# sq/Illuminant

Measured on AMD Instinct MI355X. Metric: Mparticle-steps/sec + lit Mpixels/sec (4K, 256 point lights) at 1/2/4/8 GPUs, higher is better.
Workload: dtype f32

## Files before the change

illuminant_amd/csrc/api.hip:

```cpp
#include <atomic>
#include <dlfcn.h>
#include <hip/hip_runtime.h>

#include <cstdarg>
#include <cmath>
#include <cstdio>
#include <cstdlib>
#include <algorithm>
#include <functional>
#include <array>
#include <cstring>
#include <mutex>
#include <new>
#include <unordered_map>
#include <vector>

#include "internal.hpp"

namespace {

using namespace ilm;

constexpr int kPlanePad = 1088;

// ... 120 lines not shown
            const hipError_t e = hipStreamWaitEvent(owner->main(), sh.readers[i].second, 0);
            if (e != hipSuccess) return e;
            sh.pending[i] = false;
        }
    return hipSuccess;
}
inline hipError_t shared_before_read(Shared& sh, Ctx* owner, Ctx* reader) {
    if (!sh.owner_ev) { const hipError_t e = hipEventCreateWithFlags(&sh.owner_ev, hipEventDisableTiming); if (e != hipSuccess) return e; }
    hipError_t e = hipEventRecord(sh.owner_ev, owner->main());
    if (e != hipSuccess) return e;
    return hipStreamWaitEvent(reader->main(), sh.owner_ev, 0);
}
inline hipError_t shared_after_read(Shared& sh, Ctx* reader) {
    size_t i = 0;
    while (i < sh.readers.size() && sh.readers[i].first != reader) i++;
    if (i == sh.readers.size()) {
        hipEvent_t ev = nullptr;
        const hipError_t e = hipEventCreateWithFlags(&ev, hipEventDisableTiming);
        if (e != hipSuccess) return e;
        sh.readers.emplace_back(reader, ev); sh.pending.push_back(false);
    }
    const hipError_t e = hipEventRecord(sh.readers[i].second, reader->main());
    if (e == hipSuccess) sh.pending[i] = true;
    return e;
}
inline bool siblings(const Ctx* a, const Ctx* b) { return a == b || (a->family != 0 && a->family == b->family && a->device == b->device); }

struct Sdf {
    uint32_t magic = kMagicSdf;
    Ctx* ctx = nullptr;
    Shared shared;
    uint2* texels = nullptr; int width = 0, height = 0, format = 0;
    int filter = ILM_SDF_FILTER_FP32;
    void* cells = nullptr; size_t cells_bytes = 0;
    uint64_t version = 1, cells_version = 0;
    void* cells0 = nullptr; size_t cells0_bytes = 0; uint64_t cells0_version = 0;
    int cells_slices = 0, cells_columns = 0, cells_sw = 0, cells_sh = 0;
    bool escaped = false;
    static constexpr int kDirtyWords = (kMaxTableSlices + 63) / 64;
    uint64_t dirty[kDirtyWords];
    Sdf() { for (uint64_t& w : dirty) w = ~0ull; }
    void mark_all_dirty() { for (uint64_t& w : dirty) w = ~0ull; version++; }
    void mark_slices_dirty(int first, int count) {
        const int64_t lo = std::max<int64_t>(0, (int64_t)first - 1), hi = std::min<int64_t>((int64_t)first + (int64_t)count, (int64_t)kDirtyWords * 64);
        for (int64_t v = lo; v < hi; v++) dirty[v >> 6] |= 1ull << (v & 63);
        version++;
    }
    uint64_t cell_rebuilds = 0, cell_slices_rebuilt = 0;
    int last_rebuilt_slices = 0, last_table_slices = 0;
};

struct GBuffer {
    uint32_t magic = kMagicGBuffer;
    Ctx* ctx = nullptr;
    Shared shared;
    void* texels = nullptr; int width = 0, height = 0, format = 0;
};

struct Lightmap {
    uint32_t magic = kMagicLightmap;
    Ctx* ctx = nullptr;
    void* texels = nullptr; int width = 0, height = 0, format = 0; bool external = false;
    void** d_mirrors = nullptr; int mirror_count = 0;
};

struct RenderKey {
    IlmClampedBezier4 color_from_life, color_from_velocity;
    IlmClampedBezier1 size_from_life, size_from_velocity;
    float rotation_from_life_and_index[2];
    IlmFloat4 life_ramp;
    float velocity_rotation;
};
static_assert(sizeof(RenderKey) == sizeof(float) * (2 * 20 + 2 * 8 + 2 + 4 + 1), "RenderKey has no padding");

struct System {
    uint32_t magic = kMagicSystem;
    Engine* engine = nullptr;
    std::vector<float*> chunks;
    std::vector<int32_t> used;
    std::vector<uint64_t> render_gen;
    std::vector<uint8_t> ptr_out;
    RenderKey render_key; uint64_t render_key_gen = 0;
    bool render_captured = false;
    DeviceScratch d_table; bool table_dirty = true;
    unsigned long long* d_counts = nullptr; int counts_cap = 0; int count_parity = 0;
    unsigned long long* counts_region(int r) const { return d_counts + (size_t)r * (size_t)counts_cap * kCountLines * kCountStride; }
    static size_t counts_bytes(int cap) { return sizeof(unsigned long long) * (size_t)cap * kCountStride * (4 * kCountLines + 1); }
    int split_at = -1;
    IlmHandle sdf_handle = 0;
    float4* ramp = nullptr; int ramp_w = 0, ramp_h = 0;
    DeviceScratch d_slots, d_slot_count;
    DeviceScratch spawn_positions[ILM_MAX_SPAWNS]; int spawn_position_count[ILM_MAX_SPAWNS] = {};
    float4* bitmap = nullptr; int bitmap_w = 0, bitmap_h = 0;
    float4* spawn_pattern[ILM_MAX_SPAWNS] = {}; int pattern_w[ILM_MAX_SPAWNS] = {}, pattern_h[ILM_MAX_SPAWNS] = {}, pattern_levels[ILM_MAX_SPAWNS] = {};
    unsigned long long* h_counts = nullptr; unsigned long long* h_counts_dev = nullptr; int h_counts_cap = 0;
    uint32_t count_seq = 0; int counts_first = 0, counts_span = 0;
    int counts_n = 0; bool counts_pending = false;
    bool counts_valid = false;
    uint32_t* h_sense = nullptr; size_t h_sense_cap = 0;
    hipEvent_t sense_ev = nullptr;
    int sense_n = 0; bool sense_pending = false;
};

SdfView make_sdf_view(const Sdf* f, const IlmDistanceFieldUniforms* df) {
    SdfView v;
    v.texels = f ? f->texels : nullptr;
    v.width = f ? f->width : 0;
    v.height = f ? f->height : 0;
    v.format = f ? f->format : ILM_SDF_UNORM16;
    v.wf = (float)v.width;
    v.hf = (float)v.height;
    v.inv_wf = v.width > 0 ? 1.0f / v.wf : 0.0f;
    v.wrap_half = 0.0f;
    v.cells0 = nullptr;
    v.table_slices = 0; v.columns = 1;
    v.box_x0 = v.box_y0 = v.box_z0 = 1.0f; v.box_x1 = v.box_y1 = v.box_z1 = 0.0f;
    if (df && v.width > 0) {
        const double cols = df->TextureSliceCount.x, rows = df->TextureSliceCount.y, slices = df->TextureSliceCount.w;
        const double isx = df->ConeAndMisc.w, isy = df->StepAndMisc2.w, ex = df->Extent.x, ey = df->Extent.y, ez = df->Extent.z;
        auto nearest = [](double x) { const double r = std::floor(x + 0.5); return (std::fabs(x - r) <= 1e-6 * std::fmax(1.0, r)) ? r : x; };
        const double sw = nearest(ex / isx), sh = nearest(ey / isy);
        auto whole = [](double x) { return std::isfinite(x) && x >= 1.0 && x == std::floor(x); };
        const bool consistent =
            whole(cols) && whole(rows) && whole(slices) && whole(sw) && whole(sh) && slices <= kMaxTableSlices && cols <= 1024 &&
            cols * sw == (double)v.width && rows * sh == (double)v.height && std::ceil(slices / 3.0) <= cols * rows &&
            std::fabs((double)df->TextureSliceAndTexelSize.x * cols - 1.0) < 1e-6 && std::fabs((double)df->TextureSliceAndTexelSize.y * rows - 1.0) < 1e-6 &&
            std::fabs((double)df->TextureSliceAndTexelSize.z * ex * cols - 1.0) < 1e-6 && std::fabs((double)df->TextureSliceAndTexelSize.w * ey * rows - 1.0) < 1e-6 &&
            ez > 0 && std::isfinite(ez) && std::isfinite((double)df->ConeAndMisc.y) && df->Packed1.y > 0.0f && std::isfinite((double)df->Packed1.y) &&
            df->Packed1.z > 0.0f && sw >= 4 && sh >= 4;
        bool rows_agree = consistent;
        for (int vi = 0; rows_agree && vi < (int)slices; vi++)
            rows_agree = floorf((float)vi * df->Packed1.x) == (float)((vi / 3) / (int)cols);
        if (consistent && rows_agree) {
            v.table_slices = (int)slices;
            v.columns = (int)cols;
            const double tx = 0.5625 * isx, ty = 0.5625 * isy;
            v.box_x0 = (float)tx; v.box_x1 = (float)(ex - tx);
            v.box_y0 = (float)ty; v.box_y1 = (float)(ey - ty);
            const double zmax = std::min({ (double)df->Packed1.z, ez, (slices - 1e-3) / (double)df->Packed1.y });
            v.box_z0 = df->ConeAndMisc.y; v.box_z1 = (float)((double)df->ConeAndMisc.y + zmax * (1.0 - 1e-6));
        }
    }
    if (df && v.width > 0) {
        const double third_max = std::floor(std::fabs((double)df->Packed1.z * (double)df->Packed1.y)) / 3.0 + 1.0;
        const double u_max = third_max * std::fabs((double)df->TextureSliceAndTexelSize.x) +
                             std::fabs((double)df->Extent.x * (double)df->TextureSliceAndTexelSize.z) + 1.0;
        const double x_max = u_max * (double)v.width;
        if (x_max == x_max && x_max < 1048576.0)
            v.wrap_half = 0.5f * v.inv_wf;
    }
    return v;
}

static const char* field_extent_unusable(const IlmDistanceFieldUniforms* df, char* text, size_t n) {
    if (!df) return nullptr;
    const float e[3] = { df->Extent.x, df->Extent.y, df->Extent.z };
    for (int k = 0; k < 3; k++) {
        if (std::isfinite(e[k]) && e[k] >= 0.0f) continue;
        snprintf(text, n, "the distance-field Extent.%c is %g: the field's extent must be finite and >= 0", "xyz"[k], (double)e[k]);
        return text;
    }
    return nullptr;
}

const char* field_uniforms_mismatch(const Sdf* f, const IlmDistanceFieldUniforms* df, char* text, size_t n) {
    if (!f || !df) return nullptr;
// ... 159 lines not shown
}
inline size_t align64(size_t x) { return (x + 63) & ~(size_t)63; }

int32_t reserve_field_params(Ctx* c, size_t total) { return reserve(c, c->d_field_params, total, total < 65536 ? 65536 : total * 2); }
int32_t check_volume_ranges(const IlmHeightVolume* volumes, int32_t volume_count, int32_t polygon_vertex_count) {
    for (int i = 0; i < volume_count; i++)
        if (volumes[i].FirstVertex < 0 || volumes[i].VertexCount < 0 || volumes[i].FirstVertex + volumes[i].VertexCount > polygon_vertex_count)
            return fail(ILM_ERR_OUT_OF_RANGE, "height volume %d vertex range outside the polygon array", i);
    return ILM_OK;
}
int32_t ensure_staging(Ctx* c, size_t bytes) { return reserve(c, c->staging, bytes, std::max<size_t>(bytes, (size_t)1 << 20)); }

int32_t upload_small_begin(Ctx* c, size_t bytes, void** host, int* slot_out) {
    const int slot = c->ring_pos;
    c->ring_pos = (c->ring_pos + 1) % Ctx::kRing;
    if (c->pinned_ev[slot] == nullptr)
        HIP_TRY(hipEventCreateWithFlags(&c->pinned_ev[slot], hipEventDisableTiming));
    else
        HIP_TRY(hipEventSynchronize(c->pinned_ev[slot]));
    if (c->pinned_bytes[slot] < bytes) {
        if (c->pinned[slot]) HIP_TRY(hipHostFree(c->pinned[slot]));
        c->pinned[slot] = nullptr; c->pinned_bytes[slot] = 0;
        size_t cap = bytes < 65536 ? 65536 : bytes;
        HIP_TRY(hipHostMalloc(&c->pinned[slot], cap, hipHostMallocDefault));
        c->pinned_bytes[slot] = cap;
    }
    *host = c->pinned[slot];
    *slot_out = slot;
    return ILM_OK;
}
__global__ __launch_bounds__(256) void copy_from_pinned_kernel(const uint4* __restrict__ src, uint4* __restrict__ dst, size_t words, size_t bytes) {
    for (size_t i = (size_t)blockIdx.x * 256 + threadIdx.x; i < words; i += (size_t)gridDim.x * 256) dst[i] = src[i];
    if (blockIdx.x == 0 && threadIdx.x < (bytes & 15)) {
        const size_t at = (bytes & ~(size_t)15) + threadIdx.x;
        reinterpret_cast<unsigned char*>(dst)[at] = reinterpret_cast<const unsigned char*>(src)[at];
    }
}
int32_t upload_small_commit(Ctx* c, void* dst, int slot, size_t bytes) {
    if (bytes > 4096 && bytes <= ((size_t)2 << 20) && (reinterpret_cast<uintptr_t>(dst) & 15) == 0) {
        void* dv = nullptr;
        HIP_TRY(hipHostGetDevicePointer(&dv, c->pinned[slot], 0));
        const size_t words = bytes / 16;
        const unsigned blocks = (unsigned)std::min<size_t>((words + 255) / 256, 1024);
        hipLaunchKernelGGL(copy_from_pinned_kernel, dim3(blocks ? blocks : 1), dim3(256), 0, c->main(), static_cast<const uint4*>(dv), static_cast<uint4*>(dst), words, bytes);
        HIP_TRY(hipGetLastError());
    } else {
        HIP_TRY(hipMemcpyAsync(dst, c->pinned[slot], bytes, hipMemcpyHostToDevice, c->main()));
    }
    HIP_TRY(hipEventRecord(c->pinned_ev[slot], c->main()));
    return ILM_OK;
}

int32_t upload_small(Ctx* c, void* dst, const void* src, size_t bytes) {
    void* host = nullptr;
    int slot = -1;
    const int32_t rc = upload_small_begin(c, bytes, &host, &slot);
    if (rc != ILM_OK) return rc;
    memcpy(host, src, bytes);
    return upload_small_commit(c, dst, slot, bytes);
}

int32_t stage_small(Ctx* c, const void* src, size_t bytes, const void** device_visible, int* slot_out) {
    void* host = nullptr;
    const int32_t rc = upload_small_begin(c, bytes, &host, slot_out);
    if (rc != ILM_OK) return rc;
    memcpy(host, src, bytes);
    void* dev = nullptr;
    HIP_TRY(hipHostGetDevicePointer(&dev, host, 0));
    *device_visible = dev;
    return ILM_OK;
}
int32_t staged_small_done(Ctx* c, int slot) {
    HIP_TRY(hipEventRecord(c->pinned_ev[slot], c->main()));
    return ILM_OK;
}

int32_t refresh_table(System* s) {
    Ctx* c = s->engine->ctx;
    const int n = (int)s->chunks.size();
    if (sizeof(float*) * (size_t)n > s->d_table.bytes) {
        const int32_t rc = reserve(c, s->d_table, sizeof(float*) * (size_t)n, sizeof(float*) * (size_t)(n < 64 ? 64 : n * 2));
        if (rc != ILM_OK) return rc;
        s->table_dirty = true;
    }
    if (n > s->counts_cap) {
        if (s->d_counts) { HIP_TRY(hipStreamSynchronize(c->main())); HIP_TRY(hipFree(s->d_counts)); s->d_counts = nullptr; }
        int cap = n < 64 ? 64 : n * 2;
        HIP_TRY(hipMalloc(reinterpret_cast<void**>(&s->d_counts), System::counts_bytes(cap)));
        HIP_TRY(hipMemsetAsync(s->d_counts, 0, System::counts_bytes(cap), c->main()));
        unsigned long long* old = s->h_counts;
        unsigned long long* fresh = nullptr;
        HIP_TRY(hipHostMalloc(reinterpret_cast<void**>(&fresh), sizeof(unsigned long long) * (size_t)cap, hipHostMallocMapped));
        for (int i = 0; i < cap; i++) fresh[i] = (i < s->h_counts_cap && old) ? old[i] : 0ull;
        if (old) HIP_TRY(hipHostFree(old));
        s->h_counts = fresh;
        HIP_TRY(hipHostGetDevicePointer(reinterpret_cast<void**>(&s->h_counts_dev), fresh, 0));
        s->h_counts_cap = cap;
        s->counts_cap = cap;
    }
    if (s->table_dirty && n > 0) {
        int32_t rc = upload_small(c, s->d_table.p, s->chunks.data(), sizeof(float*) * (size_t)n);
        if (rc != ILM_OK) return rc;
    }
    s->table_dirty = false;
    return ILM_OK;
}

static bool randomness_offset_unusable(const float off[2], const char* owner, int k, const char* what, char* text, size_t n) {
    for (int a = 0; a < 2; a++) {
        if (std::fabs(off[a]) < 4194304.0f) continue;
        snprintf(text, n, "%s %d: %s.%c is %g, outside (-2^22, 2^22)", owner, k, what, "xy"[a], (double)off[a]);
        return true;
    }
    return false;
}

static bool position_index_unusable(const IlmSpawnParams& p, int k, char* text, size_t n) {
    const float w = p.ChunkSizeAndIndices[3], count = p.PositionConstantCount, rate = p.PolygonRate;
    if (!std::isfinite(rate)) {
        snprintf(text, n, "spawn record %d: PolygonRate %g is not finite", k, (double)rate);
        return true;
    }
    if (count != std::floor(count)) {
        snprintf(text, n, "spawn record %d: PositionConstantCount %g is not an integer", k, (double)count);
        return true;
    }
    const bool polygon = rate > 0.05f;
    if (!(w >= 0.0f && w < count) || (!polygon && w != std::floor(w))) {
        snprintf(text, n, "spawn record %d: ChunkSizeAndIndices.w %g is not %s in [0, PositionConstantCount = %g)", k, (double)w,
                 polygon ? "a number" : "an integer", (double)count);
        return true;
    }
    return false;
}

int32_t validate_step(const System* s, const IlmStepDesc* d, int* first, int* count) {
    const int n = (int)s->chunks.size();
    if (d->OpCount < 0 || d->OpCount > ILM_MAX_OPS)
        return fail(ILM_ERR_TOO_MANY, "OpCount %d outside [0, %d]", d->OpCount, ILM_MAX_OPS);
    if (d->SpawnCount < 0 || d->SpawnCount > ILM_MAX_SPAWNS)
        return fail(ILM_ERR_TOO_MANY, "SpawnCount %d outside [0, %d]", d->SpawnCount, ILM_MAX_SPAWNS);
    if (d->UpdateMode < ILM_UPDATE_NONE || d->UpdateMode > ILM_UPDATE_ERASE)
        return fail(ILM_ERR_INVALID_ARGUMENT, "unknown UpdateMode %d", d->UpdateMode);
    for (int o = 0; o < d->OpCount; o++) {
        const IlmTransformOp& op = d->Ops[o];
        if (op.Type == ILM_OP_GRAVITY) {
            if (op.u.Gravity.AttractorCount > ILM_MAX_ATTRACTORS || op.u.Gravity.AttractorCount < 0)
                return fail(ILM_ERR_TOO_MANY, "Maximum number of attractors per instance is %d", ILM_MAX_ATTRACTORS);
        } else if (op.Type == ILM_OP_NOISE) {
            char why[256];
            if (randomness_offset_unusable(op.u.Noise.RandomnessOffset, "op", o, "RandomnessOffset", why, sizeof(why)) ||
                randomness_offset_unusable(op.u.Noise.NextRandomnessOffset, "op", o, "NextRandomnessOffset", why, sizeof(why)))
                return fail(ILM_ERR_OUT_OF_RANGE, "%s", why);
        } else if (op.Type != ILM_OP_FMA && op.Type != ILM_OP_MATRIX_MULTIPLY && op.Type != ILM_OP_SPATIAL_NOISE) {
            return fail(ILM_ERR_INVALID_ARGUMENT, "unknown transform type %d", op.Type);
        }
    }
    for (int k = 0; k < d->SpawnCount; k++) {
        const IlmSpawnRecord& r = d->Spawns[k];
        if (r.ChunkIndex < 0 || r.ChunkIndex >= n)
            return fail(ILM_ERR_OUT_OF_RANGE, "spawn target chunk %d outside [0, %d)", r.ChunkIndex, n);
        const float cs = r.Params.ChunkSizeAndIndices[0], first_i = r.Params.ChunkSizeAndIndices[1], last_i = r.Params.ChunkSizeAndIndices[2];
        if ((int)cs != s->engine->chunk_size)
            return fail(ILM_ERR_INVALID_ARGUMENT, "ChunkSizeAndIndices.x %g != engine chunk size %d", (double)cs, s->engine->chunk_size);
        if (first_i < 0 || last_i >= (float)s->engine->slots)
            return fail(ILM_ERR_OUT_OF_RANGE, "spawn range [%g, %g] outside the chunk", (double)first_i, (double)last_i);
// ... 324 lines not shown
                const float divisor = (op.Type == ILM_OP_NOISE) ? op.u.Noise.TimeDivisor : op.u.FMA.TimeDivisor;
                const int t = ar.AreaType < 0 ? -ar.AreaType : ar.AreaType;
                dv.op[o].area_none = (t < 1 || t > 5) ? 1 : 0;
                dv.op[o].t = ar.Strength * dt_ms / divisor;
                if (op.Type == ILM_OP_NOISE) {
                    const IlmNoiseParams& np = op.u.Noise;
                    const bool inert = (np.PositionScale.w == 0.0f) && std::isfinite(np.PositionOffset.w) && std::isfinite(np.PositionMinimum.w) &&
                                       std::isfinite(ar.Strength) && std::isfinite(dt_ms) && std::isfinite(divisor) && (divisor != 0.0f) &&
                                       std::isfinite(ar.AreaFalloff);
                    if (!inert) dv.noise_may_revive = 1;
                }
            } else if (op.Type == ILM_OP_SPATIAL_NOISE) {
                const IlmNoiseParams& np = op.u.SpatialNoise.Noise;
                const bool inert = (np.PositionScale.w == 0.0f) && std::isfinite(np.PositionOffset.w) && std::isfinite(np.Area.Strength) &&
                                   std::isfinite(dt_ms) && std::isfinite(np.TimeDivisor) && (np.TimeDivisor != 0.0f) && std::isfinite(np.Area.AreaFalloff);
                if (!inert) dv.noise_may_revive = 1;
            }
        }
    }
    a.partial_count = 0;
    {
        const bool noise_op = (a.op_mask & ((1u << ILM_OP_NOISE) | (1u << ILM_OP_SPATIAL_NOISE))) != 0u;
        const bool noise_touches_dead = noise_op && ((d->UpdateMode == ILM_UPDATE_NONE) || (a.derived.noise_may_revive != 0));
        for (int ci = first; noise_touches_dead && ci < first + count; ci++) s->used[(size_t)ci] = e->slots;
        for (int ci = first; !noise_touches_dead && ci < first + count && a.partial_count < kMaxPartialChunks; ci++) {
            const int used_units = (s->used[(size_t)ci] + 63) / 64;
            if (used_units * 64 < e->slots) {
                a.partial_chunk[a.partial_count] = ci;
                a.partial_units[a.partial_count] = used_units;
                a.partial_count++;
            }
        }
    }
    return ILM_OK;
}
static void finish_step(System* s, const IlmStepDesc* d, int first, int count) {
    if (d->UpdateMode == ILM_UPDATE_ERASE)
        for (int ci = first; ci < first + count; ci++) s->used[(size_t)ci] = 0;
    if (d->Flags & ILM_STEP_COUNT_LIVE) {
        s->counts_n = (int)s->chunks.size();
        s->counts_first = first; s->counts_span = count;
        s->counts_pending = true;
        s->counts_valid = true;
        s->count_parity ^= 1;
    }
}

int32_t run_step(System* s, const IlmStepDesc* d) {
    int first = 0, count = 0;
    StepLaunch a;
    const int32_t rc = prepare_step(s, d, a, &first, &count);
    if (rc != ILM_OK || count == 0) return rc;
    Engine* e = s->engine;
    Ctx* c = e->ctx;
    const bool counting = (d->Flags & ILM_STEP_COUNT_LIVE) != 0;
    const int region = s->count_parity;
    int mid = -1;
    if (step_streams() >= 2 && !c->exported && count >= 2 && (int64_t)count * (e->span / 64) >= kSplitMinUnits) {
        bool reads_other_chunks = false;
        for (int k = 0; k < d->SpawnCount; k++) reads_other_chunks = reads_other_chunks || (d->Spawns[k].Kind == ILM_SPAWN_FEEDBACK);
        if (!reads_other_chunks) {
            int64_t total = 0, left = 0;
            for (int ci = first; ci < first + count; ci++) total += (s->used[(size_t)ci] + 63) / 64 + 1;
            mid = first + 1;
            for (int ci = first; ci < first + count - 1; ci++) {
                left += (s->used[(size_t)ci] + 63) / 64 + 1;
                mid = ci + 1;
                if (2 * left >= total) break;
            }
        }
    }
    const uint64_t key = (d->UpdateMode == ILM_UPDATE_POSITIONS) ? render_key_generation(s, d) : 0;
    if (stream_capturing(c->stream_) || stream_capturing(c->aux)) s->render_captured = true;
    auto render_elide = [&](int lo, int hi) -> uint32_t {
        bool current = key != 0 && !s->render_captured;
        for (int ci = lo; current && ci < hi; ci++) current = (s->render_gen[(size_t)ci] == key) && !s->ptr_out[(size_t)ci];
        return current ? kElideDerived : 0u;
    };
    auto render_refreshed = [&](int lo, int hi, bool refreshed) {
        for (int ci = lo; ci < hi; ci++) s->render_gen[(size_t)ci] = (refreshed && key != 0 && !s->render_captured && !s->ptr_out[(size_t)ci]) ? key : 0;
    };
    const uint32_t elide_a = render_elide(first, (mid < 0) ? first + count : mid), elide_b = (mid < 0) ? 0u : render_elide(mid, first + count);
    render_refreshed(first, first + count, false);
    bool fresh_a = false, fresh_b = false;
    if (mid < 0) {
        HIP_TRY(launch_step(a, c->main(), elide_a, &fresh_a));
        render_refreshed(first, first + count, fresh_a);
    } else {
        if (s->split_at != mid) { (void)c->main(); s->split_at = mid; }
        if (c->main_pending) {
            HIP_TRY(hipEventRecord(c->ev_main, c->stream_));
            HIP_TRY(hipStreamWaitEvent(c->aux, c->ev_main, 0));
            c->main_pending = false;
        }
        StepLaunch b = a;
        a.chunk_count = mid - first;
        b.first_chunk = mid; b.chunk_count = first + count - mid;
        if (counting) {
            a.zero_n = b.zero_n = (int32_t)s->counts_cap * kCountLines;
            b.live_counts = s->counts_region(region * 2 + 1);
            b.zero_counts = s->counts_region((region ^ 1) * 2 + 1);
        }
        bool spawn_in_b = false;
        for (int k = 0; k < d->SpawnCount; k++) spawn_in_b = spawn_in_b || (d->Spawns[k].ChunkIndex >= mid);
        if (spawn_in_b) {
            HIP_TRY(launch_step(b, c->aux, elide_b, &fresh_b));
            c->aux_pending = true;
            HIP_TRY(launch_step(a, c->stream_, elide_a, &fresh_a));
        } else {
            HIP_TRY(launch_step(a, c->stream_, elide_a, &fresh_a));
            HIP_TRY(launch_step(b, c->aux, elide_b, &fresh_b));
            c->aux_pending = true;
        }
        render_refreshed(first, mid, fresh_a);
        render_refreshed(mid, first + count, fresh_b);
    }
    finish_step(s, d, first, count);
    return ILM_OK;
}

static int32_t fail_item(int32_t code, int item) {
    char text[sizeof(g_last_error)];
    snprintf(text, sizeof(text), "item %d: %s", item, g_last_error);
    memcpy(g_last_error, text, sizeof(text));
    return code;
}
int32_t run_step_batch(Engine* e, const IlmHandle* handles, const IlmStepDesc* descs, int32_t count) {
    Ctx* c = e->ctx;
    constexpr int kUnitsPerBlock = kStepThreads / 64;
    std::vector<System*> sys((size_t)count);
    size_t block_bound = 0;
    for (int i = 0; i < count; i++) {
        System* s = from_handle<System>(handles[i], kMagicSystem);
        if (!s) return fail(ILM_ERR_INVALID_HANDLE, "item %d: not a system handle", i);
        if (s->engine != e) return fail(ILM_ERR_INVALID_ARGUMENT, "item %d: the system belongs to another engine", i);
        int first = 0, n = 0;
        const int32_t rc = validate_step(s, &descs[i], &first, &n);
        if (rc != ILM_OK) return fail_item(rc, i);
        sys[(size_t)i] = s;
        block_bound += ((size_t)n * (size_t)(e->span / 64) + kUnitsPerBlock - 1) / kUnitsPerBlock;
    }
    HIP_TRY(hipSetDevice(c->device));
    const bool capturing = stream_capturing(c->stream_) || stream_capturing(c->aux);

    const size_t table_bytes = sizeof(StepBatchItem) * (size_t)count, bytes = table_bytes + sizeof(int32_t) * block_bound;
    StepBatchItem* items = nullptr;
    int32_t* item_of_block = nullptr;
    std::vector<StepLaunch> captured;
    int slot = -1;
    if (capturing) {
        captured.resize((size_t)count);
    } else {
        slot = e->batch_pos;
        e->batch_pos = (e->batch_pos + 1) % Engine::kBatchRing;
        if (e->batch_ev[slot] == nullptr) HIP_TRY(hipEventCreateWithFlags(&e->batch_ev[slot], hipEventDisableTiming));
        else HIP_TRY(hipEventSynchronize(e->batch_ev[slot]));
        if (e->batch_pinned_bytes[slot] < bytes) {
            if (e->batch_pinned[slot]) HIP_TRY(hipHostFree(e->batch_pinned[slot]));
            e->batch_pinned[slot] = nullptr; e->batch_pinned_bytes[slot] = 0;
            const size_t cap = std::max(bytes + bytes / 2, (size_t)1 << 16);
            HIP_TRY(hipHostMalloc(&e->batch_pinned[slot], cap, hipHostMallocDefault));
            e->batch_pinned_bytes[slot] = cap;
        }
        if (e->d_batch_bytes < bytes) {
            const size_t cap = std::max(std::max(bytes, e->d_batch_bytes * 2), (size_t)1 << 16);
            if (e->d_batch) e->d_batch_outgrown.push_back(e->d_batch);
            e->d_batch = nullptr; e->d_batch_bytes = 0;
            HIP_TRY(hipMalloc(&e->d_batch, cap));
            e->d_batch_bytes = cap;
        }
        items = static_cast<StepBatchItem*>(e->batch_pinned[slot]);
        item_of_block = reinterpret_cast<int32_t*>(static_cast<unsigned char*>(e->batch_pinned[slot]) + table_bytes);
    }
    auto record = [&](int i) -> StepLaunch& { return capturing ? captured[(size_t)i] : items[i].a; };

    struct Planned { int round, variant, blocks; };
    std::vector<Planned> plan((size_t)count);
    std::unordered_map<const System*, int> last_round;
    int rounds = 0, fallback = 0;
    for (int i = 0; i < count; i++) {
        System* s = sys[(size_t)i];
        const IlmStepDesc* d = &descs[i];
        int first = 0, n = 0;
        const int32_t rc = prepare_step(s, d, record(i), &first, &n);
        if (rc != ILM_OK) return fail_item(rc, i);
        plan[(size_t)i] = Planned{ 0, -1, 0 };
        if (n == 0) continue;
        if (d->UpdateMode == ILM_UPDATE_POSITIONS) (void)render_key_generation(s, d);
        if (capturing) s->render_captured = true;
        for (int ci = first; ci < first + n; ci++) s->render_gen[(size_t)ci] = 0;
        finish_step(s, d, first, n);

        Planned& p = plan[(size_t)i];
        p.variant = step_batch_layout(record(i), &p.blocks);
        if (capturing) p.variant = -1;
        if (p.variant < 0) fallback++;
        int after = last_round[s];
        for (int k = 0; k < d->SpawnCount; k++)
            if (d->Spawns[k].Kind == ILM_SPAWN_FEEDBACK) after = std::max(after, last_round[from_handle<System>(d->Spawns[k].Feedback.SourceSystem, kMagicSystem)]);
        p.round = after + 1;
        last_round[s] = p.round;
        for (int k = 0; k < d->SpawnCount; k++)
            if (d->Spawns[k].Kind == ILM_SPAWN_FEEDBACK) last_round[from_handle<System>(d->Spawns[k].Feedback.SourceSystem, kMagicSystem)] = p.round;
        rounds = std::max(rounds, p.round);
    }

    struct Launch { int round, variant, first_block, blocks, item; };
    std::vector<Launch> launches;
    size_t blocks_used = 0;
    for (int r = 1; r <= rounds; r++) {
        const size_t round_begin = launches.size();
        for (int i = 0; i < count; i++) {
            const Planned& p = plan[(size_t)i];
            if (p.round != r) continue;
            if (p.variant < 0) continue;
            size_t at = round_begin;
            while (at < launches.size() && launches[at].variant != p.variant) at++;
            if (at == launches.size()) launches.push_back(Launch{ r, p.variant, 0, 0, -1 });
            launches[at].blocks += p.blocks;
        }
        for (size_t l = round_begin; l < launches.size(); l++) {
            launches[l].first_block = (int)blocks_used;
            int block = 0;
            for (int i = 0; i < count; i++) {
                const Planned& p = plan[(size_t)i];
                if (p.round != r || p.variant != launches[l].variant) continue;
                items[i].first_block = block;
                items[i].block_count = p.blocks;
                for (int b = 0; b < p.blocks; b++) item_of_block[blocks_used + (size_t)block + (size_t)b] = i;
                block += p.blocks;
            }
            blocks_used += (size_t)launches[l].blocks;
        }
        for (int i = 0; i < count; i++)
            if (plan[(size_t)i].round == r && plan[(size_t)i].variant < 0) launches.push_back(Launch{ r, -1, 0, 0, i });
    }
    if (blocks_used > block_bound) return fail(ILM_ERR_STATE, "step batch: %zu blocks planned, %zu reserved", blocks_used, block_bound);

    const hipStream_t stream = c->main();
    int kernel_launches = 0;
    if (blocks_used > 0) {
        HIP_TRY(hipMemcpyAsync(e->d_batch, e->batch_pinned[slot], table_bytes + sizeof(int32_t) * blocks_used, hipMemcpyHostToDevice, stream));
        HIP_TRY(hipEventRecord(e->batch_ev[slot], stream));
    }
    const StepBatchItem* d_items = static_cast<const StepBatchItem*>(e->d_batch);
    const int32_t* d_item_of_block = reinterpret_cast<const int32_t*>(static_cast<const unsigned char*>(e->d_batch) + table_bytes);
    for (const Launch& l : launches) {
        if (l.variant >= 0) {
            HIP_TRY(launch_step_batch(l.variant, d_items, d_item_of_block + l.first_block, l.blocks, stream));
            kernel_launches++;
        } else {
            HIP_TRY(launch_step(record(l.item), stream, 0u, nullptr));
        }
    }
    e->last_batch_launches = kernel_launches; e->last_batch_rounds = rounds; e->last_batch_fallback = fallback;
    return ILM_OK;
}

int32_t copy_counts(System* s, const unsigned long long* d_region64, uint32_t* out, int32_t capacity, int32_t saturate16) {
    const uint32_t* d_region = reinterpret_cast<const uint32_t*>(d_region64);
    Ctx* c = s->engine->ctx;
    const int n = (int)s->chunks.size();
    if (capacity < n)
        return fail(ILM_ERR_OUT_OF_RANGE, "capacity %d < chunk count %d", capacity, n);
    if (n == 0) return ILM_OK;
    const size_t bytes = sizeof(uint32_t) * (size_t)n * kCountStride;
    std::vector<uint32_t> fallback;
    const uint32_t* tmp = nullptr;
    if ((reinterpret_cast<uintptr_t>(d_region) & 15) == 0 && bytes <= ((size_t)2 << 20)) {
        unsigned char* block = nullptr;
        int slot = -1;
        const int32_t rc = upload_small_begin(c, bytes, reinterpret_cast<void**>(&block), &slot);
        if (rc != ILM_OK) return rc;
        void* dv = nullptr;
        HIP_TRY(hipHostGetDevicePointer(&dv, block, 0));
        const size_t words = bytes / 16;
        hipLaunchKernelGGL(copy_from_pinned_kernel, dim3((unsigned)std::max<size_t>(1, std::min<size_t>((words + 255) / 256, 1024))), dim3(256), 0, c->main(),
                           reinterpret_cast<const uint4*>(d_region), static_cast<uint4*>(dv), words, bytes);
        HIP_TRY(hipGetLastError());
        const int32_t rc2 = staged_small_done(c, slot);
        if (rc2 != ILM_OK) return rc2;
        HIP_TRY(hipStreamSynchronize(c->main()));
        tmp = reinterpret_cast<const uint32_t*>(block);
    } else {
        fallback.resize((size_t)n * kCountStride);
        HIP_TRY(hipMemcpyAsync(fallback.data(), d_region, bytes, hipMemcpyDeviceToHost, c->main()));
        HIP_TRY(hipStreamSynchronize(c->main()));
        tmp = fallback.data();
    }
    for (int i = 0; i < n; i++) {
        const uint32_t v = tmp[(size_t)i * kCountStride];
        out[i] = (saturate16 && v > ref::kLiveCountSaturation) ? ref::kLiveCountSaturation : v;
    }
    return ILM_OK;
}

}

namespace ilm {
int32_t api_fail(int32_t code, const char* fmt, ...) {
    va_list ap;
    va_start(ap, fmt);
    vsnprintf(g_last_error, sizeof(g_last_error), fmt, ap);
    va_end(ap);
    return code;
}
IlmHandle handle_register(const void* object, uint32_t magic) {
    HandleRegistry& r = handle_registry();
    std::lock_guard<std::mutex> lock(r.mutex);
    r.live[reinterpret_cast<uintptr_t>(object)] = magic;
    return static_cast<IlmHandle>(reinterpret_cast<uintptr_t>(object));
}
bool handle_is_live(IlmHandle h, uint32_t magic) {
    HandleRegistry& r = handle_registry();
    std::lock_guard<std::mutex> lock(r.mutex);
    const auto it = r.live.find(static_cast<uintptr_t>(h));
    return it != r.live.end() && it->second == magic;
}
void handle_retire(const void* object) { retire_handle(object); }
int ctx_child_count(IlmHandle h) {
    const Ctx* c = from_handle<Ctx>(h, kMagicCtx);
    return c ? c->children : -1;
}
int set_step_streams(int n) { return set_step_streams_impl(n); }
int32_t system_chunk_view(IlmHandle system, int chunk, bool written, float** out_base, int64_t* out_stride, int32_t* out_chunk_size, IlmHandle* out_ctx) {
    System* s = from_handle<System>(system, kMagicSystem);
    if (!s) return fail(ILM_ERR_INVALID_HANDLE, "not a system handle");
    if (chunk < 0 || chunk >= (int)s->chunks.size()) return fail(ILM_ERR_OUT_OF_RANGE, "chunk %d outside [0, %d)", chunk, (int)s->chunks.size());
    if (out_base) *out_base = s->chunks[(size_t)chunk];
    if (out_stride) *out_stride = s->engine->stride;
    if (out_chunk_size) *out_chunk_size = s->engine->chunk_size;
    if (out_ctx) *out_ctx = to_handle(s->engine->ctx);
    if (written) {
        s->used[(size_t)chunk] = s->engine->slots;
        s->render_gen[(size_t)chunk] = 0;
    }
    return ILM_OK;
}
hipStream_t ctx_stream_joined(IlmHandle h) {
    Ctx* c = from_handle<Ctx>(h, kMagicCtx);
    return c ? c->main() : nullptr;
}
const TraceApi& trace_api() {
    static const TraceApi api = [] {
        TraceApi t;
        const char* e = getenv("ILM_TRACE");
        if (!e || atoi(e) == 0) return t;
        for (const char* name : { "librocprofiler-sdk-roctx.so.1", "librocprofiler-sdk-roctx.so", "libroctx64.so.4", "libroctx64.so" }) {
            void* lib = dlopen(name, RTLD_NOW | RTLD_GLOBAL);
            if (!lib) continue;
            t.push = reinterpret_cast<int (*)(const char*)>(dlsym(lib, "roctxRangePushA"));
            t.pop = reinterpret_cast<int (*)()>(dlsym(lib, "roctxRangePop"));
            if (t.push && t.pop) { t.on = true; break; }
        }
        if (!t.on) fprintf(stderr, "libilluminant_hip: ILM_TRACE is set but no roctx library could be bound: no ranges\n");
        return t;
    }();
    return api;
}
static std::mutex g_armed_mutex;
static std::vector<Lightmap*> g_armed;
static std::atomic<int> g_armed_count{0};
static void forget_armed(const Lightmap* m) {
    std::lock_guard<std::mutex> lock(g_armed_mutex);
    g_armed.erase(std::remove(g_armed.begin(), g_armed.end(), m), g_armed.end());
    g_armed_count.store((int)g_armed.size(), std::memory_order_release);
}

int32_t lightmap_set_mirrors(IlmHandle h, void* const* buffers, int count) {
    Lightmap* m = from_handle<Lightmap>(h, kMagicLightmap);
    if (!m) return fail(ILM_ERR_INVALID_HANDLE, "not a lightmap handle");
    if (count < 0 || count > 64 || (count > 0 && !buffers)) return fail(ILM_ERR_INVALID_ARGUMENT, "bad mirror list");
    HIP_TRY(hipSetDevice(m->ctx->device));
    HIP_TRY(hipStreamSynchronize(m->ctx->main()));
    std::vector<Lightmap*>& armed = m->ctx->mirrored;
    armed.erase(std::remove(armed.begin(), armed.end(), m), armed.end());
    forget_armed(m);
    if (count == 0) {
        if (m->d_mirrors) HIP_TRY(hipFree(m->d_mirrors));
        m->d_mirrors = nullptr; m->mirror_count = 0;
        return ILM_OK;
    }
    if (!m->d_mirrors) HIP_TRY(hipMalloc(reinterpret_cast<void**>(&m->d_mirrors), sizeof(void*) * 64));
    HIP_TRY(hipMemcpy(m->d_mirrors, buffers, sizeof(void*) * (size_t)count, hipMemcpyHostToDevice));
    m->mirror_count = count;
    armed.push_back(m);
    {
        std::lock_guard<std::mutex> lock(g_armed_mutex);
        g_armed.push_back(m);
        g_armed_count.store((int)g_armed.size(), std::memory_order_release);
    }
    return ILM_OK;
}

static const Lightmap* mirror_table_of(const Lightmap* m, bool* foreign) {
    *foreign = false;
    if (m->d_mirrors && m->mirror_count > 0) return m;
    if (!m->external || g_armed_count.load(std::memory_order_acquire) == 0) return nullptr;
    for (const Lightmap* e : m->ctx->mirrored)
        if (e->texels == m->texels && e->width == m->width && m->height <= e->height && e->format == m->format && e->d_mirrors && e->mirror_count > 0) return e;
    std::lock_guard<std::mutex> lock(g_armed_mutex);
    for (const Lightmap* e : g_armed)
        if (e->texels == m->texels && e->ctx != m->ctx) *foreign = true;
    return nullptr;
}
static int32_t set_launch_mirrors(const Lightmap* m, LightLaunch* a) {
    bool foreign = false;
    const Lightmap* t = mirror_table_of(m, &foreign);
    if (foreign)
        return fail(ILM_ERR_STATE, "the lightmap aliases the buffer of a group lightmap member that ANOTHER context holds in store mode: a pass from here "
                                   "would not be mirrored into the other members' frames (render through the member's context, or disarm the mode)");
    a->mirrors = t ? t->d_mirrors : nullptr; a->mirror_count = t ? t->mirror_count : 0;
    return ILM_OK;
}
}

extern "C" {

// ... 152 lines not shown
    *out = h;
    return ILM_OK;
}

static int32_t acquire_chunk(Engine* e, float** out) {
    if (e->spare.empty()) {
        const size_t bytes = e->chunk_bytes();
        const int k = (int)std::min<size_t>(8, std::max<size_t>(1, ((size_t)64 << 20) / bytes));
        float* base = nullptr;
        hipError_t err = hipMalloc(reinterpret_cast<void**>(&base), bytes * (size_t)k);
        int got = k;
        if (err != hipSuccess && k > 1) { (void)hipGetLastError(); got = 1; err = hipMalloc(reinterpret_cast<void**>(&base), bytes); }
        if (err != hipSuccess) return fail((int32_t)err, "a particle chunk of %zu bytes: %s", bytes, hipGetErrorString(err));
        HIP_TRY(hipMemsetAsync(base, 0, bytes * (size_t)got, e->ctx->main()));
        e->slabs.push_back(Engine::Slab{ base, got });
        for (int i = got - 1; i >= 0; i--) e->spare.push_back(base + (size_t)i * (bytes / sizeof(float)));
    }
    *out = e->spare.back();
    e->spare.pop_back();
    return ILM_OK;
}
static void release_chunk(Engine* e, float* chunk) {
    (void)hipMemsetAsync(chunk, 0, e->chunk_bytes(), e->ctx->main());
    e->spare.push_back(chunk);
    const size_t chunk_floats = e->chunk_bytes() / sizeof(float);
    while ((int)e->spare.size() > Engine::kSpareChunks) {
        size_t victim = e->slabs.size();
        for (size_t i = 0; i < e->slabs.size() && victim == e->slabs.size(); i++) {
            const float* lo = e->slabs[i].base; const float* hi = lo + (size_t)e->slabs[i].chunks * chunk_floats;
            int spare_here = 0;
            for (const float* p : e->spare) spare_here += (p >= lo && p < hi) ? 1 : 0;
            if (spare_here == e->slabs[i].chunks) victim = i;
        }
        if (victim == e->slabs.size()) break;
        const float* lo = e->slabs[victim].base; const float* hi = lo + (size_t)e->slabs[victim].chunks * chunk_floats;
        e->spare.erase(std::remove_if(e->spare.begin(), e->spare.end(), [&](const float* p) { return p >= lo && p < hi; }), e->spare.end());
        (void)hipStreamSynchronize(e->ctx->main());
        (void)hipFree(e->slabs[victim].base);
        e->slabs.erase(e->slabs.begin() + (long)victim);
    }
}

int32_t ilm_engine_destroy(IlmHandle h) {
    Engine* e = from_handle<Engine>(h, kMagicEngine);
    if (!e) return fail(ILM_ERR_INVALID_HANDLE, "not an engine handle");
    if (e->children > 0) return fail(ILM_ERR_STATE, "%d system(s) of this engine are still alive", e->children);
    e->ctx->children--;
    (void)hipSetDevice(e->ctx->device);
    (void)hipStreamSynchronize(e->ctx->main());
    if (e->rnd) (void)hipFree(e->rnd);
    if (e->rnd_lp) (void)hipFree(e->rnd_lp);
    for (const Engine::Slab& slab : e->slabs) (void)hipFree(slab.base);
    for (int k = 0; k < Engine::kBatchRing; k++) {
        if (e->batch_pinned[k]) (void)hipHostFree(e->batch_pinned[k]);
        if (e->batch_ev[k]) (void)hipEventDestroy(e->batch_ev[k]);
    }
    if (e->d_batch) (void)hipFree(e->d_batch);
    for (void* p : e->d_batch_outgrown) (void)hipFree(p);
    retire_handle(e);
    delete e;
    return ILM_OK;
}

int32_t ilm_system_create(IlmHandle hengine, IlmHandle* out) {
    Engine* e = from_handle<Engine>(hengine, kMagicEngine);
    if (!e) return fail(ILM_ERR_INVALID_HANDLE, "not an engine handle");
    if (!out) return fail(ILM_ERR_INVALID_ARGUMENT, "NULL argument");
    System* s = new (std::nothrow) System();
    if (!s) return fail(ILM_ERR_INVALID_ARGUMENT, "out of host memory");
    s->engine = e;
    e->children++;
    *out = to_handle(s);
    return ILM_OK;
}

int32_t ilm_system_destroy(IlmHandle h) {
    System* s = from_handle<System>(h, kMagicSystem);
    if (!s) return fail(ILM_ERR_INVALID_HANDLE, "not a system handle");
    Ctx* c = s->engine->ctx;
    s->engine->children--;
    (void)hipSetDevice(c->device);
    (void)hipStreamSynchronize(c->main());
    for (float* p : s->chunks) release_chunk(s->engine, p);
    for (DeviceScratch* b : { &s->d_table, &s->d_slots, &s->d_slot_count }) release(*b);
    for (DeviceScratch& b : s->spawn_positions) release(b);
    if (s->d_counts) (void)hipFree(s->d_counts);
    if (s->ramp) (void)hipFree(s->ramp);
    for (int k = 0; k < ILM_MAX_SPAWNS; k++)
        if (s->spawn_pattern[k]) (void)hipFree(s->spawn_pattern[k]);
    if (s->bitmap) (void)hipFree(s->bitmap);
    if (s->h_counts) (void)hipHostFree(s->h_counts);
    if (s->h_sense) (void)hipHostFree(s->h_sense);
    if (s->sense_ev) (void)hipEventDestroy(s->sense_ev);
    retire_handle(s);
    delete s;
    return ILM_OK;
}

int32_t ilm_system_add_chunk(IlmHandle h, int32_t* out_index) {
    System* s = from_handle<System>(h, kMagicSystem);
    if (!s) return fail(ILM_ERR_INVALID_HANDLE, "not a system handle");
    Engine* e = s->engine;
    HIP_TRY(hipSetDevice(e->ctx->device));
    float* base = nullptr;
    { const int32_t rc = acquire_chunk(e, &base); if (rc != ILM_OK) return rc; }
    s->chunks.push_back(base);
    s->used.push_back(0);
    s->render_gen.push_back(0);
    s->ptr_out.push_back(0);
    s->table_dirty = true;
    if (out_index) *out_index = (int32_t)s->chunks.size() - 1;
    return ILM_OK;
}

int32_t ilm_system_remove_chunk(IlmHandle h, int32_t index) {
    System* s = from_handle<System>(h, kMagicSystem);
    if (!s) return fail(ILM_ERR_INVALID_HANDLE, "not a system handle");
    if (index < 0 || index >= (int)s->chunks.size())
        return fail(ILM_ERR_OUT_OF_RANGE, "chunk %d outside [0, %d)", index, (int)s->chunks.size());
    Ctx* c = s->engine->ctx;
    HIP_TRY(hipSetDevice(c->device));
    HIP_TRY(hipStreamSynchronize(c->main()));
    release_chunk(s->engine, s->chunks[(size_t)index]);
    s->chunks.erase(s->chunks.begin() + index);
    s->used.erase(s->used.begin() + index);
    s->render_gen.erase(s->render_gen.begin() + index);
    s->ptr_out.erase(s->ptr_out.begin() + index);
    s->table_dirty = true;
    return ILM_OK;
}

int32_t ilm_system_chunk_count(IlmHandle h, int32_t* out_count) {
    System* s = from_handle<System>(h, kMagicSystem);
    if (!s || !out_count) return fail(ILM_ERR_INVALID_HANDLE, "not a system handle");
    *out_count = (int32_t)s->chunks.size();
    return ILM_OK;
}

static int32_t check_plane_range(System* s, int32_t chunk, int32_t plane, int32_t first_slot, int32_t count) {
    if (chunk < 0 || chunk >= (int)s->chunks.size())
        return fail(ILM_ERR_OUT_OF_RANGE, "chunk %d outside [0, %d)", chunk, (int)s->chunks.size());
    if (plane < ILM_PLANE_POSITION || plane > ILM_PLANE_RENDER_DATA)
        return fail(ILM_ERR_INVALID_ARGUMENT, "unknown plane %d", plane);
    if (first_slot < 0 || count < 0 || first_slot + count > s->engine->slots)
        return fail(ILM_ERR_OUT_OF_RANGE, "slot range [%d, %d) outside [0, %d)", first_slot, first_slot + count, s->engine->slots);
    return ILM_OK;
}

int32_t ilm_chunk_upload(IlmHandle h, int32_t chunk, int32_t plane, const IlmFloat4* src, int32_t first_slot, int32_t count) {
    ILM_TRACE_RANGE("ilm_chunk_upload");
    System* s = from_handle<System>(h, kMagicSystem);
    if (!s) return fail(ILM_ERR_INVALID_HANDLE, "not a system handle");
    if (!src) return fail(ILM_ERR_INVALID_ARGUMENT, "src is NULL");
    int32_t rc = check_plane_range(s, chunk, plane, first_slot, count);
    if (rc != ILM_OK || count == 0) return rc;
    Engine* e = s->engine; Ctx* c = e->ctx;
    HIP_TRY(hipSetDevice(c->device));
    const size_t bytes = sizeof(float4) * (size_t)count;
    rc = ensure_staging(c, bytes);
    if (rc != ILM_OK) return rc;
    HIP_TRY(hipMemcpyAsync(c->staging.p, src, bytes, hipMemcpyHostToDevice, c->main()));
    s->used[(size_t)chunk] = std::max(s->used[(size_t)chunk], first_slot + count);
    s->render_gen[(size_t)chunk] = 0;
    HIP_TRY(launch_aos_to_soa(c->staging.as<const float4>(), s->chunks[(size_t)chunk] + (int64_t)plane * 4 * e->stride,
                              e->stride, first_slot, count, c->main()));
    HIP_TRY(hipStreamSynchronize(c->main()));
    return ILM_OK;
}

int32_t ilm_chunk_download(IlmHandle h, int32_t chunk, int32_t plane, IlmFloat4* dst, int32_t first_slot, int32_t count) {
    ILM_TRACE_RANGE("ilm_chunk_download");
    System* s = from_handle<System>(h, kMagicSystem);
    if (!s) return fail(ILM_ERR_INVALID_HANDLE, "not a system handle");
    if (!dst) return fail(ILM_ERR_INVALID_ARGUMENT, "dst is NULL");
    int32_t rc = check_plane_range(s, chunk, plane, first_slot, count);
    if (rc != ILM_OK || count == 0) return rc;
    Engine* e = s->engine; Ctx* c = e->ctx;
    HIP_TRY(hipSetDevice(c->device));
    const size_t bytes = sizeof(float4) * (size_t)count;
    rc = ensure_staging(c, bytes);
    if (rc != ILM_OK) return rc;
    HIP_TRY(launch_soa_to_aos(s->chunks[(size_t)chunk] + (int64_t)plane * 4 * e->stride, e->stride,
                              c->staging.as<float4>(), first_slot, count, c->main()));
    HIP_TRY(hipMemcpyAsync(dst, c->staging.p, bytes, hipMemcpyDeviceToHost, c->main()));
    HIP_TRY(hipStreamSynchronize(c->main()));
    return ILM_OK;
}

int32_t ilm_chunk_device_ptr(IlmHandle h, int32_t chunk, int32_t component, void** out_ptr, int64_t* out_stride) {
    System* s = from_handle<System>(h, kMagicSystem);
    if (!s) return fail(ILM_ERR_INVALID_HANDLE, "not a system handle");
    if (chunk < 0 || chunk >= (int)s->chunks.size() || component < 0 || component >= kComponents)
        return fail(ILM_ERR_OUT_OF_RANGE, "chunk/component out of range");
    if (out_ptr) *out_ptr = s->chunks[(size_t)chunk] + (int64_t)component * s->engine->stride;
    s->used[(size_t)chunk] = s->engine->slots;
    s->render_gen[(size_t)chunk] = 0;
    s->ptr_out[(size_t)chunk] = 1;
    if (out_stride) *out_stride = s->engine->stride;
    return ILM_OK;
}

int32_t ilm_system_set_distance_field(IlmHandle h, IlmHandle hsdf) {
    System* s = from_handle<System>(h, kMagicSystem);
    if (!s) return fail(ILM_ERR_INVALID_HANDLE, "not a system handle");
    if (hsdf == 0) { s->sdf_handle = 0; return ILM_OK; }
    Sdf* f = from_handle<Sdf>(hsdf, kMagicSdf);
    if (!f) return fail(ILM_ERR_INVALID_HANDLE, "not a distance field handle");
    if (f->ctx != s->engine->ctx) return fail(ILM_ERR_INVALID_ARGUMENT, "distance field belongs to another context");
    { char why[256]; if (field_filter_unsupported(f, "a particle system", why, sizeof(why))) return fail(ILM_ERR_INVALID_ARGUMENT, "%s", why); }
    s->sdf_handle = hsdf;
    return ILM_OK;
}

int32_t ilm_system_set_life_ramp(IlmHandle h, const IlmFloat4* texels, int32_t width, int32_t height) {
    System* s = from_handle<System>(h, kMagicSystem);
    if (!s) return fail(ILM_ERR_INVALID_HANDLE, "not a system handle");
    Ctx* c = s->engine->ctx;
    HIP_TRY(hipSetDevice(c->device));
    HIP_TRY(hipStreamSynchronize(c->main()));
    if (s->ramp) { HIP_TRY(hipFree(s->ramp)); s->ramp = nullptr; s->ramp_w = s->ramp_h = 0; }
    if (!texels || width <= 0 || height <= 0) return ILM_OK;
    const size_t bytes = sizeof(float4) * (size_t)width * (size_t)height;
    HIP_TRY(hipMalloc(reinterpret_cast<void**>(&s->ramp), bytes));
    HIP_TRY(hipMemcpy(s->ramp, texels, bytes, hipMemcpyHostToDevice));
    s->ramp_w = width; s->ramp_h = height;
    return ILM_OK;
}

int32_t ilm_system_set_spawn_positions(IlmHandle h, int32_t slot, const IlmFloat4* positions, int32_t count) {
    System* s = from_handle<System>(h, kMagicSystem);
    if (!s) return fail(ILM_ERR_INVALID_HANDLE, "not a system handle");
    if (slot < 0 || slot >= ILM_MAX_SPAWNS) return fail(ILM_ERR_OUT_OF_RANGE, "spawn slot %d outside [0, %d)", slot, ILM_MAX_SPAWNS);
    if (count < 0 || (count > 0 && !positions)) return fail(ILM_ERR_INVALID_ARGUMENT, "bad position list");
    if (count > (1 << 20)) return fail(ILM_ERR_TOO_MANY, "at most %d positions", 1 << 20);
    Ctx* c = s->engine->ctx;
    HIP_TRY(hipSetDevice(c->device));
    int32_t rc = reserve(c, s->spawn_positions[slot], sizeof(float4) * (size_t)count, sizeof(float4) * (size_t)((count + 127) / 128 * 128));
    if (rc != ILM_OK) return rc;
    if (count > 0) {
        rc = upload_small(c, s->spawn_positions[slot].p, positions, sizeof(float4) * (size_t)count);
        if (rc != ILM_OK) return rc;
    }
    s->spawn_position_count[slot] = count;
    return ILM_OK;
}

int32_t ilm_system_set_spawn_pattern(IlmHandle h, int32_t slot, const IlmFloat4* texels, int32_t width, int32_t height, int32_t levels) {
    System* s = from_handle<System>(h, kMagicSystem);
    if (!s) return fail(ILM_ERR_INVALID_HANDLE, "not a system handle");
    if (slot < 0 || slot >= ILM_MAX_SPAWNS) return fail(ILM_ERR_OUT_OF_RANGE, "spawn slot %d outside [0, %d)", slot, ILM_MAX_SPAWNS);
    if (levels < 0 || levels > 16) return fail(ILM_ERR_OUT_OF_RANGE, "%d mip levels outside [0, 16]", levels);
    if (levels > 0 && (!texels || width < 1 || height < 1 || width > 16384 || height > 16384))
        return fail(ILM_ERR_INVALID_ARGUMENT, "bad pattern texture (%d x %d)", width, height);
    Ctx* c = s->engine->ctx;
    HIP_TRY(hipSetDevice(c->device));
    HIP_TRY(hipStreamSynchronize(c->main()));
    if (s->spawn_pattern[slot]) HIP_TRY(hipFree(s->spawn_pattern[slot]));
    s->spawn_pattern[slot] = nullptr;
    s->pattern_w[slot] = s->pattern_h[slot] = s->pattern_levels[slot] = 0;
    if (levels == 0) return ILM_OK;
    size_t total = 0;
    for (int l = 0, lw = width, lh = height; l < levels; l++) {
        total += (size_t)lw * (size_t)lh;
        lw = std::max(1, lw >> 1); lh = std::max(1, lh >> 1);
    }
    HIP_TRY(hipMalloc(reinterpret_cast<void**>(&s->spawn_pattern[slot]), sizeof(float4) * total));
    HIP_TRY(hipMemcpy(s->spawn_pattern[slot], texels, sizeof(float4) * total, hipMemcpyHostToDevice));
    s->pattern_w[slot] = width; s->pattern_h[slot] = height; s->pattern_levels[slot] = levels;
    return ILM_OK;
}

int32_t ilm_system_step(IlmHandle h, const IlmStepDesc* desc) {
    ILM_TRACE_RANGE("ilm_system_step");
    System* s = from_handle<System>(h, kMagicSystem);
    if (!s) return fail(ILM_ERR_INVALID_HANDLE, "not a system handle");
    if (!desc) return fail(ILM_ERR_INVALID_ARGUMENT, "desc is NULL");
    return run_step(s, desc);
}

// ... 405 lines not shown
    HIP_TRY(hipMemcpyAsync(out_distances, d_out, out_bytes, hipMemcpyDeviceToHost, c->main()));
    HIP_TRY(hipStreamSynchronize(c->main()));
    return ILM_OK;
}

int32_t ilm_debug_sdf_sample_inside(IlmHandle h, const IlmDistanceFieldUniforms* df, const float* positions, int32_t count, float* out_distances,
                                    int32_t* out_used_table) {
    Sdf* f = from_handle<Sdf>(h, kMagicSdf);
    if (!f) return fail(ILM_ERR_INVALID_HANDLE, "not a distance field handle");
    if (!df || count < 0 || (count > 0 && (!positions || !out_distances || !out_used_table))) return fail(ILM_ERR_INVALID_ARGUMENT, "bad arguments");
    { char why[256]; if (field_extent_unusable(df, why, sizeof(why))) return fail(ILM_ERR_INVALID_ARGUMENT, "%s", why); }
    if (count == 0) return ILM_OK;
    Ctx* c = f->ctx;
    HIP_TRY(hipSetDevice(c->device));
    const size_t in_bytes = sizeof(float) * 3 * (size_t)count, out_bytes = sizeof(float) * (size_t)count;
    int32_t rc = ensure_staging(c, in_bytes + 2 * out_bytes);
    if (rc != ILM_OK) return rc;
    float* d_in = c->staging.as<float>();
    float* d_out = d_in + 3 * (size_t)count;
    int32_t* d_used = reinterpret_cast<int32_t*>(d_out + (size_t)count);
    HIP_TRY(hipMemcpyAsync(d_in, positions, in_bytes, hipMemcpyHostToDevice, c->main()));
    TraceSdfView view;
    HIP_TRY(make_trace_view(f, df, c->main(), &view));
    HIP_TRY(launch_sdf_sample_inside(view, *df, d_in, count, d_out, d_used, c->main(), f->filter));
    HIP_TRY(hipMemcpyAsync(out_distances, d_out, out_bytes, hipMemcpyDeviceToHost, c->main()));
    HIP_TRY(hipMemcpyAsync(out_used_table, d_used, out_bytes, hipMemcpyDeviceToHost, c->main()));
    HIP_TRY(hipStreamSynchronize(c->main()));
    return ILM_OK;
}

int32_t ilm_debug_divide_by_constants(IlmHandle hctx, float* out_divisors, uint64_t* out_mismatches, int32_t capacity, int32_t* out_count) {
    Ctx* c = from_handle<Ctx>(hctx, kMagicCtx);
    if (!c) return fail(ILM_ERR_INVALID_HANDLE, "not a context handle");
    if (!out_divisors || !out_mismatches || !out_count || capacity < 2) return fail(ILM_ERR_INVALID_ARGUMENT, "bad arguments");
    HIP_TRY(hipSetDevice(c->device));
    float pairs[2][2];
    light_constant_divisors(pairs);
    for (int i = 0; i < 2; i++) {
        HIP_TRY(hipMemsetAsync(c->d_stats, 0, 2 * sizeof(unsigned long long), c->main()));
        HIP_TRY(launch_divide_by_constant(pairs[i][0], pairs[i][1], c->d_stats, c->main()));
        unsigned long long bad[2] = { 0, 0 };
        HIP_TRY(hipMemcpyAsync(bad, c->d_stats, sizeof(bad), hipMemcpyDeviceToHost, c->main()));
        HIP_TRY(hipStreamSynchronize(c->main()));
        out_divisors[i] = pairs[i][0];
        out_mismatches[2 * i] = bad[0];
        out_mismatches[2 * i + 1] = bad[1];
    }
    *out_count = 2;
    return ILM_OK;
}

int32_t ilm_debug_step_interpreter(int32_t interpreter) { return (int32_t)set_step_interpreter(interpreter); }
int32_t ilm_debug_last_step_kernel(void) { return (int32_t)last_step_kernel(); }
int32_t ilm_debug_step_streams(int32_t streams) { return (int32_t)set_step_streams(streams); }
int32_t ilm_debug_last_light_launch(IlmHandle hctx, int32_t* out_workgroups, int32_t* out_split, int32_t* out_tile_macro) {
    Ctx* c = from_handle<Ctx>(hctx, kMagicCtx);
    if (!c) return fail(ILM_ERR_INVALID_HANDLE, "not a context handle");
    if (out_workgroups) *out_workgroups = c->last_light_blocks;
    if (out_split) *out_split = c->last_light_split;
    if (out_tile_macro) *out_tile_macro = c->last_light_macro;
    return ILM_OK;
}

int32_t ilm_debug_step_sdf_samples(IlmHandle hctx, int32_t enable, uint64_t* out_samples) {
    Ctx* c = from_handle<Ctx>(hctx, kMagicCtx);
    if (!c) return fail(ILM_ERR_INVALID_HANDLE, "not a context handle");
    HIP_TRY(hipSetDevice(c->device));
    HIP_TRY(hipStreamSynchronize(c->main()));
    unsigned long long value = 0;
    HIP_TRY(step_sdf_sample_counter(enable, &value));
    if (out_samples) *out_samples = (uint64_t)value;
    return ILM_OK;
}

int32_t ilm_debug_step_regular_waves(IlmHandle hctx, int32_t enable, uint64_t* out_regular, uint64_t* out_selected) {
    Ctx* c = from_handle<Ctx>(hctx, kMagicCtx);
    if (!c) return fail(ILM_ERR_INVALID_HANDLE, "not a context handle");
    HIP_TRY(hipSetDevice(c->device));
    HIP_TRY(hipStreamSynchronize(c->main()));
    unsigned long long value[2] = { 0, 0 };
    HIP_TRY(step_regular_wave_counter(enable, value));
    if (out_regular) *out_regular = (uint64_t)value[0];
    if (out_selected) *out_selected = (uint64_t)value[1];
    return ILM_OK;
}

int32_t ilm_debug_divide(IlmHandle hctx, const float* numerators, const float* denominators, int32_t count, float* out_fast, float* out_ieee) {
    Ctx* c = from_handle<Ctx>(hctx, kMagicCtx);
    if (!c) return fail(ILM_ERR_INVALID_HANDLE, "not a context handle");
    if (count < 0 || (count > 0 && (!numerators || !denominators || !out_fast || !out_ieee))) return fail(ILM_ERR_INVALID_ARGUMENT, "bad arguments");
    if (count == 0) return ILM_OK;
    HIP_TRY(hipSetDevice(c->device));
    const size_t bytes = sizeof(float) * (size_t)count;
    int32_t rc = ensure_staging(c, 4 * bytes);
    if (rc != ILM_OK) return rc;
    float* d_n = c->staging.as<float>();
    float* d_d = d_n + count; float* d_f = d_d + count; float* d_i = d_f + count;
    HIP_TRY(hipMemcpyAsync(d_n, numerators, bytes, hipMemcpyHostToDevice, c->main()));
    HIP_TRY(hipMemcpyAsync(d_d, denominators, bytes, hipMemcpyHostToDevice, c->main()));
    HIP_TRY(launch_divide_probe(d_n, d_d, count, d_f, d_i, c->main()));
    HIP_TRY(hipMemcpyAsync(out_fast, d_f, bytes, hipMemcpyDeviceToHost, c->main()));
    HIP_TRY(hipMemcpyAsync(out_ieee, d_i, bytes, hipMemcpyDeviceToHost, c->main()));
    HIP_TRY(hipStreamSynchronize(c->main()));
    return ILM_OK;
}

int32_t ilm_sdf_destroy(IlmHandle h) {
    Sdf* f = from_handle<Sdf>(h, kMagicSdf);
    if (!f) return fail(ILM_ERR_INVALID_HANDLE, "not a distance field handle");
    f->ctx->children--;
    (void)hipSetDevice(f->ctx->device);
    (void)hipStreamSynchronize(f->ctx->main());
    for (auto& r : f->shared.readers) (void)hipEventSynchronize(r.second);
    f->shared.release();
    if (f->texels) (void)hipFree(f->texels);
    if (f->cells) (void)hipFree(f->cells);
    if (f->cells0) (void)hipFree(f->cells0);
    retire_handle(f);
    delete f;
    return ILM_OK;
}

int32_t ilm_sdf_download(IlmHandle h, uint16_t* texels) {
    ILM_TRACE_RANGE("ilm_sdf_download");
    Sdf* f = from_handle<Sdf>(h, kMagicSdf);
    if (!f) return fail(ILM_ERR_INVALID_HANDLE, "not a distance field handle");
    if (!texels) return fail(ILM_ERR_INVALID_ARGUMENT, "texels is NULL");
    HIP_TRY(hipSetDevice(f->ctx->device));
    HIP_TRY(hipMemcpyAsync(texels, f->texels, sizeof(uint2) * (size_t)f->width * (size_t)f->height, hipMemcpyDeviceToHost, f->ctx->main()));
    HIP_TRY(hipStreamSynchronize(f->ctx->main()));
    return ILM_OK;
}

int32_t ilm_sdf_device_ptr(IlmHandle h, void** out_ptr) {
    Sdf* f = from_handle<Sdf>(h, kMagicSdf);
    if (!f || !out_ptr) return fail(ILM_ERR_INVALID_HANDLE, "not a distance field handle");
    *out_ptr = f->texels;
    f->escaped = true;
    return ILM_OK;
}

int32_t ilm_sdf_mark_dirty(IlmHandle h, int32_t first_virtual_slice, int32_t slice_count) {
    Sdf* f = from_handle<Sdf>(h, kMagicSdf);
    if (!f) return fail(ILM_ERR_INVALID_HANDLE, "not a distance field handle");
    if (slice_count < 0 || first_virtual_slice < 0) return fail(ILM_ERR_OUT_OF_RANGE, "slices [%d, %d + %d)", first_virtual_slice, first_virtual_slice, slice_count);
    if (slice_count == 0) f->mark_all_dirty(); else f->mark_slices_dirty(first_virtual_slice, slice_count);
    f->escaped = false;
    return ILM_OK;
}

int32_t ilm_sdf_trace_info(IlmHandle h, IlmSdfTraceInfo* out) {
    Sdf* f = from_handle<Sdf>(h, kMagicSdf);
    if (!f || !out) return fail(ILM_ERR_INVALID_HANDLE, "not a distance field handle");
    out->CellBytes = (uint64_t)f->cells_bytes;
    out->CellRebuilds = f->cell_rebuilds; out->CellSlicesRebuilt = f->cell_slices_rebuilt;
    out->LastRebuiltSlices = f->last_rebuilt_slices; out->TableSlices = f->last_table_slices;
    out->RebuiltEveryFrame = f->escaped ? 1 : 0; out->Reserved = 0;
    return ILM_OK;
}

int32_t ilm_sdf_set_filter(IlmHandle h, int32_t fraction_bits) {
    Sdf* f = from_handle<Sdf>(h, kMagicSdf);
    if (!f) return fail(ILM_ERR_INVALID_HANDLE, "not a distance field handle");
    if (fraction_bits != ILM_SDF_FILTER_FP32 && fraction_bits != ILM_SDF_FILTER_FIXED8)
        return fail(ILM_ERR_INVALID_ARGUMENT, "filter of %d fraction bits: ILM_SDF_FILTER_FP32 (0) or ILM_SDF_FILTER_FIXED8 (8)", fraction_bits);
    f->filter = fraction_bits;
// ... 1690 lines not shown
```

illuminant_amd/csrc/internal.hpp:

```cpp
#pragma once

#include <hip/hip_runtime.h>
#include <stdint.h>

#include "../../include/illuminant_hip.h"
#include "hlsl_math.hpp"

namespace ilm {

constexpr int kComponents = 20;
constexpr int kSlotsPerThread = 4;
constexpr int kStepThreads = 128;
constexpr int kSlotsPerBlock = 1024;

struct StepDerived {
    float dt_s;
    float inv_rw, inv_rh;
    int32_t cs_shift;
    int32_t noise_may_revive;
    uint32_t bezier_codes;
    uint32_t update_bits;
    struct NoiseFast {
        int32_t op;
        int32_t classes;
        int32_t yb[4];
        uint32_t wcode[16];
        IlmFloat4 position[3][3];
        IlmFloat4 velocity[3][3];
    } noise;
    struct Op {
        int32_t area_none;
        float   t;
        float   max_accel;
        int32_t _pad;
    } op[ILM_MAX_OPS];
};

constexpr int kNoiseBigClasses = 5;
static_assert(sizeof(IlmSpawnRecord) * ILM_MAX_SPAWNS >= 2 * kNoiseBigClasses * kNoiseBigClasses * sizeof(IlmFloat4), "noise tables fit the spawn records");

constexpr int kMaxPartialChunks = 4;
struct StepLaunch {
    IlmStepDesc desc;
    StepDerived derived;
    float* const* chunk_bases;
    int64_t stride;
    int32_t span;
    int32_t chunk_size;
    int32_t slots;
    int32_t first_chunk, chunk_count;
    uint32_t op_mask;
    int32_t streaming;
    const float4* rnd; int32_t rw, rh;
    const uint2* rnd_lp;
    const float4* ramp; int32_t ramp_w, ramp_h;
    const float4* spawn_positions[ILM_MAX_SPAWNS]; int32_t spawn_position_count[ILM_MAX_SPAWNS];
    const float* source_base[ILM_MAX_SPAWNS];
    const float4* spawn_pattern[ILM_MAX_SPAWNS]; int32_t pattern_w[ILM_MAX_SPAWNS], pattern_h[ILM_MAX_SPAWNS], pattern_levels[ILM_MAX_SPAWNS];
    SdfView sdf;
    int32_t partial_count; int32_t partial_chunk[kMaxPartialChunks]; int32_t partial_units[kMaxPartialChunks];
    unsigned long long* live_counts;
    unsigned long long* zero_counts;
    unsigned long long* host_counts;
    uint32_t count_seq;
    int32_t zero_n;
    int32_t count_buckets;
    int32_t units_per_chunk;
    int32_t upc_shift;
    int32_t unit_begin, unit_end;
    int32_t unit_rotate, total_padded;
};

static_assert(sizeof(StepLaunch) <= 4096, "StepLaunch travels in the kernarg segment (4 KB)");

struct alignas(4096) StepBatchItem {
    StepLaunch a;
    int32_t first_block;
    int32_t block_count;
};
static_assert(sizeof(StepBatchItem) == 4096 && offsetof(StepBatchItem, a) == 0, "a batch record is its StepLaunch plus the block range, 4 KB");

constexpr int kCountStride = 16;
constexpr int kCountLines = 17;
constexpr uint32_t kElideDerived = 1u;
constexpr uint32_t kElideColor = 2u;
constexpr uint32_t kElideRotation = 4u;
hipError_t launch_step(StepLaunch& a, hipStream_t stream, uint32_t render_elide = 0u, bool* refreshed = nullptr);
int step_batch_layout(StepLaunch& a, int* blocks);
hipError_t launch_step_batch(int variant, const StepBatchItem* table, const int32_t* item_of_block, int blocks, hipStream_t stream);
hipError_t step_sdf_sample_counter(int enable, unsigned long long* out);
hipError_t step_regular_wave_counter(int enable, unsigned long long out[2]);
bool step_wants_slice0_cells(const IlmStepDesc& d, int format);
hipError_t launch_build_slice0_cells(const uint2* texels, int width, int height, void* cells, hipStream_t stream);
int set_step_interpreter(int on);
int last_step_kernel();
int set_step_streams(int n);
hipStream_t ctx_stream_joined(IlmHandle ctx);
struct TraceApi { int (*push)(const char*) = nullptr; int (*pop)() = nullptr; bool on = false; };
const TraceApi& trace_api();
struct TraceRange {
    bool on;
    explicit TraceRange(const char* name) : on(trace_api().on) { if (on) (void)trace_api().push(name); }
    ~TraceRange() { if (on) (void)trace_api().pop(); }
    TraceRange(const TraceRange&) = delete;
    TraceRange& operator=(const TraceRange&) = delete;
};
#define ILM_TRACE_RANGE(name) ::ilm::TraceRange ilm_trace_range_(name)
int32_t lightmap_set_mirrors(IlmHandle lightmap, void* const* buffers, int count);

hipError_t launch_aos_to_soa(const float4* src, float* plane0, int64_t stride, int32_t first_slot, int32_t count, hipStream_t stream);
hipError_t launch_soa_to_aos(const float* plane0, int64_t stride, float4* dst, int32_t first_slot, int32_t count, hipStream_t stream);

hipError_t launch_count_live(float* const* chunk_bases, int64_t stride, int32_t span, int32_t slots, int32_t chunk_count, uint32_t* counts, hipStream_t stream);
constexpr int kSenseStride = 32;
struct SenseLaunch {
    float* const* chunk_bases; int64_t stride; int32_t span, slots;
    int32_t first_chunk, chunk_count, sensor_count;
    int32_t tiles_per_block;
    uint32_t* counts;
    IlmAreaParams sensors[ILM_MAX_SENSORS];
};
hipError_t launch_sense(SenseLaunch& a, hipStream_t stream);
hipError_t launch_live_slots(const float* life, int32_t slots, uint32_t* out_slots, uint32_t capacity, uint32_t* out_count, uint32_t* block_counts, hipStream_t stream);

struct GBufferView {
    const void* texels;
    int32_t width, height, format;
};

struct RampView { const float4* texels; int32_t width, height; };

struct LightLaunch {
    int32_t light_count;
    IlmEnvironment env;
    IlmDistanceFieldUniforms df;
    GBufferView gbuffer;
    TraceSdfView sdf;
    float ambient[4];
    void* lightmap; int32_t width, height, format;
    int32_t row_begin, row_end;
    unsigned long long* stats;
    const int32_t* light_count_ptr;
    int32_t accumulate;
    int32_t blend_fp16;
    RampView ramp;
    int32_t tile_macro;
    const uint16_t* group_order;
    int32_t split;
    int32_t taper[3], taper_slots;
    float4* partials;
    uint32_t* tickets;
    void* const* mirrors;
    int32_t mirror_count;
    int16_t blend_color, blend_alpha;
};
static_assert(sizeof(LightLaunch) == 456, "the blend functions fill the descriptor's tail padding: the kernels' argument offsets stay where they were");
constexpr int kLightParts = 8;
constexpr int kLightTile = 16;
constexpr int kLightTileThreads = (kLightTile / 8) * (kLightTile / 8) * 64;

constexpr size_t kLightRecBytes = 128;
struct TraceGate {
    float x0, x1, y0, y1, z0, z1;
    float field_ok;
};
TraceGate make_trace_gate(const IlmDistanceFieldUniforms& df, const SdfView& sdf);
hipError_t launch_prepare_lights(const IlmLightVertex* lights, int count, const IlmEnvironment& env, const IlmDistanceFieldUniforms& df,
                                 const SdfView& sdf, void* recs, hipStream_t stream);
hipError_t launch_sphere_lights_prepared(const LightLaunch& a, const void* recs, hipStream_t stream, int sdf_filter = ILM_SDF_FILTER_FP32);
hipError_t launch_prepare_directional_lights(const IlmLightVertex* lights, int count, const IlmEnvironment& env, const IlmDistanceFieldUniforms& df,
                                             void* recs, hipStream_t stream);
hipError_t launch_directional_lights_prepared(const LightLaunch& a, const void* recs, hipStream_t stream);
constexpr size_t kProjectorRecBytes = 192;
constexpr int32_t kMaxProjectorLights = 1 << 24;
// ... 255 lines not shown
```

illuminant_amd/csrc/particles.hip:

```cpp
#include <cmath>
#include <cstddef>
#include <cstdlib>
#include <cstring>

#include <atomic>
#include <type_traits>
#include "internal.hpp"
#include "distance_functions.hpp"
#include "bezier.hpp"

namespace ilm {

ILM_DEV float dt_seconds(const IlmParticleSystemUniforms& s) { return s.GlobalSettings.x / kVelocityConstantScale; }

ILM_DEV bool category_ok(float type, const float mm[2]) { return (type >= mm[0]) && (type <= mm[1]); }

ILM_DEV float4 random_custom(const float4* __restrict__ rnd, int rw, int rh, float texel_x, float texel_y, float x, float y,
                             float off_x, float off_y, float rate_x, float rate_y) {
#pragma clang fp contract(off)
    const float u = ((x * rate_x) + off_x) * texel_x;
    const float v = ((y * rate_y) + off_y) * texel_y;
    const int tx = wrap_index_fast(floorf(u * (float)rw), rw);
    const int ty = wrap_index_fast(floorf(v * (float)rh), rh);
    return rnd[ty * rw + tx];
// ... 535 lines not shown

ILM_DEV float render_index(float vx, float vy) { return vx + (vy * ref::kRenderDataIndexRowPitch); }
ILM_DEV float rotation_unscaled(float vx, float vy) { return ((vx != vx) || (vy != vy)) ? __builtin_nanf("") : 0.0f; }
ILM_DEV float render_rotation(float rotation, float life, float index, const IlmParticleSystemUniforms& sys, const IlmUpdateParams& p) {
    return (rotation * sys.AnimationRateAndRotationAndZToY.z) + ((life * p.RotationFromLifeAndIndex[0]) + (index * p.RotationFromLifeAndIndex[1]));
}

ILM_DEV void render_data(float vx, float vy, float4 position, float4 velocity, float4 attributes,
                         const IlmParticleSystemUniforms& sys, const IlmUpdateParams& p, uint32_t codes, uint32_t bits,
                         const float4* __restrict__ ramp, int ramp_w, int ramp_h,
                         float4& render_color, float4& rdata) {
    if (position.w <= 0.0f) {
        render_color = rdata = mk4(0.0f, 0.0f, 0.0f, 0.0f);
        return;
    }
    const float index = render_index(vx, vy);
    const float velocity_length = fmaxf(len3_fast(xyz(velocity)), 0.0001f);

    float4 color = mul4(bezier4_coded(p.ColorFromLife, position.w, codes & 0xFFu), bezier4_coded(p.ColorFromVelocity, velocity_length, (codes >> 8) & 0xFFu));
    if (bits & 1u) {
        float u = (position.w - p.LifeRampSettings.y) / p.LifeRampSettings.z;
        if (bits & 4u)
            u = 1.0f - sat(u);
        const float v = index / p.LifeRampSettings.w;
        float4 texel = mk4(1.0f, 1.0f, 1.0f, 1.0f);
        if (ramp != nullptr && ramp_w > 0 && ramp_h > 0) {
            const int tx = clamp_tap(floorf(u * (float)ramp_w), ramp_w);
            const int ty = wrap_index(floorf(v * (float)ramp_h), ramp_h);
            texel = ramp[ty * ramp_w + tx];
        }
        color = lerp4(color, mul4(texel, color), sat(fabsf(p.LifeRampSettings.x)));
    }

    float4 rc = mul4(attributes, color);
    rc.w = sat(rc.w);
    rc.x *= rc.w; rc.y *= rc.w; rc.z *= rc.w;
    render_color = rc;

    float rotation = 0.0f;
    if (bits & 2u) {
        rotation = rotation_unscaled(velocity.x, velocity.y);
    } else if (!((fabsf(velocity.x) < 0.01f) && (fabsf(velocity.y) < 0.01f))) {
        rotation = atan2f(velocity.y, velocity.x);
        if (rotation < 0.0f)
            rotation += 2.0f * kPi;
    }
    rdata.x = bezier1_coded(p.SizeFromLife, position.w, (codes >> 16) & 0xFFu) * bezier1_coded(p.SizeFromVelocity, velocity_length, codes >> 24);
    rdata.y = render_rotation(rotation, position.w, index, sys, p);
    rdata.z = velocity_length;
    rdata.w = velocity.w;
}

ILM_DEV void update_positions(float4& pos, float4& vel, const IlmParticleSystemUniforms& sys, float dts) {
#pragma clang fp contract(off)
    const f3 velocity = friction_and_maximum(xyz(vel), sys, dts);
    const float new_life = pos.w - (sys.GlobalSettings.w * dts);
    if (new_life <= 0.0f) {
        pos = vel = mk4(0.0f, 0.0f, 0.0f, 0.0f);
    } else {
        pos = mk4(pos.x + velocity.x * dts, pos.y + velocity.y * dts, pos.z + velocity.z * dts, new_life);
        vel = mk4(velocity.x, velocity.y, velocity.z, vel.w);
    }
}
ILM_DEV void update_positions_select(float4& pos, float4& vel, const IlmParticleSystemUniforms& sys, float dts, bool live) {
#pragma clang fp contract(off)
    const f3 velocity = friction_and_maximum(xyz(vel), sys, dts);
    const float new_life = pos.w - (sys.GlobalSettings.w * dts);
    const bool keep = live && !(new_life <= 0.0f);
    pos = mk4(keep ? pos.x + velocity.x * dts : 0.0f, keep ? pos.y + velocity.y * dts : 0.0f, keep ? pos.z + velocity.z * dts : 0.0f, keep ? new_life : 0.0f);
    vel = mk4(keep ? velocity.x : 0.0f, keep ? velocity.y : 0.0f, keep ? velocity.z : 0.0f, keep ? vel.w : 0.0f);
}
ILM_DEV void update_positions_unselected(float4& pos, float4& vel, const IlmParticleSystemUniforms& sys, float dts) {
#pragma clang fp contract(off)
    const f3 velocity = friction_and_maximum(xyz(vel), sys, dts);
    const float new_life = pos.w - (sys.GlobalSettings.w * dts);
    pos = mk4(pos.x + velocity.x * dts, pos.y + velocity.y * dts, pos.z + velocity.z * dts, new_life);
    vel = mk4(velocity.x, velocity.y, velocity.z, vel.w);
}

__device__ unsigned long long g_step_sdf_samples;
__device__ int g_step_count_sdf_samples;
__device__ unsigned long long g_step_regular_waves[2];
__device__ int g_step_count_regular_waves;

template <int FMT>
ILM_DEV void df_long(float4& pos, float4& vel, float x, float y, float initial_distance, float step_distance0, bool first_done,
                     const IlmParticleSystemUniforms& sys, float dts, const IlmDistanceFieldUniforms& df, const SdfView& sdf, int& samples) {
#pragma clang fp contract(off)
    const float4 zero = mk4(0.0f, 0.0f, 0.0f, 0.0f);
    float new_life = pos.w - (sys.GlobalSettings.w * dts);
    const float collision_distance = sys.CollisionSettings.z;
    const float max_velocity = sys.GlobalSettings.z;
    const f3 old_xyz = xyz(pos);
    const f3 unit_vector = norm3(xyz(vel));
    const f3 velocity = friction_and_maximum(xyz(vel), sys, dts);
    const f3 scaled_velocity = velocity * dts;

    bool collided = false, escaping = false;
    f3 collision_position = mk3(0.0f, 0.0f, 0.0f), new_position = old_xyz;
    float4 new_velocity = zero;

    const bool was_colliding = initial_distance < collision_distance;
    float travel_distance = fmaxf(0.0f, fminf(initial_distance, len3(scaled_velocity)));
    int step_count = ref::kMaxStepCount;
    if (was_colliding)
        step_count = 1;
    else if (travel_distance <= 0.001f)
        step_count = 0;

    for (int i = 0; i < step_count; i++) {
        const f3 test_position = old_xyz + (unit_vector * travel_distance);
        float step_distance = step_distance0;
        if (!(first_done && i == 0)) {
            step_distance = sample_distance_field<(FMT & 1), true, (FMT & 2) != 0, (FMT & 4) != 0>(test_position, df, sdf);
            samples++;
        }
        if (step_distance < collision_distance) {
            collided = true;
            collision_position = test_position;
        }
        escaping = step_distance > initial_distance;
        if (collided && !escaping) {
            collision_position = test_position;
            const float offset = clampf(step_distance + collision_distance, 0.05f, 16.0f);
            travel_distance = fmaxf(0.0f, travel_distance - offset);
        } else
            step_count = 0;
        if (travel_distance <= 0.001f)
            step_count = 0;
    }

    if (collided) {
        const bool bounce = vel.w <= 0.0f;
        const bool redirect = was_colliding && !escaping;
        f3 normal = mk3(0.0f, 0.0f, 0.0f);
        if (bounce || redirect) {
            normal = estimate_normal4<FMT>(collision_position, df, sdf);
            samples += 4;
        }
        const float escape_speed = fminf(max_velocity, sys.CollisionSettings.x);
        if (redirect) {
            normal = normal * mk3(1.0f, 1.0f, 0.0f);
            if (len3(normal) < ref::kNoNormalThreshold) {
                const float a = (x / 67.0f) + (y / 13.0f);
                normal = mk3(sinf(a), cosf(a), 0.0f);
            }
            const f3 nv = (norm3(normal) * escape_speed) * ref::kInitialEscapeSpeed;
            new_velocity = mk4(nv.x, nv.y, nv.z, ref::kBounceDelay);
            new_position = old_xyz + (nv * dts);
        } else if (bounce) {
            const float d2 = 2.0f * dot3(normal, unit_vector);
            f3 bounce_vector = ((normal - unit_vector) * d2) * -1.0f;
            if (len3(bounce_vector) < ref::kNoNormalThreshold)
                bounce_vector = unit_vector * -1.0f;
            else
                bounce_vector = norm3(bounce_vector);
            new_position = collision_position;
            const f3 nv = bounce_vector * fminf(max_velocity, len3(velocity) * sys.CollisionSettings.y);
            new_velocity = mk4(nv.x, nv.y, nv.z, ref::kBounceDelay);
            new_life -= sys.CollisionSettings.w;
        } else {
            const float new_speed = fmaxf(len3(xyz(vel)) * ref::kEscapeSpeedAcceleration, escape_speed);
            const f3 nv = unit_vector * new_speed;
            new_velocity = mk4(nv.x, nv.y, nv.z, 0.0f);
            new_position = old_xyz + (unit_vector * travel_distance);
        }
// ... 295 lines not shown
                            a.units_per_chunk / kUnitsPerBlock, a.count_buckets, a.live_counts, a.zero_counts, a.zero_n, a.host_counts, a.count_seq);
    }
}

typedef const StepBatchItem __attribute__((address_space(4))) CStepBatchItem;
typedef const int32_t __attribute__((address_space(4))) CInt32;
ILM_DEV void touch_record_lines_step(CStepLaunch* ap) {
    uint32_t sink;
    asm volatile(ILM_T16(0x0) ILM_T16(0x400) ILM_T16(0x800) ILM_T4(0xc00) ILM_T4(0xd00) ILM_T4(0xe00) ILM_T1(0xf00) ILM_T1(0xf40) ILM_T1(0xf80)
                 "s_waitcnt lgkmcnt(0)" : "=&s"(sink) : "s"(ap));
}
template <int FMT, bool DF, bool SPAWN, int MINW, bool EXT = false>
__global__ __launch_bounds__(kStepThreads, MINW) void step_batch_kernel(const StepBatchItem* table, const int32_t* item_of_block) {
    __shared__ uint32_t wave_live[kStepThreads / 64];
    const int item = ((CInt32*)item_of_block)[blockIdx.x];
    CStepBatchItem* ip = (CStepBatchItem*)table + item;
    CStepLaunch* ap = (CStepLaunch*)ip;
    const StepLaunch& a = *(const StepLaunch*)ap;
    const int block = (int)blockIdx.x - ip->first_block;
    if (block < kTouchBlocks) touch_record_lines_step(ap);
    const unsigned lane = threadIdx.x & 63u;
    const int wave = __builtin_amdgcn_readfirstlane((int)threadIdx.x >> 6);
    int v = block * (kStepThreads / 64) + a.unit_rotate;
    const int total = a.unit_end - a.unit_begin;
    if (v >= a.total_padded) v -= a.total_padded;
    const int u = a.unit_begin + v + wave;
    uint32_t n_live = 0;
    if (v + wave < total) {
        const int chunk_rel = (a.upc_shift >= 0) ? (u >> a.upc_shift) : (u / a.units_per_chunk);
        const int seg = u - chunk_rel * a.units_per_chunk;
        const int chunk = a.first_chunk + chunk_rel;
        bool untouched = false;
        for (int k = 0; k < a.partial_count; k++)
            untouched = untouched || ((a.partial_chunk[k] == chunk) && (seg >= a.partial_units[k]));
        if (!untouched) {
            const UnitPlanes up = unit_planes(((CBase*)a.chunk_bases)[chunk], a.stride, seg * 64);
            const SlotIn cur = load_slot<true, false>(up, lane * 4u);
            NoiseDeltas noise;
            noise.valid = false;
            if (a.derived.noise.op >= 0) {
                const int first = seg * 64;
                const int row = (a.derived.cs_shift >= 0) ? (first >> a.derived.cs_shift) : (first / a.chunk_size);
                noise = noise_prepare(a.derived.noise, reinterpret_cast<const IlmFloat4*>(&a.desc.Spawns[0]), first - row * a.chunk_size, row);
            }
            const bool live_after = process_unit<FMT, DF, SPAWN, EXT, false>(ap, up, chunk, seg * 64 + (int)lane, lane, seg, cur, noise);
            n_live = (uint32_t)__popcll(__ballot(live_after));
        }
    }
    if (a.desc.Flags & ILM_STEP_COUNT_LIVE) {
        const int first_unit = a.unit_begin + v;
        const int chunk_rel = (a.upc_shift >= 0) ? (first_unit >> a.upc_shift) : (first_unit / a.units_per_chunk);
        constexpr int kUnitsPerBlock = kStepThreads / 64;
        publish_block_count_at(block == 0, wave_live, n_live, lane, wave, v < total, a.first_chunk + chunk_rel,
                               (first_unit - chunk_rel * a.units_per_chunk) / kUnitsPerBlock, a.units_per_chunk / kUnitsPerBlock, a.count_buckets,
                               a.live_counts, a.zero_counts, a.zero_n, a.host_counts, a.count_seq);
    }
}

struct LeanAttractor { float x, y, z, radius, strength, _p0, _p1, _p2; };
constexpr int kLeanMaxAttractors = 8;
struct LeanGravity {
    int32_t count; uint32_t types;
    float max_accel, _pad0;
    float cat_lo, cat_hi, _pad1, _pad2;
    LeanAttractor a[kLeanMaxAttractors];
};
union LeanOp {
    LeanGravity gravity;
    IlmNoiseParams noise;
    IlmFMAParams fma;
};
struct LeanStep {
    float* const* chunk_bases;
    unsigned long long* live_counts; unsigned long long* zero_counts; unsigned long long* host_counts;
    int64_t stride;
    int32_t upc_shift, unit_rotate, total_padded, total_units;
    int32_t first_chunk, cs_shift, zero_n; uint32_t flags;
    uint32_t count_seq; int32_t count_buckets;
    float regular_cat_lo, regular_cat_hi;
    int32_t partial_chunk[kMaxPartialChunks], partial_units[kMaxPartialChunks];
    int32_t partial_count, op_count, spawn_count; uint32_t elide;
    int32_t op_type[ILM_MAX_OPS];
    int32_t spawn_chunk[ILM_MAX_SPAWNS], spawn_unit_lo[ILM_MAX_SPAWNS], spawn_unit_hi[ILM_MAX_SPAWNS];
    int32_t _pad1[2];
    float dt_s; uint32_t bezier_codes, update_bits; int32_t noise_op;
    IlmParticleSystemUniforms sys;
    IlmUpdateParams update;
    StepDerived::Op dop[ILM_MAX_OPS];
    LeanOp op[ILM_MAX_OPS];
    StepDerived::NoiseFast noise;
    const float4* rnd; int32_t rw, rh; float inv_rw, inv_rh; int32_t _pad2[2];
    union {
        IlmSpawnRecord spawns[ILM_MAX_SPAWNS];
        IlmFloat4 noise_big[2 * kNoiseBigClasses * kNoiseBigClasses];
    };
};
static_assert(sizeof(LeanStep) <= 4096, "LeanStep travels in the kernarg segment (4 KB)");

template <bool FILTER = true>
ILM_DEV void apply_gravity_lean(float4& pos, float4& vel, const LeanGravity& g, float dt_ms, float mv) {
    if (FILTER && ((pos.w <= 0.0f) || !((vel.w >= g.cat_lo) && (vel.w <= g.cat_hi))))
        return;
    f3 acceleration = mk3(0.0f, 0.0f, 0.0f);
    const uint32_t types = g.types;
    int i = 0;
#ifndef ILM_GRAVITY_EXACT
    for (; i + 4 <= g.count && ((((types >> (2 * i)) | (types >> (2 * i + 1))) & 0x55u) == 0x55u); i += 4) {
        f3 term[4];
#pragma unroll
        for (int k = 0; k < 4; k++) {
            const LeanAttractor A = g.a[i + k];
            const bool squared = ((types >> (2 * (i + k))) & 2u) != 0u;
            term[k] = gravity_term(mk3(A.x, A.y, A.z) - xyz(pos), squared ? 2u : 1u, A.radius, A.strength, dt_ms);
        }
        acceleration = (((acceleration + term[0]) + term[1]) + term[2]) + term[3];
    }
#endif
    for (; i < g.count; i++) {
        const LeanAttractor A = g.a[i];
        acceleration = acceleration + gravity_term(mk3(A.x, A.y, A.z) - xyz(pos), (types >> (2 * i)) & 3u, A.radius, A.strength, dt_ms);
    }
    gravity_finish(vel, acceleration, g.max_accel, mv);
}

typedef const LeanStep __attribute__((address_space(4))) CLeanStep;
static_assert(sizeof(LeanStep) >= 0xc84 && sizeof(LeanStep) <= 0xcc0, "touch_kernarg_lines_lean reads one dword of each 64-byte line of LeanStep");

ILM_DEV void lean_unit_slot(const LeanStep& a, int seg, unsigned lane, int& first, int& row, int& x0, float& fx, float& fy) {
    first = seg * 64;
    row = first >> a.cs_shift;
    x0 = first - (row << a.cs_shift);
    fx = (float)(x0 + (int)lane); fy = (float)row;
}

ILM_DEV bool same_bits(float a, float b) { return __builtin_bit_cast(uint32_t, a) == __builtin_bit_cast(uint32_t, b); }
template <bool STREAM>
ILM_DEV void st_plane_changed(const UnitPlanes& u, int c, unsigned lane4, float v, float loaded) {
    if (!STREAM || __ballot(!same_bits(v, loaded)) != 0ull) st_plane<STREAM>(u, c, lane4, v);
}
ILM_DEV bool same_curve_t(const IlmFloat4& rc, float v0, float v1, uint32_t code) {
    if ((code & 3u) == 0u) return true;
    const float t1 = t_for_coded_bezier(rc, v1, code);
    return same_bits(t_for_coded_bezier(rc, v0, code), t1) && (t1 == t1);
}
template <bool SPAWN, bool STREAM>
ILM_DEV void store_changed_render_planes(const LeanStep& a, const UnitPlanes& up, unsigned lane4, float fx, float fy, const SlotIn& cur,
                                         float4 pos, float4 vel, float4 attr, bool spawned) {
    const float4 zero = mk4(0.0f, 0.0f, 0.0f, 0.0f);
    const IlmUpdateParams& p = a.update;
    const uint32_t codes = a.bezier_codes;
    const bool live0 = !(cur.life <= 0.0f), live1 = !(pos.w <= 0.0f);
    const bool dead = !live0 && !live1, both = live0 && live1;
    float4 rc, rd;
    render_data(fx, fy, pos, vel, zero, a.sys, p, codes, a.update_bits, nullptr, 0, 0, rc, rd);
    float speed0 = 0.0f, speed1 = 0.0f;
    if ((codes & 0x03000300u) != 0u) {
        speed0 = fmaxf(len3_fast(mk3(cur.vx, cur.vy, cur.vz)), 0.0001f);
        speed1 = fmaxf(len3_fast(xyz(vel)), 0.0001f);
    }
    const bool same_v = same_bits(cur.vx, vel.x) && same_bits(cur.vy, vel.y) && same_bits(cur.vz, vel.z);
    const bool rc_same = dead || (both && !spawned && ((a.elide & kElideColor) != 0u) && same_curve_t(p.ColorFromLife.RangeAndCount, cur.life, pos.w, codes & 0xFFu) &&
                                  same_curve_t(p.ColorFromVelocity.RangeAndCount, speed0, speed1, (codes >> 8) & 0xFFu));
    const bool rdx_same = dead || (both && same_curve_t(p.SizeFromLife.RangeAndCount, cur.life, pos.w, (codes >> 16) & 0xFFu) &&
                                   same_curve_t(p.SizeFromVelocity.RangeAndCount, speed0, speed1, codes >> 24) && (rd.x == rd.x));
    bool rdy_same = dead;
    if (a.update_bits & 2u) {
        const float y0 = render_rotation(rotation_unscaled(cur.vx, cur.vy), cur.life, render_index(fx, fy), a.sys, p);
        rdy_same = rdy_same || (both && same_bits(y0, rd.y) && (rd.y == rd.y));
    }
    const bool rdz_same = dead || (both && same_v);
    const bool rdw_same = dead || (both && same_bits(cur.ct, vel.w) && (vel.w == vel.w));
    if (__ballot(!rc_same) != 0ull) {
        const float4 stored = load_attributes<STREAM>(up, lane4);
        if (!SPAWN || !spawned) attr = stored;
        float4 rd_unused;
        render_data(fx, fy, pos, vel, attr, a.sys, p, codes, a.update_bits, nullptr, 0, 0, rc, rd_unused);
        store_render_color<STREAM>(up, lane4, rc);
    }
    if (__ballot(!rdx_same) != 0ull) st_plane<STREAM>(up, 16, lane4, rd.x);
    if (__ballot(!rdy_same) != 0ull) st_plane<STREAM>(up, 17, lane4, rd.y);
    if (__ballot(!rdz_same) != 0ull) st_plane<STREAM>(up, 18, lane4, rd.z);
    if (__ballot(!rdw_same) != 0ull) st_plane<STREAM>(up, 19, lane4, rd.w);
}

constexpr int kCurvesGeneral = 0, kCurvesClamp = 1;
constexpr uint32_t kClampCodes = 0x13131313u;

struct CurveT { float t1; bool same; };
ILM_DEV CurveT clamp_curve_t(const IlmFloat4& rc, float v0, float v1, uint32_t code) {
    CurveT c = { 0.0f, true };
    if ((code & 3u) != 0u) {
        c.t1 = t_for_clamp_bezier(rc, v1, code);
        c.same = same_bits(t_for_clamp_bezier(rc, v0, code), c.t1) && (c.t1 == c.t1);
    }
    return c;
}
ILM_DEV void store_changed_render_planes_clamp(const LeanStep& a, const UnitPlanes& up, unsigned lane4, float fx, float fy, const SlotIn& cur,
                                               float4 pos, float4 vel) {
    const IlmUpdateParams& p = a.update;
    const uint32_t codes = a.bezier_codes & kClampCodes;
    const uint32_t c_cl = codes & 0xFFu, c_cv = (codes >> 8) & 0xFFu, c_sl = (codes >> 16) & 0xFFu, c_sv = codes >> 24;
    const bool live0 = !(cur.life <= 0.0f), live1 = !(pos.w <= 0.0f);
    const bool dead = !live0 && !live1, both = live0 && live1;
    const float index = render_index(fx, fy);
    const float speed1 = fmaxf(len3_fast(xyz(vel)), 0.0001f);
    float speed0 = 0.0f;
    if ((codes & 0x03000300u) != 0u)
        speed0 = fmaxf(len3_fast(mk3(cur.vx, cur.vy, cur.vz)), 0.0001f);
    const CurveT cl = clamp_curve_t(p.ColorFromLife.RangeAndCount, cur.life, pos.w, c_cl);
    const CurveT cv = clamp_curve_t(p.ColorFromVelocity.RangeAndCount, speed0, speed1, c_cv);
    const CurveT sl = clamp_curve_t(p.SizeFromLife.RangeAndCount, cur.life, pos.w, c_sl);
    const CurveT sv = clamp_curve_t(p.SizeFromVelocity.RangeAndCount, speed0, speed1, c_sv);
    const float size_l = ((c_sl & 3u) == 0u) ? p.SizeFromLife.ABCD.x : bezier1_at(p.SizeFromLife, sl.t1, c_sl & 3u);
    const float size_v = ((c_sv & 3u) == 0u) ? p.SizeFromVelocity.ABCD.x : bezier1_at(p.SizeFromVelocity, sv.t1, c_sv & 3u);
    float4 rd;
    rd.x = live1 ? size_l * size_v : 0.0f;
    rd.y = live1 ? render_rotation(rotation_unscaled(vel.x, vel.y), pos.w, index, a.sys, p) : 0.0f;
    rd.z = live1 ? speed1 : 0.0f;
    rd.w = live1 ? vel.w : 0.0f;
    const float y0 = render_rotation(rotation_unscaled(cur.vx, cur.vy), cur.life, index, a.sys, p);
    const bool same_v = same_bits(cur.vx, vel.x) && same_bits(cur.vy, vel.y) && same_bits(cur.vz, vel.z);
    const bool rc_same = dead || (both && ((a.elide & kElideColor) != 0u) && cl.same && cv.same);
    const bool rdx_same = dead || (both && sl.same && sv.same && (rd.x == rd.x));
    const bool rdy_same = dead || (both && same_bits(y0, rd.y) && (rd.y == rd.y));
    const bool rdz_same = dead || (both && same_v);
    const bool rdw_same = dead || (both && same_bits(cur.ct, vel.w) && (vel.w == vel.w));
    if (__ballot(!rc_same) != 0ull) {
        const float4 attr = load_attributes<true>(up, lane4);
        const float4 color_l = ((c_cl & 3u) == 0u) ? ld4(p.ColorFromLife.A) : bezier4_at(p.ColorFromLife, cl.t1, c_cl & 3u);
        const float4 color_v = ((c_cv & 3u) == 0u) ? ld4(p.ColorFromVelocity.A) : bezier4_at(p.ColorFromVelocity, cv.t1, c_cv & 3u);
        float4 rc = mul4(attr, mul4(color_l, color_v));
        rc.w = sat(rc.w);
        rc.x *= rc.w; rc.y *= rc.w; rc.z *= rc.w;
        st_plane<true>(up, 12, lane4, live1 ? rc.x : 0.0f); st_plane<true>(up, 13, lane4, live1 ? rc.y : 0.0f);
        st_plane<true>(up, 14, lane4, live1 ? rc.z : 0.0f); st_plane<true>(up, 15, lane4, live1 ? rc.w : 0.0f);
    }
    if (__ballot(!rdx_same) != 0ull) st_plane<true>(up, 16, lane4, rd.x);
    if (__ballot(!rdy_same) != 0ull) st_plane<true>(up, 17, lane4, rd.y);
    if (__ballot(!rdz_same) != 0ull) st_plane<true>(up, 18, lane4, rd.z);
    if (__ballot(!rdw_same) != 0ull) st_plane<true>(up, 19, lane4, rd.w);
}

ILM_DEV uint64_t lane_mask(bool p) { return __builtin_amdgcn_ballot_w64(p); }
constexpr uint64_t kAllLanes = ~0ull;
constexpr int kBodySelecting = 0, kBodyRegular = 1;

ILM_DEV uint64_t regular_lanes_loaded(const LeanStep& a, const SlotIn& cur) {
    return lane_mask(cur.life > 0.0f) & lane_mask(cur.life < __builtin_inff()) & lane_mask(cur.ct >= a.regular_cat_lo) & lane_mask(cur.ct <= a.regular_cat_hi) &
           lane_mask(!__builtin_isunordered(cur.vx, cur.vy));
}
ILM_DEV uint64_t regular_lanes_updated(float new_life, float vx, float vy) {
    return lane_mask(new_life > 0.0f) & lane_mask(new_life < __builtin_inff()) & lane_mask(!__builtin_isunordered(vx, vy));
}
ILM_DEV uint64_t clamp_curve_changed(const IlmFloat4& rc, float v0, float v1, uint32_t code, float& t1) {
    t1 = 0.0f;
    if ((code & 3u) == 0u) return 0ull;
    t1 = t_for_clamp_bezier(rc, v1, code);
    return lane_mask(!same_bits(t_for_clamp_bezier(rc, v0, code), t1)) | lane_mask(t1 != t1);
}

ILM_DEV void store_changed_render_planes_regular(const LeanStep& a, const UnitPlanes& up, unsigned lane4, float fx, float fy, const SlotIn& cur,
                                                 float4 pos, float4 vel, uint64_t v_changed) {
    const IlmUpdateParams& p = a.update;
    const uint32_t codes = a.bezier_codes & kClampCodes;
    const uint32_t c_cl = codes & 0xFFu, c_cv = (codes >> 8) & 0xFFu, c_sl = (codes >> 16) & 0xFFu, c_sv = codes >> 24;
    const float speed1 = fmaxf(len3_fast(xyz(vel)), 0.0001f);
    float speed0 = 0.0f;
    if ((codes & 0x03000300u) != 0u)
        speed0 = fmaxf(len3_fast(mk3(cur.vx, cur.vy, cur.vz)), 0.0001f);
    float t_cl, t_cv, t_sl, t_sv;
    const uint64_t rc_changed = clamp_curve_changed(p.ColorFromLife.RangeAndCount, cur.life, pos.w, c_cl, t_cl) |
                                clamp_curve_changed(p.ColorFromVelocity.RangeAndCount, speed0, speed1, c_cv, t_cv);
    const uint64_t size_changed = clamp_curve_changed(p.SizeFromLife.RangeAndCount, cur.life, pos.w, c_sl, t_sl) |
                                  clamp_curve_changed(p.SizeFromVelocity.RangeAndCount, speed0, speed1, c_sv, t_sv);
    if (((a.elide & kElideColor) == 0u) || rc_changed != 0ull) {
        const float4 attr = load_attributes<true>(up, lane4);
        const float4 color_l = ((c_cl & 3u) == 0u) ? ld4(p.ColorFromLife.A) : bezier4_at(p.ColorFromLife, t_cl, c_cl & 3u);
        const float4 color_v = ((c_cv & 3u) == 0u) ? ld4(p.ColorFromVelocity.A) : bezier4_at(p.ColorFromVelocity, t_cv, c_cv & 3u);
        float4 rc = mul4(attr, mul4(color_l, color_v));
        rc.w = sat(rc.w);
        rc.x *= rc.w; rc.y *= rc.w; rc.z *= rc.w;
        st_plane<true>(up, 12, lane4, rc.x); st_plane<true>(up, 13, lane4, rc.y); st_plane<true>(up, 14, lane4, rc.z); st_plane<true>(up, 15, lane4, rc.w);
    }
    const float size_l = ((c_sl & 3u) == 0u) ? p.SizeFromLife.ABCD.x : bezier1_at(p.SizeFromLife, t_sl, c_sl & 3u);
    const float size_v = ((c_sv & 3u) == 0u) ? p.SizeFromVelocity.ABCD.x : bezier1_at(p.SizeFromVelocity, t_sv, c_sv & 3u);
    const float rdx = size_l * size_v;
    if ((size_changed | lane_mask(rdx != rdx)) != 0ull) st_plane<true>(up, 16, lane4, rdx);
    if ((a.elide & kElideRotation) == 0u) {
        const float index = render_index(fx, fy);
        const float rdy = render_rotation(0.0f, pos.w, index, a.sys, p);
        const float y0 = render_rotation(0.0f, cur.life, index, a.sys, p);
        if ((lane_mask(!same_bits(y0, rdy)) | lane_mask(rdy != rdy)) != 0ull) st_plane<true>(up, 17, lane4, rdy);
    }
    if (v_changed != 0ull) st_plane<true>(up, 18, lane4, speed1);
}


template <bool SPAWN, bool STREAM, int CURVES>
ILM_DEV void step_lean_block() {
    static_assert(CURVES == kCurvesGeneral || (STREAM && !SPAWN), "the curve classes are instantiations of the streaming variant without spawners");
    __shared__ uint32_t wave_live[kStepThreads / 64];
    const LeanStep& a = *(const LeanStep*)(CLeanStep*)__builtin_amdgcn_kernarg_segment_ptr();
    if (blockIdx.x < kTouchBlocks) touch_kernarg_lines_lean();
    const unsigned lane = threadIdx.x & 63u;
    const int wave = __builtin_amdgcn_readfirstlane((int)threadIdx.x >> 6);
    int v = (int)blockIdx.x * (kStepThreads / 64) + a.unit_rotate;
    if (v >= a.total_padded) v -= a.total_padded;
    const int u = v + wave;
    uint32_t n_live = 0;
    if (u < a.total_units) {
        const int chunk_rel = u >> a.upc_shift;
        const int seg = u - (chunk_rel << a.upc_shift);
        const int chunk = a.first_chunk + chunk_rel;
        bool untouched = false;
        if (a.partial_count != 0) {
#pragma unroll
            for (int k = 0; k < kMaxPartialChunks; k++)
                untouched = untouched || ((a.partial_chunk[k] == chunk) && (seg >= a.partial_units[k]));
        }
        if (!untouched) {
            const unsigned lane4 = lane * 4u;
            const UnitPlanes up = unit_planes(((CBase*)a.chunk_bases)[chunk], a.stride, seg * 64);
            const bool elide = STREAM && ((CURVES == kCurvesClamp) || (a.elide & kElideDerived) != 0u);
            SlotIn cur = load_slot<false, STREAM>(up, lane4);
            if (!elide) {
                const float4 stored = load_attributes<STREAM>(up, lane4);
                cur.ar = stored.x; cur.ag = stored.y; cur.ab = stored.z; cur.aa = stored.w;
            }
            int first, row, x0; float fx, fy;
            lean_unit_slot(a, seg, lane, first, row, x0, fx, fy);
            NoiseDeltas noise;
            noise.valid = false;
            if (a.noise_op >= 0)
                noise = noise_prepare(a.noise, a.noise_big, x0, row);

            float4 pos = mk4(cur.px, cur.py, cur.pz, cur.life);
            float4 vel = mk4(cur.vx, cur.vy, cur.vz, cur.ct);
            float4 attr = mk4(cur.ar, cur.ag, cur.ab, cur.aa);
            bool spawn_here = false, spawned = false;
            if constexpr (SPAWN) {
                for (int s = 0; s < a.spawn_count; s++) {
                    if (a.spawn_chunk[s] == chunk && seg >= a.spawn_unit_lo[s] && seg <= a.spawn_unit_hi[s]) {
                        const IlmSpawnRecord& r = a.spawns[s];
                        const float fi = (float)(first + (int)lane);
                        if (fi >= r.Params.ChunkSizeAndIndices[1] && fi <= r.Params.ChunkSizeAndIndices[2]) {
                            spawn_here = true;
                            if (spawn_slot(pos, vel, attr, fx, fy, a.rnd, a.rw, a.rh, a.inv_rw, a.inv_rh, r.Params))
                                spawned = true;
                        }
                    }
                }
            }
            const bool process = !(cur.life <= 0.0f) || spawn_here;
            const float4 zero = mk4(0.0f, 0.0f, 0.0f, 0.0f);
            float4 rc = zero, rd = zero;
            if constexpr (CURVES == kCurvesClamp) {
                int body = kBodySelecting;
                if (regular_lanes_loaded(a, cur) == kAllLanes) {
                    body = kBodyRegular;
#pragma unroll
                    for (int o = 0; o < ILM_MAX_OPS; o++) {
                        if (body == kBodyRegular && o < a.op_count) {
                            const int type = a.op_type[o];
                            if (type == ILM_OP_GRAVITY) {
                                apply_gravity_lean<false>(pos, vel, a.op[o].gravity, a.sys.GlobalSettings.x, a.sys.GlobalSettings.z);
                            } else if (type == ILM_OP_NOISE) {
                                apply_noise<false, false>(pos, vel, fx, fy, a.rnd, a.rw, a.rh, a.sys, a.op[o].noise, a.inv_rw, a.inv_rh, a.dop[o],
                                                          (o == a.noise_op) ? noise : NoiseDeltas{ false, zero, zero });
                            } else {
                                apply_fma<false, false>(pos, vel, a.sys, a.op[o].fma, a.dop[o]);
                                if ((lane_mask(pos.w <= 0.0f) | lane_mask(!same_bits(vel.w, cur.ct))) != 0ull) body = kBodySelecting;
                            }
                        }
                    }
                }
                if (body == kBodyRegular) {
                    update_positions_unselected(pos, vel, a.sys, a.dt_s);
                    const bool stays = regular_lanes_updated(pos.w, vel.x, vel.y) == kAllLanes;
                    if (__builtin_amdgcn_readfirstlane(*(CInt32*)&g_step_count_regular_waves) != 0 && lane == 0u)
                        atomicAdd(&g_step_regular_waves[stays ? 0 : 1], 1ull);
                    if (stays) {
                        const uint64_t vx_changed = lane_mask(!same_bits(vel.x, cur.vx)), vy_changed = lane_mask(!same_bits(vel.y, cur.vy)), vz_changed = lane_mask(!same_bits(vel.z, cur.vz));
                        if (lane_mask(!same_bits(pos.x, cur.px)) != 0ull) st_plane<true>(up, 0, lane4, pos.x);
                        if (lane_mask(!same_bits(pos.y, cur.py)) != 0ull) st_plane<true>(up, 1, lane4, pos.y);
                        if (lane_mask(!same_bits(pos.z, cur.pz)) != 0ull) st_plane<true>(up, 2, lane4, pos.z);
                        if (lane_mask(!same_bits(pos.w, cur.life)) != 0ull) st_plane<true>(up, 3, lane4, pos.w);
                        if (vx_changed != 0ull) st_plane<true>(up, 4, lane4, vel.x);
                        if (vy_changed != 0ull) st_plane<true>(up, 5, lane4, vel.y);
                        if (vz_changed != 0ull) st_plane<true>(up, 6, lane4, vel.z);
                        store_changed_render_planes_regular(a, up, lane4, fx, fy, cur, pos, vel, vx_changed | vy_changed | vz_changed);
                        n_live = 64u;
                        goto unit_stored;
                    }
                    const bool keep = !(pos.w <= 0.0f);
                    pos = mk4(keep ? pos.x : 0.0f, keep ? pos.y : 0.0f, keep ? pos.z : 0.0f, keep ? pos.w : 0.0f);
                    vel = mk4(keep ? vel.x : 0.0f, keep ? vel.y : 0.0f, keep ? vel.z : 0.0f, keep ? vel.w : 0.0f);
                }
                if (body == kBodySelecting) {
                    pos = mk4(cur.px, cur.py, cur.pz, cur.life);
                    vel = mk4(cur.vx, cur.vy, cur.vz, cur.ct);
                    if (__ballot(process) != 0ull) {
#pragma unroll
                        for (int o = 0; o < ILM_MAX_OPS; o++) {
                            if (o < a.op_count) {
                                const int type = a.op_type[o];
                                if (type == ILM_OP_GRAVITY)
                                    apply_gravity_lean(pos, vel, a.op[o].gravity, a.sys.GlobalSettings.x, a.sys.GlobalSettings.z);
                                else if (type == ILM_OP_NOISE)
                                    apply_noise<true, false>(pos, vel, fx, fy, a.rnd, a.rw, a.rh, a.sys, a.op[o].noise, a.inv_rw, a.inv_rh, a.dop[o],
                                                             (o == a.noise_op) ? noise : NoiseDeltas{ false, zero, zero });
                                else
                                    apply_fma<true, false>(pos, vel, a.sys, a.op[o].fma, a.dop[o]);
                            }
                        }
                        update_positions_select(pos, vel, a.sys, a.dt_s, process && !(pos.w <= 0.0f));
                    } else {
                        pos = vel = zero;
                    }
                }
            } else if (__ballot(process) != 0ull) {
                if (process) {
                    for (int o = 0; o < a.op_count; o++) {
                        const int type = a.op_type[o];
                        if (type == ILM_OP_GRAVITY)
                            apply_gravity_lean(pos, vel, a.op[o].gravity, a.sys.GlobalSettings.x, a.sys.GlobalSettings.z);
                        else if (type == ILM_OP_NOISE)
                            apply_noise(pos, vel, fx, fy, a.rnd, a.rw, a.rh, a.sys, a.op[o].noise, a.inv_rw, a.inv_rh, a.dop[o],
                                        (o == a.noise_op) ? noise : NoiseDeltas{ false, zero, zero });
                        else
                            apply_fma(pos, vel, a.sys, a.op[o].fma, a.dop[o]);
                    }
                    if (pos.w <= 0.0f) {
                        pos = vel = zero;
                    } else {
                        update_positions(pos, vel, a.sys, a.dt_s);
                        if (!elide)
                            render_data(fx, fy, pos, vel, attr, a.sys, a.update, a.bezier_codes, a.update_bits, nullptr, 0, 0, rc, rd);
                    }
                } else {
                    pos = vel = zero;
                }
            } else {
                pos = vel = zero;
            }
            st_plane_changed<STREAM>(up, 0, lane4, pos.x, cur.px); st_plane_changed<STREAM>(up, 1, lane4, pos.y, cur.py);
            st_plane_changed<STREAM>(up, 2, lane4, pos.z, cur.pz); st_plane_changed<STREAM>(up, 3, lane4, pos.w, cur.life);
            st_plane_changed<STREAM>(up, 4, lane4, vel.x, cur.vx); st_plane_changed<STREAM>(up, 5, lane4, vel.y, cur.vy);
            st_plane_changed<STREAM>(up, 6, lane4, vel.z, cur.vz); st_plane_changed<STREAM>(up, 7, lane4, vel.w, cur.ct);
            if constexpr (SPAWN) {
                if (spawned)
                    store_attributes<STREAM>(up, lane4, attr);
            }
            if (!elide) {
                store_render<STREAM>(up, lane4, rc, rd);
            } else if constexpr (CURVES == kCurvesClamp) {
                store_changed_render_planes_clamp(a, up, lane4, fx, fy, cur, pos, vel);
            } else {
                store_changed_render_planes<SPAWN, STREAM>(a, up, lane4, fx, fy, cur, pos, vel, attr, spawned);
            }
            n_live = (uint32_t)__popcll(__ballot(pos.w > 0.0f));
        unit_stored: __attribute__((unused));
        }
    }
    if (a.flags & ILM_STEP_COUNT_LIVE)
        publish_block_count(wave_live, n_live, lane, wave, v < a.total_units, a.first_chunk + (v >> a.upc_shift),
                            (v & ((1 << a.upc_shift) - 1)) / (kStepThreads / 64), (1 << a.upc_shift) / (kStepThreads / 64), a.count_buckets,
                            a.live_counts, a.zero_counts, a.zero_n, a.host_counts, a.count_seq);
}

template <bool SPAWN, bool STREAM>
__global__ __launch_bounds__(kStepThreads) void step_lean_kernel(const LeanStep a_) { step_lean_block<SPAWN, STREAM, kCurvesGeneral>(); }
__global__ __launch_bounds__(kStepThreads) void step_lean_clamp_kernel(const LeanStep a_) { step_lean_block<false, true, kCurvesClamp>(); }

struct LeanStepDf {
    LeanStep base;
    IlmDistanceFieldUniforms df;
    SdfView sdf;
};
static_assert(sizeof(LeanStepDf) <= 4096, "LeanStepDf travels in the kernarg segment (4 KB)");
static_assert(sizeof(LeanStepDf) > 0xd40 && sizeof(LeanStepDf) <= 0xe00, "touch_kernarg_lines_lean_df reads one dword of each 64-byte line of LeanStepDf");
ILM_DEV void touch_kernarg_lines_lean_df() {
// ... 237 lines not shown
            if (g.AttractorCount > kLeanMaxAttractors) return false;
            LeanGravity& l = f.op[o].gravity;
            l.count = g.AttractorCount < 0 ? 0 : g.AttractorCount;
            l.max_accel = a.derived.op[o].max_accel;
            l.cat_lo = g.CategoryFilter[0]; l.cat_hi = g.CategoryFilter[1];
            l.types = 0;
            for (int i = 0; i < l.count; i++) {
                l.a[i].x = g.AttractorPositions[i][0]; l.a[i].y = g.AttractorPositions[i][1]; l.a[i].z = g.AttractorPositions[i][2];
                l.a[i].radius = g.AttractorRadiusesAndStrengths[i][0];
                l.a[i].strength = g.AttractorRadiusesAndStrengths[i][1];
                const float type = g.AttractorRadiusesAndStrengths[i][2];
                l.types |= ((type >= 1.5f) ? 2u : ((type >= 0.5f) ? 1u : 0u)) << (2 * i);
            }
        } else if (op.Type == ILM_OP_NOISE) {
            if (!a.derived.op[o].area_none || a.derived.noise.op != o) return false;
            f.op[o].noise = op.u.Noise;
        } else {
            if (!a.derived.op[o].area_none) return false;
            f.op[o].fma = op.u.FMA;
        }
    }
    float cat_lo = -INFINITY, cat_hi = INFINITY;
    for (int o = 0; o < d.OpCount; o++) {
        const IlmTransformOp& op = d.Ops[o];
        const float* mm = (op.Type == ILM_OP_GRAVITY) ? op.u.Gravity.CategoryFilter : (op.Type == ILM_OP_NOISE) ? op.u.Noise.Area.CategoryFilter : op.u.FMA.Area.CategoryFilter;
        if (std::isnan(mm[0]) || std::isnan(mm[1])) cat_lo = NAN;
        cat_lo = (mm[0] > cat_lo) ? mm[0] : cat_lo;
        cat_hi = (mm[1] < cat_hi) ? mm[1] : cat_hi;
    }
    f.regular_cat_lo = cat_lo; f.regular_cat_hi = cat_hi;
    f.elide = (d.Update.RotationFromLifeAndIndex[0] == 0.0f && std::isfinite(d.Update.RotationFromLifeAndIndex[1]) && (a.derived.update_bits & 2u)) ? kElideRotation : 0u;
    f.op_count = d.OpCount;
    f.noise_op = a.derived.noise.op;
    f.noise = a.derived.noise;
    f.spawn_count = 0;
    for (int s = 0; s < ILM_MAX_SPAWNS; s++) { f.spawn_chunk[s] = -1; f.spawn_unit_lo[s] = 1; f.spawn_unit_hi[s] = 0; }
    for (int s = 0; s < d.SpawnCount; s++) {
        const IlmSpawnRecord& r = d.Spawns[s];
        if (r.Kind != ILM_SPAWN_INLINE) return false;
        f.spawns[s] = r;
        f.spawn_chunk[s] = r.ChunkIndex;
        const float first = r.Params.ChunkSizeAndIndices[1], last = r.Params.ChunkSizeAndIndices[2];
        if (last >= first && last >= 0.0f) {
            const double lo = first < 0.0f ? 0.0 : std::floor((double)first), hi = std::floor((double)last);
            const double max_unit = (double)(a.units_per_chunk - 1);
            f.spawn_unit_lo[s] = (int32_t)std::fmin(lo / 64.0, max_unit + 1.0);
            f.spawn_unit_hi[s] = (int32_t)std::fmin(hi / 64.0, max_unit);
        }
        f.spawn_count = s + 1;
    }
    if (d.SpawnCount == 0 && a.derived.noise.op >= 0 && a.derived.noise.classes == kNoiseBigClasses)
        memcpy(f.noise_big, &d.Spawns[0], sizeof(f.noise_big));
    f.chunk_bases = a.chunk_bases;
    f.live_counts = a.live_counts; f.zero_counts = a.zero_counts; f.zero_n = a.zero_n; f.host_counts = a.host_counts; f.count_seq = a.count_seq; f.count_buckets = a.count_buckets;
    f.stride = a.stride;
    f.upc_shift = a.upc_shift; f.unit_rotate = a.unit_rotate; f.total_padded = a.total_padded; f.total_units = a.unit_end - a.unit_begin;
    f.first_chunk = a.first_chunk; f.cs_shift = a.derived.cs_shift; f.flags = d.Flags;
    f.partial_count = a.partial_count;
    for (int k = 0; k < kMaxPartialChunks; k++) {
        f.partial_chunk[k] = (k < a.partial_count) ? a.partial_chunk[k] : -1;
        f.partial_units[k] = (k < a.partial_count) ? a.partial_units[k] : 0;
    }
    f.dt_s = a.derived.dt_s; f.bezier_codes = a.derived.bezier_codes; f.update_bits = a.derived.update_bits;
    f.sys = d.System; f.update = d.Update;
    f.rnd = a.rnd; f.rw = a.rw; f.rh = a.rh; f.inv_rw = a.derived.inv_rw; f.inv_rh = a.derived.inv_rh;
    return true;
}

static bool color_curves_bounded(const IlmUpdateParams& u) {
    for (const IlmClampedBezier4* b : { &u.ColorFromLife, &u.ColorFromVelocity })
        for (const IlmFloat4* q : { &b->A, &b->B, &b->C, &b->D })
            for (const float x : { q->x, q->y, q->z, q->w })
                if (!(std::fabs(x) <= 0x1p60f)) return false;
    return true;
}

static std::atomic<int> g_last_step_kernel{ILM_STEP_KERNEL_NONE};
int last_step_kernel() { return g_last_step_kernel; }

static bool curves_clamp(const LeanStep& f, bool spawning, bool streaming) {
    return streaming && !spawning && (f.elide & kElideDerived) != 0u && (f.bezier_codes & ~kClampCodes) == 0u && f.update_bits == 2u;
}

static hipError_t launch_lean_step(const LeanStep& f, bool spawning, bool streaming, hipStream_t stream) {
    const int units_per_block = kStepThreads / 64;
    const dim3 grid((unsigned)((f.total_units + units_per_block - 1) / units_per_block), 1, 1), block(kStepThreads, 1, 1);
    const bool clamp = curves_clamp(f, spawning, streaming);
    if (spawning) {
        if (streaming) hipLaunchKernelGGL((step_lean_kernel<true, true>), grid, block, 0, stream, f);
        else hipLaunchKernelGGL((step_lean_kernel<true, false>), grid, block, 0, stream, f);
    } else {
        if (clamp) hipLaunchKernelGGL(step_lean_clamp_kernel, grid, block, 0, stream, f);
        else if (streaming) hipLaunchKernelGGL((step_lean_kernel<false, true>), grid, block, 0, stream, f);
        else hipLaunchKernelGGL((step_lean_kernel<false, false>), grid, block, 0, stream, f);
    }
    g_last_step_kernel = clamp ? ILM_STEP_KERNEL_LEAN_CLAMP : ILM_STEP_KERNEL_LEAN;
    return hipGetLastError();
}

constexpr int kFieldSlice0 = 2;
constexpr int kFieldCells0 = 4;
static_assert((ILM_SDF_UNORM16 | ILM_SDF_FP16) == 1, "the format is bit 0 of the collision kernels' first template argument");
static bool field_is_slice0(const IlmDistanceFieldUniforms& df, int format) {
    return (format == ILM_SDF_UNORM16) && (df.Packed1.y == 0.0f) && std::isfinite(df.Packed1.x) && std::isfinite(df.Packed1.z) &&
           std::isfinite(df.TextureSliceAndTexelSize.x) && std::isfinite(df.TextureSliceAndTexelSize.y);
}
template <bool CELLS, class Launch>
static hipError_t with_field_format(const StepLaunch& a, Launch launch) {
    int fmt = (int)a.sdf.format | (field_is_slice0(a.desc.DistanceField, (int)a.sdf.format) ? kFieldSlice0 : 0);
    if (CELLS && fmt == (ILM_SDF_UNORM16 | kFieldSlice0) && a.sdf.cells0 != nullptr) fmt |= kFieldCells0;
    switch (fmt) {
        case ILM_SDF_UNORM16: return launch(std::integral_constant<int, ILM_SDF_UNORM16>());
        case ILM_SDF_FP16: return launch(std::integral_constant<int, ILM_SDF_FP16>());
        case ILM_SDF_UNORM16 | kFieldSlice0: return launch(std::integral_constant<int, ILM_SDF_UNORM16 | kFieldSlice0>());
        case ILM_SDF_FP16 | kFieldSlice0: return launch(std::integral_constant<int, ILM_SDF_FP16 | kFieldSlice0>());
        case ILM_SDF_UNORM16 | kFieldSlice0 | kFieldCells0:
            if constexpr (CELLS) return launch(std::integral_constant<int, ILM_SDF_UNORM16 | kFieldSlice0 | kFieldCells0>());
    }
    return hipErrorInvalidValue;
}
struct BlockLayout { int total_padded, unit_rotate, count_buckets; };
static BlockLayout block_layout(int total_units, int unit_rotate, int units_per_chunk, int upb) {
    BlockLayout l;
    l.total_padded = (total_units + upb - 1) / upb * upb;
    l.unit_rotate = unit_rotate / upb * upb;
    l.count_buckets = 1;
    while (l.count_buckets * 2 <= kCountLines - 1 && (units_per_chunk / upb) % (l.count_buckets * 2) == 0) l.count_buckets *= 2;
    return l;
}
__global__ __launch_bounds__(256) void build_slice0_cells_kernel(const uint2* __restrict__ texels, int width, int height, uint2* __restrict__ cells) {
    const int x0 = (int)blockIdx.x * 256 + (int)threadIdx.x, yr = (int)blockIdx.y;
    if (x0 >= width) return;
    const int yi = yr - 1;
    const int y0 = min(max(yi, 0), height - 1);
    const int y1 = ((uint32_t)yi < (uint32_t)(height - 1)) ? y0 + 1 : y0;
    const int x1 = (x0 + 1 == width) ? 0 : x0 + 1;
    const uint32_t r00 = texels[(size_t)y0 * width + x0].x & 0xFFFFu, r10 = texels[(size_t)y0 * width + x1].x & 0xFFFFu;
    const uint32_t r01 = texels[(size_t)y1 * width + x0].x & 0xFFFFu, r11 = texels[(size_t)y1 * width + x1].x & 0xFFFFu;
    cells[(size_t)yr * width + x0] = make_uint2(r00 | (r10 << 16), r01 | (r11 << 16));
}
hipError_t launch_build_slice0_cells(const uint2* texels, int width, int height, void* cells, hipStream_t stream) {
    hipLaunchKernelGGL(build_slice0_cells_kernel, dim3((unsigned)((width + 255) / 256), (unsigned)(height + 1)), dim3(256), 0, stream, texels, width, height, static_cast<uint2*>(cells));
    return hipGetLastError();
}
static bool step_interpreter_forced();
bool step_wants_slice0_cells(const IlmStepDesc& d, int format) {
    const char* e = getenv("ILM_DF_CELLS0");
    if (e && atoi(e) == 0) return false;
    const char* lean = getenv("ILM_DF_LEAN");
    if ((lean && atoi(lean) == 0) || step_interpreter_forced()) return false;
    if (!(d.UpdateMode == ILM_UPDATE_WITH_DISTANCE_FIELD && format == ILM_SDF_UNORM16 && field_is_slice0(d.DistanceField, format))) return false;
    const float ey = d.DistanceField.Extent.y, tw = d.DistanceField.TextureSliceAndTexelSize.w;
    const float v_max = ey * tw;
    return std::isfinite(ey) && std::isfinite(tw) && std::isfinite(v_max) && ey >= 0.0f && tw >= 0.0f && v_max <= 1.0f;
}

template <int FMT, bool SPAWN>
static hipError_t launch_lean_df_variant(const LeanStepDf& f, int k, bool streaming, const dim3& grid, hipStream_t stream) {
    const dim3 block(kStepThreads, 1, 1);
    if (streaming) hipLaunchKernelGGL((step_lean_df_kernel<FMT, SPAWN, true, 4>), grid, block, 0, stream, f);
    else if (k == 4) hipLaunchKernelGGL((step_lean_df_kernel<FMT, SPAWN, false, 4>), grid, block, 0, stream, f);
    else if (k == 2) hipLaunchKernelGGL((step_lean_df_kernel<FMT, SPAWN, false, 2>), grid, block, 0, stream, f);
    else hipLaunchKernelGGL((step_lean_df_kernel<FMT, SPAWN, false, 1>), grid, block, 0, stream, f);
    return hipGetLastError();
}
static hipError_t launch_lean_df_step(LeanStepDf& f, const StepLaunch& a, bool spawning, hipStream_t stream) {
// ... 3 lines not shown
    int k = (forced_k == 1 || forced_k == 2 || forced_k == 4) ? forced_k : ((f.base.total_units >= 65536) ? 4 : 2);
    if (streaming) k = 4;
    const int upb = (kStepThreads / 64) * k;
    const BlockLayout l = block_layout(f.base.total_units, f.base.unit_rotate, a.units_per_chunk, upb);
    f.base.total_padded = l.total_padded; f.base.unit_rotate = l.unit_rotate; f.base.count_buckets = l.count_buckets;
    const dim3 grid((unsigned)(l.total_padded / upb), 1, 1);
    return with_field_format<true>(a, [&](auto fmt) {
        return spawning ? launch_lean_df_variant<decltype(fmt)::value, true>(f, k, streaming, grid, stream) : launch_lean_df_variant<decltype(fmt)::value, false>(f, k, streaming, grid, stream);
    });
}

static bool needs_extended_variant(const StepLaunch& a) {
    if (a.op_mask & ((1u << ILM_OP_MATRIX_MULTIPLY) | (1u << ILM_OP_SPATIAL_NOISE))) return true;
    for (int s = 0; s < a.desc.SpawnCount; s++)
        if (a.desc.Spawns[s].Kind != ILM_SPAWN_INLINE) return true;
    return false;
}

constexpr int kDfMinWaves = 6;
template <bool SPAWN>
static hipError_t launch_step_variant(const StepLaunch& a, hipStream_t stream) {
    const int units = a.unit_end - a.unit_begin;
    if (units <= 0) return hipSuccess;
    const int units_per_block = kStepThreads / 64;
    const dim3 grid((unsigned)((units + units_per_block - 1) / units_per_block), 1, 1), block(kStepThreads, 1, 1);
    const bool df = a.desc.UpdateMode == ILM_UPDATE_WITH_DISTANCE_FIELD;
    if (needs_extended_variant(a)) {
        if (df)
            return with_field_format<false>(a, [&](auto fmt) {
                hipLaunchKernelGGL((step_kernel<decltype(fmt)::value, true, true, 1, true>), grid, block, 0, stream, a);
                return hipGetLastError();
            });
        hipLaunchKernelGGL((step_kernel<ILM_SDF_UNORM16, false, true, 1, true>), grid, block, 0, stream, a);
    } else if (df) {
        return with_field_format<false>(a, [&](auto fmt) {
            hipLaunchKernelGGL((step_kernel<decltype(fmt)::value, true, SPAWN, kDfMinWaves>), grid, block, 0, stream, a);
            return hipGetLastError();
        });
    } else if (a.streaming) {
        hipLaunchKernelGGL((step_kernel<ILM_SDF_UNORM16, false, SPAWN, 1, false, true>), grid, block, 0, stream, a);
    } else {
        hipLaunchKernelGGL((step_kernel<ILM_SDF_UNORM16, false, SPAWN, 1>), grid, block, 0, stream, a);
    }
    return hipGetLastError();
}

static std::atomic<int> g_step_interpreter{-1};
static bool step_interpreter_forced() {
    if (g_step_interpreter < 0) {
        const char* e = getenv("ILM_STEP_LEAN");
        g_step_interpreter = (e && atoi(e) == 0) ? 1 : 0;
    }
    return g_step_interpreter != 0;
}
int set_step_interpreter(int on) {
    const int before = step_interpreter_forced() ? 1 : 0;
    g_step_interpreter = on ? 1 : 0;
    return before;
}

static bool layout_step(StepLaunch& a) {
    a.units_per_chunk = a.span / 64;
    a.upc_shift = -1;
    for (int b = 0; b < 31; b++)
        if ((1 << b) == a.units_per_chunk) a.upc_shift = b;
    a.unit_begin = 0;
    a.unit_end = a.chunk_count * a.units_per_chunk;
    int first_spawn_unit = 0;
    bool spawning = false;
    for (int s = 0; s < a.desc.SpawnCount; s++) {
        const IlmSpawnRecord& r = a.desc.Spawns[s];
        if (r.ChunkIndex < a.first_chunk || r.ChunkIndex >= a.first_chunk + a.chunk_count)
            continue;
        if (r.Params.ChunkSizeAndIndices[2] < r.Params.ChunkSizeAndIndices[1])
            continue;
        if (!spawning)
            first_spawn_unit = (r.ChunkIndex - a.first_chunk) * a.units_per_chunk + (int)r.Params.ChunkSizeAndIndices[1] / 64;
        spawning = true;
    }
    const BlockLayout l = block_layout(a.unit_end, first_spawn_unit, a.units_per_chunk, kStepThreads / 64);
    a.total_padded = l.total_padded; a.unit_rotate = l.unit_rotate; a.count_buckets = l.count_buckets;
    return spawning;
}
hipError_t launch_step(StepLaunch& a, hipStream_t stream, uint32_t render_elide, bool* refreshed) {
    if (refreshed) *refreshed = false;
    const bool spawning = layout_step(a);
    if (!step_interpreter_forced() && a.unit_end > a.unit_begin) {
        if (a.desc.UpdateMode == ILM_UPDATE_WITH_DISTANCE_FIELD) {
            const char* lean_env = getenv("ILM_DF_LEAN");
            const bool lean_df = !(lean_env && atoi(lean_env) == 0);
            LeanStepDf f;
            if (lean_df && build_lean_step(a, f.base)) {
                f.df = a.desc.DistanceField;
                f.sdf = a.sdf;
                g_last_step_kernel = ILM_STEP_KERNEL_LEAN_DF;
                return launch_lean_df_step(f, a, spawning, stream);
            }
        } else {
            LeanStep f;
            if (build_lean_step(a, f)) {
                f.elide = ((render_elide & kElideDerived) && a.streaming) ? (kElideDerived | (color_curves_bounded(a.desc.Update) ? kElideColor : 0u) | (f.elide & kElideRotation)) : 0u;
                const hipError_t e = launch_lean_step(f, spawning, a.streaming != 0, stream);
                if (refreshed) *refreshed = (e == hipSuccess);
                return e;
            }
        }
    }
    g_last_step_kernel = ILM_STEP_KERNEL_INTERPRETER;
    return spawning ? launch_step_variant<true>(a, stream) : launch_step_variant<false>(a, stream);
}

int step_batch_layout(StepLaunch& a, int* blocks) {
    const bool spawning = layout_step(a);
    const int units = a.unit_end - a.unit_begin;
    *blocks = (units + kStepThreads / 64 - 1) / (kStepThreads / 64);
    if (a.streaming || units <= 0) return -1;
    int field = 0;
    if (a.desc.UpdateMode == ILM_UPDATE_WITH_DISTANCE_FIELD) {
        if (with_field_format<false>(a, [&](auto fmt) { field = 1 + decltype(fmt)::value; return hipSuccess; }) != hipSuccess) return -1;
    }
    return (field << 2) | (needs_extended_variant(a) ? 2 : (spawning ? 1 : 0));
}
template <int FMT, bool DF>
static hipError_t launch_step_batch_variant(int kind, const StepBatchItem* table, const int32_t* item_of_block, const dim3& grid, hipStream_t stream) {
    const dim3 block(kStepThreads, 1, 1);
    constexpr int kMinWaves = DF ? kDfMinWaves : 1;
    if (kind == 2) hipLaunchKernelGGL((step_batch_kernel<FMT, DF, true, 1, true>), grid, block, 0, stream, table, item_of_block);
    else if (kind == 1) hipLaunchKernelGGL((step_batch_kernel<FMT, DF, true, kMinWaves>), grid, block, 0, stream, table, item_of_block);
    else hipLaunchKernelGGL((step_batch_kernel<FMT, DF, false, kMinWaves>), grid, block, 0, stream, table, item_of_block);
    return hipGetLastError();
}
hipError_t launch_step_batch(int variant, const StepBatchItem* table, const int32_t* item_of_block, int blocks, hipStream_t stream) {
    if (blocks <= 0) return hipSuccess;
    const dim3 grid((unsigned)blocks, 1, 1);
    const int kind = variant & 3;
    g_last_step_kernel = ILM_STEP_KERNEL_BATCH;
    switch (variant >> 2) {
        case 0: return launch_step_batch_variant<ILM_SDF_UNORM16, false>(kind, table, item_of_block, grid, stream);
        case 1 + ILM_SDF_UNORM16: return launch_step_batch_variant<ILM_SDF_UNORM16, true>(kind, table, item_of_block, grid, stream);
        case 1 + ILM_SDF_FP16: return launch_step_batch_variant<ILM_SDF_FP16, true>(kind, table, item_of_block, grid, stream);
        case 1 + (ILM_SDF_UNORM16 | kFieldSlice0): return launch_step_batch_variant<ILM_SDF_UNORM16 | kFieldSlice0, true>(kind, table, item_of_block, grid, stream);
        case 1 + (ILM_SDF_FP16 | kFieldSlice0): return launch_step_batch_variant<ILM_SDF_FP16 | kFieldSlice0, true>(kind, table, item_of_block, grid, stream);
    }
    return hipErrorInvalidValue;
}

__global__ __launch_bounds__(256) void aos_to_soa_kernel(const float4* __restrict__ src, float* __restrict__ plane0, int64_t stride,
                                                          int first_slot, int count) {
    const int i = (int)blockIdx.x * 256 + (int)threadIdx.x;
    if (i >= count) return;
    const float4 v = src[i];
    float* p = plane0 + first_slot + i;
    p[0] = v.x; p[stride] = v.y; p[2 * stride] = v.z; p[3 * stride] = v.w;
}
__global__ __launch_bounds__(256) void soa_to_aos_kernel(const float* __restrict__ plane0, int64_t stride, float4* __restrict__ dst,
                                                          int first_slot, int count) {
    const int i = (int)blockIdx.x * 256 + (int)threadIdx.x;
    if (i >= count) return;
    const float* p = plane0 + first_slot + i;
    dst[i] = mk4(p[0], p[stride], p[2 * stride], p[3 * stride]);
}
hipError_t launch_aos_to_soa(const float4* src, float* plane0, int64_t stride, int32_t first_slot, int32_t count, hipStream_t stream) {
    if (count <= 0) return hipSuccess;
    hipLaunchKernelGGL(aos_to_soa_kernel, dim3((count + 255) / 256), dim3(256), 0, stream, src, plane0, stride, first_slot, count);
    return hipGetLastError();
}
hipError_t launch_soa_to_aos(const float* plane0, int64_t stride, float4* dst, int32_t first_slot, int32_t count, hipStream_t stream) {
    if (count <= 0) return hipSuccess;
    hipLaunchKernelGGL(soa_to_aos_kernel, dim3((count + 255) / 256), dim3(256), 0, stream, plane0, stride, dst, first_slot, count);
    return hipGetLastError();
}

__global__ __launch_bounds__(256) void count_live_kernel(float* const* __restrict__ bases, int64_t stride, int slots, uint32_t* __restrict__ counts) {
    __shared__ uint32_t wave_live[4];
    const int chunk = (int)blockIdx.y;
    const float* life = bases[chunk] + 3 * stride;
    const int i0 = ((int)blockIdx.x * 256 + (int)threadIdx.x) * 4;
    const float4 l = *reinterpret_cast<const float4*>(life + i0);
    const uint32_t n = (uint32_t)__popcll(__ballot((i0 < slots) && (l.x > 0.0f))) + (uint32_t)__popcll(__ballot((i0 + 1 < slots) && (l.y > 0.0f))) +
                       (uint32_t)__popcll(__ballot((i0 + 2 < slots) && (l.z > 0.0f))) + (uint32_t)__popcll(__ballot((i0 + 3 < slots) && (l.w > 0.0f)));
    if ((threadIdx.x & 63) == 0) wave_live[threadIdx.x >> 6] = n;
    __syncthreads();
    if (threadIdx.x == 0) {
        const uint32_t total = wave_live[0] + wave_live[1] + wave_live[2] + wave_live[3];
        if (total != 0) atomicAdd(&counts[chunk * kCountStride], total);
    }
}
hipError_t launch_count_live(float* const* chunk_bases, int64_t stride, int32_t span, int32_t slots, int32_t chunk_count, uint32_t* counts, hipStream_t stream) {
    if (chunk_count <= 0) return hipSuccess;
    hipLaunchKernelGGL(count_live_kernel, dim3((unsigned)(span / 1024), (unsigned)chunk_count), dim3(256), 0, stream, chunk_bases, stride, slots, counts);
// ... 60 lines not shown
    if ((int)threadIdx.x < a.sensor_count) {
        const int k = (int)threadIdx.x;
        const uint32_t total = wave_counts[0][k] + wave_counts[1][k] + wave_counts[2][k] + wave_counts[3][k];
        if (total != 0u) atomicAdd(&a.counts[((size_t)k * (size_t)a.chunk_count + (size_t)chunk) * kSenseStride], total);
    }
}
hipError_t launch_sense(SenseLaunch& a, hipStream_t stream) {
    if (a.chunk_count <= 0 || a.sensor_count <= 0) return hipSuccess;
    if (a.chunk_count > 65535 || a.sensor_count > ILM_MAX_SENSORS) return hipErrorInvalidValue;
    bool area = false;
    for (int k = 0; k < a.sensor_count; k++) area = area || (a.sensors[k].AreaType != 0);
    const int tiles = a.span / 1024;
    const long long total_tiles = (long long)tiles * a.chunk_count;
    a.tiles_per_block = (int)std::min<long long>(8, std::max<long long>(1, total_tiles / 2048));
    const dim3 grid((unsigned)((tiles + a.tiles_per_block - 1) / a.tiles_per_block), (unsigned)a.chunk_count);
    if (area) hipLaunchKernelGGL(sense_kernel<true>, grid, dim3(256), 0, stream, a);
    else hipLaunchKernelGGL(sense_kernel<false>, grid, dim3(256), 0, stream, a);
    return hipGetLastError();
}

__global__ __launch_bounds__(1024) void live_slots_count_kernel(const float* __restrict__ life, int slots, uint32_t* __restrict__ block_counts) {
    __shared__ uint32_t wave_counts[16];
    const int lane = (int)threadIdx.x & 63, wave = (int)threadIdx.x >> 6;
    const int i = (int)blockIdx.x * 1024 + (int)threadIdx.x;
    const bool alive = (i < slots) && (life[i] > 0.0f);
    const unsigned long long mask = __ballot(alive);
    if (lane == 0) wave_counts[wave] = (uint32_t)__popcll(mask);
    __syncthreads();
    if (threadIdx.x == 0) {
        uint32_t t = 0;
        for (int w = 0; w < 16; w++) t += wave_counts[w];
        block_counts[blockIdx.x] = t;
    }
}
__global__ __launch_bounds__(1024) void live_slots_emit_kernel(const float* __restrict__ life, int slots, const uint32_t* __restrict__ block_counts,
                                                                uint32_t* __restrict__ out, uint32_t capacity, uint32_t* __restrict__ out_count) {
    __shared__ uint32_t wave_counts[16];
    __shared__ uint32_t partial[16];
    const int lane = (int)threadIdx.x & 63, wave = (int)threadIdx.x >> 6;
    uint32_t before = 0;
    for (int b = (int)threadIdx.x; b < (int)blockIdx.x; b += 1024) before += block_counts[b];
    for (int off = 32; off > 0; off >>= 1) before += __shfl_down(before, off);
    if (lane == 0) partial[wave] = before;
    const int i = (int)blockIdx.x * 1024 + (int)threadIdx.x;
    const bool alive = (i < slots) && (life[i] > 0.0f);
    const unsigned long long mask = __ballot(alive);
    const uint32_t prefix = (uint32_t)__popcll(mask & ((1ull << lane) - 1ull));
    if (lane == 0) wave_counts[wave] = (uint32_t)__popcll(mask);
    __syncthreads();
    uint32_t base = 0;
    for (int w = 0; w < 16; w++) base += partial[w];
    uint32_t wave_base = base;
    for (int w = 0; w < wave; w++) wave_base += wave_counts[w];
    if (alive) {
        const uint32_t dst = wave_base + prefix;
        if (dst < capacity) out[dst] = (uint32_t)i;
    }
    if ((blockIdx.x == gridDim.x - 1) && (threadIdx.x == 0)) {
        uint32_t t = base;
        for (int w = 0; w < 16; w++) t += wave_counts[w];
        *out_count = t;
    }
}
hipError_t launch_live_slots(const float* life, int32_t slots, uint32_t* out_slots, uint32_t capacity, uint32_t* out_count, uint32_t* block_counts, hipStream_t stream) {
    const unsigned blocks = (unsigned)((slots + 1023) / 1024);
    if (blocks == 0) return hipMemsetAsync(out_count, 0, sizeof(uint32_t), stream);
    hipLaunchKernelGGL(live_slots_count_kernel, dim3(blocks), dim3(1024), 0, stream, life, slots, block_counts);
    hipLaunchKernelGGL(live_slots_emit_kernel, dim3(blocks), dim3(1024), 0, stream, life, slots, block_counts, out_slots, capacity, out_count);
    return hipGetLastError();
}

hipError_t step_sdf_sample_counter(int enable, unsigned long long* out) {
    unsigned long long value = 0, zero = 0;
    hipError_t e = hipMemcpyFromSymbol(&value, HIP_SYMBOL(g_step_sdf_samples), sizeof(value));
    if (e != hipSuccess) return e;
    e = hipMemcpyToSymbol(HIP_SYMBOL(g_step_sdf_samples), &zero, sizeof(zero));
    if (e != hipSuccess) return e;
    const int flag = enable ? 1 : 0;
    e = hipMemcpyToSymbol(HIP_SYMBOL(g_step_count_sdf_samples), &flag, sizeof(flag));
    if (out) *out = value;
    return e;
}

hipError_t step_regular_wave_counter(int enable, unsigned long long out[2]) {
    unsigned long long value[2] = { 0, 0 }, zero[2] = { 0, 0 };
    hipError_t e = hipMemcpyFromSymbol(value, HIP_SYMBOL(g_step_regular_waves), sizeof(value));
    if (e != hipSuccess) return e;
    e = hipMemcpyToSymbol(HIP_SYMBOL(g_step_regular_waves), zero, sizeof(zero));
    if (e != hipSuccess) return e;
    const int flag = enable ? 1 : 0;
    e = hipMemcpyToSymbol(HIP_SYMBOL(g_step_count_regular_waves), &flag, sizeof(flag));
    if (out) { out[0] = value[0]; out[1] = value[1]; }
    return e;
}

}
```

illuminant_amd/native.py:

```python
import ctypes as C
import os

import numpy as np

from . import abi

_HERE = os.path.dirname(os.path.abspath(__file__))
LIB_PATH = os.environ.get("ILM_HIP_LIB") or os.path.join(_HERE, "lib", "libilluminant_hip.so")

_lib = None


class IlluminantError(RuntimeError):
    def __init__(self, code, message):
        super().__init__("illuminant_hip error %d: %s" % (code, message))
        self.code = code


_H = abi.Handle
_P = C.c_void_p
_I = C.c_int32
SYMBOLS = {
    "ilm_abi_version": (_I, []),
    "ilm_last_error": (C.c_char_p, []),
    "ilm_device_count": (_I, []),
    "ilm_debug_reference_constant": (_I, [C.c_char_p, C.POINTER(C.c_double)]),
    "ilm_debug_reference_constant_count": (_I, []),
    "ilm_debug_reference_constant_key": (C.c_char_p, [_I]),
    "ilm_ctx_create": (_I, [_I, C.POINTER(_H)]),
    "ilm_ctx_create_sibling": (_I, [_H, C.POINTER(_H)]),
    "ilm_ctx_destroy": (_I, [_H]),
    "ilm_ctx_sync": (_I, [_H]),
    "ilm_ctx_stream": (_I, [_H, C.POINTER(_P)]),
    "ilm_timer_start": (_I, [_H]),
    "ilm_timer_stop": (_I, [_H, C.POINTER(C.c_float)]),
    "ilm_engine_create": (_I, [_H, _I, _P, _I, _I, C.POINTER(_H)]),
    "ilm_engine_destroy": (_I, [_H]),
    "ilm_system_create": (_I, [_H, C.POINTER(_H)]),
    "ilm_system_destroy": (_I, [_H]),
    "ilm_system_add_chunk": (_I, [_H, C.POINTER(_I)]),
    "ilm_system_remove_chunk": (_I, [_H, _I]),
    "ilm_system_chunk_count": (_I, [_H, C.POINTER(_I)]),
    "ilm_chunk_upload": (_I, [_H, _I, _I, _P, _I, _I]),
    "ilm_chunk_download": (_I, [_H, _I, _I, _P, _I, _I]),
    "ilm_chunk_device_ptr": (_I, [_H, _I, _I, C.POINTER(_P), C.POINTER(C.c_int64)]),
    "ilm_system_set_distance_field": (_I, [_H, _H]),
    "ilm_system_set_life_ramp": (_I, [_H, _P, _I, _I]),
    "ilm_system_step": (_I, [_H, _P]),
    "ilm_engine_step_batch": (_I, [_H, _P, _P, _I]),
    "ilm_debug_last_step_batch": (_I, [_H, C.POINTER(_I), C.POINTER(_I), C.POINTER(_I)]),
    "ilm_spawn": (_I, [_H, _I, _P, _P]),
    "ilm_gravity": (_I, [_H, _I, _P, _P]),
    "ilm_noise": (_I, [_H, _I, _P, _P]),
    "ilm_fma": (_I, [_H, _I, _P, _P]),
    "ilm_matrix_multiply": (_I, [_H, _I, _P, _P]),
    "ilm_spatial_noise": (_I, [_H, _I, _P, _P]),
    "ilm_system_set_spawn_positions": (_I, [_H, _I, _P, _I]),
    "ilm_system_set_spawn_pattern": (_I, [_H, _I, _P, _I, _I, _I]),
    "ilm_update": (_I, [_H, _I, _P, _P, _P]),
    "ilm_erase": (_I, [_H, _I]),
    "ilm_system_live_counts": (_I, [_H, _P, _I, _I]),
    "ilm_system_step_counts": (_I, [_H, _P, _I, _I]),
    "ilm_system_poll_counts": (_I, [_H, _P, _I, _I, C.POINTER(_I)]),
    "ilm_system_sense": (_I, [_H, _I, _I, _P, _I, _P, _I]),
    "ilm_system_sense_async": (_I, [_H, _I, _I, _P, _I]),
    "ilm_system_poll_sense": (_I, [_H, _P, _I, C.POINTER(_I)]),
    "ilm_chunk_live_slots": (_I, [_H, _I, _P, _I, C.POINTER(_I)]),
    "ilm_sdf_create": (_I, [_H, _I, _I, _I, C.POINTER(_H)]),
    "ilm_sdf_upload": (_I, [_H, _P]),
    "ilm_sdf_sample": (_I, [_H, _P, _P, _I, _P]),
    "ilm_debug_sdf_sample_inside": (_I, [_H, _P, _P, _I, _P, _P]),
    "ilm_debug_divide": (_I, [_H, _P, _P, _I, _P, _P]),
    "ilm_debug_step_interpreter": (_I, [_I]),
    "ilm_debug_last_step_kernel": (_I, []),
    "ilm_debug_step_streams": (_I, [_I]),
    "ilm_debug_step_sdf_samples": (_I, [_H, _I, C.POINTER(C.c_uint64)]),
    "ilm_debug_step_regular_waves": (_I, [_H, _I, C.POINTER(C.c_uint64), C.POINTER(C.c_uint64)]),
    "ilm_debug_last_light_launch": (_I, [_H, C.POINTER(C.c_int32), C.POINTER(C.c_int32), C.POINTER(C.c_int32)]),
    "ilm_debug_divide_by_constants": (_I, [_H, _P, _P, _I, C.POINTER(_I)]),
    "ilm_sdf_destroy": (_I, [_H]),
    "ilm_sdf_download": (_I, [_H, _P]),
    "ilm_sdf_device_ptr": (_I, [_H, C.POINTER(_P)]),
    "ilm_sdf_mark_dirty": (_I, [_H, _I, _I]),
    "ilm_sdf_trace_info": (_I, [_H, C.POINTER(abi.SdfTraceInfo)]),
    "ilm_sdf_set_filter": (_I, [_H, _I]),
    "ilm_sdf_get_filter": (_I, [_H, C.POINTER(_I)]),
    "ilm_sdf_render_slices": (_I, [_H, _H, _P, _P, _I, _P, _I, _P, _I, _P, _I]),
    "ilm_gbuffer_create": (_I, [_H, _I, _I, _I, C.POINTER(_H)]),
    "ilm_gbuffer_upload": (_I, [_H, _P]),
    "ilm_gbuffer_destroy": (_I, [_H]),
    "ilm_gbuffer_download": (_I, [_H, _P]),
    "ilm_gbuffer_render": (_I, [_H, _P, _P, _I, _P, _I]),
    "ilm_gbuffer_render_meshes": (_I, [_H, _P, _P, _I, _P, _I, _P, _I, _P, _I]),
    "ilm_lightmap_create": (_I, [_H, _I, _I, _I, _P, C.POINTER(_H)]),
    "ilm_lightmap_download": (_I, [_H, _P, _I, _I]),
    "ilm_lightmap_device_ptr": (_I, [_H, C.POINTER(_P)]),
    "ilm_lightmap_destroy": (_I, [_H]),
    "ilm_render_sphere_lights": (_I, [_H, _P, _I, _P, _P, _H, _H, _P, _H, _I, _I, _P]),
    "ilm_render_directional_lights": (_I, [_H, _P, _I, _P, _P, _H, _H, _P, _H, _I, _I, _P]),
    "ilm_render_line_lights": (_I, [_H, _P, _I, _P, _P, _H, _H, _P, _H, _I, _I, _P]),
    "ilm_render_volumetric_lights": (_I, [_H, _P, _I, _P, _P, _H, _H, _P, _H, _I, _I, _P]),
    "ilm_render_projector_lights": (_I, [_H, _P, _I, _P, _P, _H, _H, _P, _H, _I, _I, _P]),
    "ilm_render_particle_lights": (_I, [_H, _H, _P, _I, _P, _P, _P, _H, _H, _H, _I, _I, _P]),
    "ilm_render_light_probes": (_I, [_H, _P, _I, _P, _P, _I, _P, _P, _H, _P]),
    "ilm_render_directional_light_probes": (_I, [_H, _P, _I, _P, _P, _I, _P, _P, _H, _P]),
    "ilm_render_line_light_probes": (_I, [_H, _P, _I, _P, _P, _I, _P, _P, _H, _P]),
    "ilm_system_readback": (_I, [_H, _P, _I, _P, _P, _I, C.POINTER(_I)]),
    "ilm_system_readback_view": (_I, [_H, _P, _I, _P, C.POINTER(_P), C.POINTER(_I)]),
    "ilm_render_particles": (_I, [_H, _P, _I, _P, _H, _P]),
    "ilm_engine_render_particles_batch": (_I, [_H, _P, _I, _H, _P]),
    "ilm_debug_last_render_batch": (_I, [_H, C.POINTER(_I), C.POINTER(_I), C.POINTER(_I)]),
    "ilm_lightmap_clear": (_I, [_H, _P]),
    "ilm_ctx_set_light_ramp": (_I, [_H, _P, _I, _I]),
    "ilm_ctx_set_projector_texture": (_I, [_H, _P, _I, _I]),
    "ilm_ctx_set_projector_texture_mips": (_I, [_H, _P, _I, _I, _I]),
    "ilm_ctx_set_lightmap_blend": (_I, [_H, _I]),
    "ilm_ctx_set_light_blend_function": (_I, [_H, _I, _I]),
    "ilm_ctx_set_light_split": (_I, [_H, _I]),
    "ilm_system_set_bitmap": (_I, [_H, _P, _I, _I]),
    "ilm_resolve_lighting": (_I, [_H, _H, _P, _I, _I]),
    "ilm_resolve_lighting_with_albedo": (_I, [_H, _H, _H, _P, _I, _I]),
    "ilm_resolve_lighting_scaled": (_I, [_H, _H, _H, _P, _P, _P, _P, _P, _I, _I, _I, _I]),
    "ilm_resolve_lighting_lut": (_I, [_H, _H, _H, _P, _P, _P, _P, _P, _P, _I, _I, _I, _I]),
    "ilm_lightmap_upload": (_I, [_H, _P, _I, _I]),
    "ilm_lightmap_luminance": (_I, [_H, _I, _I, _I, _P, _I, C.POINTER(_I), C.POINTER(_I), C.POINTER(_I)]),
    "ilm_lightmap_histogram": (_I, [_H, _P, _P, _P, _P]),
    "ilm_debug_queue_luminance": (_I, [_H, _I, _I, _I]),
    "ilm_visualize_distance_field": (_I, [_H, _H, _P, _P, _P, _H, _P]),
    "ilm_group_create": (_I, [_P, _I, C.POINTER(_H)]),
    "ilm_group_unique_id": (_I, [_P]),
    "ilm_group_create_rank": (_I, [_I, _I, _I, _P, C.POINTER(_H)]),
    "ilm_group_destroy": (_I, [_H]),
    "ilm_group_info": (_I, [_H, C.POINTER(_I), C.POINTER(_I), C.POINTER(_I), C.POINTER(_I)]),
    "ilm_group_ctx": (_I, [_H, _I, C.POINTER(_H)]),
    "ilm_group_sync": (_I, [_H]),
    "ilm_group_all_gather": (_I, [_H, _P, C.c_uint64, _I]),
    "ilm_group_host_all_gather": (_I, [_H, _P, _P, C.c_uint32]),
    "ilm_group_lightmap_create": (_I, [_H, _I, _I, _I, C.POINTER(_H)]),
    "ilm_group_lightmap_member": (_I, [_H, _I, C.POINTER(_H)]),
    "ilm_group_lightmap_strip": (_I, [_H, _I, C.POINTER(_I), C.POINTER(_I), C.POINTER(_I)]),
    "ilm_group_lightmap_set_strips": (_I, [_H, C.POINTER(C.c_int32), C.POINTER(C.c_int32)]),
    "ilm_group_lightmap_gather": (_I, [_H, _I]),
    "ilm_group_lightmap_store_mode": (_I, [_H, _I]),
    "ilm_group_lightmap_wait": (_I, [_H]),
    "ilm_group_lightmap_destroy": (_I, [_H]),
    "ilm_group_render_sphere_lights": (_I, [_H, _P, _I, _P, _P, _P, _P, _P, _H, _I, _P]),
    "ilm_group_live_counts": (_I, [_H, _P, _I, _P, _I, _I]),
    "ilm_group_gather_chunks": (_I, [_H, _P, _P, _I, _I, _I, _I]),
}


def lib():
    global _lib
    if _lib is None:
        if not os.path.exists(LIB_PATH):
            raise IlluminantError(abi.ERR_NO_DEVICE, "%s not built: run `python -c 'import __graft_entry__ as g; g.build()'` "
                                  "(there is no CPU fallback)" % LIB_PATH)
        handle = C.CDLL(LIB_PATH)
        for name, (res, args) in SYMBOLS.items():
            fn = getattr(handle, name)
# ... 856 lines not shown
```

include/illuminant_hip.h:

```cpp
#ifndef ILLUMINANT_HIP_H
#define ILLUMINANT_HIP_H

#include <stdint.h>

#ifdef __cplusplus
extern "C" {
#endif

#define ILM_ABI_VERSION 11

#define ILM_OK                    0
#define ILM_ERR_INVALID_ARGUMENT  (-1)
#define ILM_ERR_INVALID_HANDLE    (-2)
#define ILM_ERR_OUT_OF_RANGE      (-3)
#define ILM_ERR_TOO_MANY          (-4)
#define ILM_ERR_NO_DEVICE         (-5)
#define ILM_ERR_STATE             (-6)

typedef uint64_t IlmHandle;


typedef struct IlmFloat4 { float x, y, z, w; } IlmFloat4;

typedef struct IlmMatrix { float m[16]; } IlmMatrix;
// ... 234 lines not shown

int32_t ilm_timer_start(IlmHandle ctx);
int32_t ilm_timer_stop(IlmHandle ctx, float* out_ms);


#define ILM_RANDOMNESS_WIDTH  807
#define ILM_RANDOMNESS_HEIGHT 653
int32_t ilm_engine_create(IlmHandle ctx, int32_t chunk_size,
                          const IlmFloat4* randomness, int32_t rand_width, int32_t rand_height,
                          IlmHandle* out_engine);
int32_t ilm_engine_destroy(IlmHandle engine);

int32_t ilm_system_create(IlmHandle engine, IlmHandle* out_system);
int32_t ilm_system_destroy(IlmHandle system);
int32_t ilm_system_add_chunk(IlmHandle system, int32_t* out_chunk_index);
int32_t ilm_system_remove_chunk(IlmHandle system, int32_t chunk_index);
int32_t ilm_system_chunk_count(IlmHandle system, int32_t* out_count);

int32_t ilm_chunk_upload(IlmHandle system, int32_t chunk_index, int32_t plane,
                         const IlmFloat4* src, int32_t first_slot, int32_t count);
int32_t ilm_chunk_download(IlmHandle system, int32_t chunk_index, int32_t plane,
                           IlmFloat4* dst, int32_t first_slot, int32_t count);
int32_t ilm_chunk_device_ptr(IlmHandle system, int32_t chunk_index, int32_t component,
                             void** out_ptr, int64_t* out_stride_floats);

int32_t ilm_system_set_distance_field(IlmHandle system, IlmHandle sdf);
int32_t ilm_system_set_life_ramp(IlmHandle system, const IlmFloat4* texels, int32_t width, int32_t height);

int32_t ilm_system_set_spawn_positions(IlmHandle system, int32_t spawn_slot, const IlmFloat4* positions, int32_t count);

int32_t ilm_system_set_spawn_pattern(IlmHandle system, int32_t spawn_slot, const IlmFloat4* texels,
                                     int32_t width, int32_t height, int32_t levels);

int32_t ilm_system_step(IlmHandle system, const IlmStepDesc* desc);

int32_t ilm_engine_step_batch(IlmHandle engine, const IlmHandle* systems, const IlmStepDesc* descs, int32_t count);
int32_t ilm_debug_last_step_batch(IlmHandle engine, int32_t* out_launches, int32_t* out_rounds, int32_t* out_fallback_items);

int32_t ilm_spawn  (IlmHandle system, int32_t chunk_index, const IlmParticleSystemUniforms* sys, const IlmSpawnParams* p);
int32_t ilm_gravity(IlmHandle system, int32_t chunk_index, const IlmParticleSystemUniforms* sys, const IlmGravityParams* p);
int32_t ilm_noise  (IlmHandle system, int32_t chunk_index, const IlmParticleSystemUniforms* sys, const IlmNoiseParams* p);
int32_t ilm_fma    (IlmHandle system, int32_t chunk_index, const IlmParticleSystemUniforms* sys, const IlmFMAParams* p);
int32_t ilm_matrix_multiply(IlmHandle system, int32_t chunk_index, const IlmParticleSystemUniforms* sys, const IlmMatrixMultiplyParams* p);
int32_t ilm_spatial_noise  (IlmHandle system, int32_t chunk_index, const IlmParticleSystemUniforms* sys, const IlmSpatialNoiseParams* p);
int32_t ilm_update (IlmHandle system, int32_t chunk_index, const IlmParticleSystemUniforms* sys, const IlmUpdateParams* p,
                    const IlmDistanceFieldUniforms* df );
int32_t ilm_erase  (IlmHandle system, int32_t chunk_index);

int32_t ilm_system_live_counts(IlmHandle system, uint32_t* out_counts, int32_t capacity, int32_t saturate16);

int32_t ilm_system_step_counts(IlmHandle system, uint32_t* out_counts, int32_t capacity, int32_t saturate16);

int32_t ilm_system_poll_counts(IlmHandle system, uint32_t* out_counts, int32_t capacity, int32_t saturate16, int32_t* out_ready);

#define ILM_MAX_SENSORS 8
int32_t ilm_system_sense(IlmHandle system, int32_t first_chunk, int32_t chunk_count, const IlmAreaParams* sensors, int32_t sensor_count,
                         uint32_t* out_counts, int32_t capacity);
int32_t ilm_system_sense_async(IlmHandle system, int32_t first_chunk, int32_t chunk_count, const IlmAreaParams* sensors, int32_t sensor_count);
int32_t ilm_system_poll_sense(IlmHandle system, uint32_t* out_counts, int32_t capacity, int32_t* out_ready);

int32_t ilm_chunk_live_slots(IlmHandle system, int32_t chunk_index, uint32_t* out_slots, int32_t capacity, int32_t* out_count);


int32_t ilm_sdf_create(IlmHandle ctx, int32_t atlas_width, int32_t atlas_height, int32_t format, IlmHandle* out_sdf);
int32_t ilm_sdf_upload(IlmHandle sdf, const uint16_t* texels);
int32_t ilm_sdf_sample(IlmHandle sdf, const IlmDistanceFieldUniforms* df, const float* positions, int32_t count, float* out_distances);

int32_t ilm_debug_sdf_sample_inside(IlmHandle sdf, const IlmDistanceFieldUniforms* df, const float* positions, int32_t count,
                                    float* out_distances, int32_t* out_used_table);

int32_t ilm_debug_divide(IlmHandle ctx, const float* numerators, const float* denominators, int32_t count, float* out_fast, float* out_ieee);
int32_t ilm_debug_divide_by_constants(IlmHandle ctx, float* out_divisors, uint64_t* out_mismatches, int32_t capacity, int32_t* out_count);
int32_t ilm_debug_step_interpreter(int32_t interpreter);
#define ILM_STEP_KERNEL_NONE         0
#define ILM_STEP_KERNEL_INTERPRETER  1
#define ILM_STEP_KERNEL_LEAN         2
#define ILM_STEP_KERNEL_LEAN_CLAMP   3
#define ILM_STEP_KERNEL_LEAN_DF      4
#define ILM_STEP_KERNEL_BATCH        5
int32_t ilm_debug_last_step_kernel(void);
int32_t ilm_debug_step_streams(int32_t streams);
int32_t ilm_debug_step_sdf_samples(IlmHandle ctx, int32_t enable, uint64_t* out_samples);
int32_t ilm_debug_step_regular_waves(IlmHandle ctx, int32_t enable, uint64_t* out_regular, uint64_t* out_selected);
int32_t ilm_debug_last_light_launch(IlmHandle ctx, int32_t* out_workgroups, int32_t* out_split, int32_t* out_tile_macro);
int32_t ilm_sdf_destroy(IlmHandle sdf);
int32_t ilm_sdf_download(IlmHandle sdf, uint16_t* texels);
int32_t ilm_sdf_device_ptr(IlmHandle sdf, void** out_ptr);
int32_t ilm_sdf_mark_dirty(IlmHandle sdf, int32_t first_virtual_slice, int32_t slice_count);
typedef struct IlmSdfTraceInfo {
    uint64_t CellBytes;
    uint64_t CellRebuilds;
    uint64_t CellSlicesRebuilt;
    int32_t  LastRebuiltSlices;
    int32_t  TableSlices;
    int32_t  RebuiltEveryFrame;
    int32_t  Reserved;
} IlmSdfTraceInfo;
int32_t ilm_sdf_trace_info(IlmHandle sdf, IlmSdfTraceInfo* out);

#define ILM_SDF_FILTER_FP32    0
#define ILM_SDF_FILTER_FIXED8  8
int32_t ilm_sdf_set_filter(IlmHandle sdf, int32_t fraction_bits);
int32_t ilm_sdf_get_filter(IlmHandle sdf, int32_t* out_fraction_bits);


enum {
    ILM_OBSTRUCTION_ELLIPSOID = 0, ILM_OBSTRUCTION_BOX = 1, ILM_OBSTRUCTION_CYLINDER = 2,
    ILM_OBSTRUCTION_SPHEROID = 3, ILM_OBSTRUCTION_OCTAGON = 4
};
typedef struct IlmObstruction {
    float   Center[3];      int32_t Type;
    float   Size[3];        int32_t IsDynamic;
    float   Orientation[4];
} IlmObstruction;

typedef struct IlmHeightVolume {
    int32_t FirstVertex, VertexCount;
    float   ZBase, Height;
    int32_t IsDynamic;
    int32_t TopFaceEnableShadows;
    int32_t _pad[2];
} IlmHeightVolume;

#define ILM_DISTANCE_LIMIT 520.0f

typedef struct IlmDistanceFieldRenderDesc {
    int32_t VirtualWidth, VirtualHeight;
    float   VirtualDepth, ZOffset;
    int32_t SliceWidth, SliceHeight, SliceCount, ColumnCount;
    int32_t RowCount;
    float   MaximumEncodedDistance;
    float   InvScaleFactorX, InvScaleFactorY;
    int32_t DynamicFlagFilter;
    int32_t _pad[3];
} IlmDistanceFieldRenderDesc;

int32_t ilm_sdf_render_slices(IlmHandle sdf, IlmHandle clear_source, const IlmDistanceFieldRenderDesc* desc,
                              const int32_t* first_virtual_slices, int32_t triplet_count,
                              const IlmObstruction* obstructions, int32_t obstruction_count,
                              const IlmHeightVolume* volumes, int32_t volume_count,
                              const float* polygon_xy, int32_t polygon_vertex_count);

int32_t ilm_gbuffer_create(IlmHandle ctx, int32_t width, int32_t height, int32_t format, IlmHandle* out_gbuffer);
int32_t ilm_gbuffer_upload(IlmHandle gbuffer, const void* texels);
int32_t ilm_gbuffer_destroy(IlmHandle gbuffer);
int32_t ilm_gbuffer_download(IlmHandle gbuffer, void* texels);

typedef struct IlmGBufferRenderDesc {
    float   ViewportPosition[2];
    float   ViewportScale[2];
    float   GroundZ;
    int32_t RenderGroundPlane;
    int32_t EnableGroundShadows;
    int32_t _pad;
} IlmGBufferRenderDesc;

int32_t ilm_gbuffer_render(IlmHandle gbuffer, const IlmGBufferRenderDesc* desc,
                           const IlmHeightVolume* volumes, int32_t volume_count,
                           const float* polygon_xy, int32_t polygon_vertex_count);


typedef struct IlmHeightVolumeVertex {
    float Position[3];
    float Normal[3];
    float ZRange[2];
    float EnableShadows;
// ... 343 lines not shown
```

Measured before the change: 91470.

## Cache per-chunk category bounds to skip category plane loads in clamp step

Adds a per-chunk record of the min/max category value, filled by a new reduction kernel whenever a chunk's record is stale. The clamp-curves lean step checks the record, and when every particle in the chunk is provably inside the regular category range it skips loading the category plane, loading it later only if the wave leaves the regular path. Records are invalidated on uploads, pointer exposure, spawning, FMA ops and graph capture. The cost is extra scan launches and host bookkeeping for stale chunks, and one more scalar load per wave.

```diff
diff --git a/illuminant_amd/csrc/api.hip b/illuminant_amd/csrc/api.hip
--- a/illuminant_amd/csrc/api.hip
+++ b/illuminant_amd/csrc/api.hip
@@ -226,6 +226,8 @@
     std::vector<uint8_t> ptr_out;
     RenderKey render_key; uint64_t render_key_gen = 0;
     bool render_captured = false;
+    std::vector<uint8_t> cat_current;
+    DeviceScratch d_cat;
     DeviceScratch d_table; bool table_dirty = true;
     unsigned long long* d_counts = nullptr; int counts_cap = 0; int count_parity = 0;
     unsigned long long* counts_region(int r) const { return d_counts + (size_t)r * (size_t)counts_cap * kCountLines * kCountStride; }
@@ -551,6 +553,12 @@
         const int32_t rc = reserve(c, s->d_table, sizeof(float*) * (size_t)n, sizeof(float*) * (size_t)(n < 64 ? 64 : n * 2));
         if (rc != ILM_OK) return rc;
         s->table_dirty = true;
+    }
+    if (sizeof(float) * kCategoryRecordStride * (size_t)n > s->d_cat.bytes) {
+        const int32_t rc = reserve(c, s->d_cat, sizeof(float) * kCategoryRecordStride * (size_t)n, sizeof(float) * kCategoryRecordStride * (size_t)(n < 64 ? 64 : n * 2));
+        if (rc != ILM_OK) return rc;
+        HIP_TRY(hipMemsetAsync(s->d_cat.p, 0, s->d_cat.bytes, c->main()));
+        s->cat_current.assign(s->chunks.size(), 0);
     }
     if (n > s->counts_cap) {
         if (s->d_counts) { HIP_TRY(hipStreamSynchronize(c->main())); HIP_TRY(hipFree(s->d_counts)); s->d_counts = nullptr; }
@@ -1041,9 +1049,12 @@
     };
     const uint32_t elide_a = render_elide(first, (mid < 0) ? first + count : mid), elide_b = (mid < 0) ? 0u : render_elide(mid, first + count);
     render_refreshed(first, first + count, false);
+    CategoryRecords records = { s->d_cat.as<float>(), s->cat_current.data(), s->used.data() };
+    CategoryRecords* cat = &records;
+    if (s->render_captured) { s->cat_current.assign(s->chunks.size(), 0); cat = nullptr; }
     bool fresh_a = false, fresh_b = false;
     if (mid < 0) {
-        HIP_TRY(launch_step(a, c->main(), elide_a, &fresh_a));
+        HIP_TRY(launch_step(a, c->main(), elide_a, &fresh_a, cat));
         render_refreshed(first, first + count, fresh_a);
     } else {
         if (s->split_at != mid) { (void)c->main(); s->split_at = mid; }
@@ -1063,12 +1074,12 @@
         bool spawn_in_b = false;
         for (int k = 0; k < d->SpawnCount; k++) spawn_in_b = spawn_in_b || (d->Spawns[k].ChunkIndex >= mid);
         if (spawn_in_b) {
-            HIP_TRY(launch_step(b, c->aux, elide_b, &fresh_b));
+            HIP_TRY(launch_step(b, c->aux, elide_b, &fresh_b, cat));
             c->aux_pending = true;
-            HIP_TRY(launch_step(a, c->stream_, elide_a, &fresh_a));
+            HIP_TRY(launch_step(a, c->stream_, elide_a, &fresh_a, cat));
         } else {
-            HIP_TRY(launch_step(a, c->stream_, elide_a, &fresh_a));
-            HIP_TRY(launch_step(b, c->aux, elide_b, &fresh_b));
+            HIP_TRY(launch_step(a, c->stream_, elide_a, &fresh_a, cat));
+            HIP_TRY(launch_step(b, c->aux, elide_b, &fresh_b, cat));
             c->aux_pending = true;
         }
         render_refreshed(first, mid, fresh_a);
@@ -1147,7 +1158,7 @@
         if (n == 0) continue;
         if (d->UpdateMode == ILM_UPDATE_POSITIONS) (void)render_key_generation(s, d);
         if (capturing) s->render_captured = true;
-        for (int ci = first; ci < first + n; ci++) s->render_gen[(size_t)ci] = 0;
+        for (int ci = first; ci < first + n; ci++) s->render_gen[(size_t)ci] = s->cat_current[(size_t)ci] = 0;
         finish_step(s, d, first, n);
 
         Planned& p = plan[(size_t)i];
@@ -1293,6 +1304,7 @@
     if (written) {
         s->used[(size_t)chunk] = s->engine->slots;
         s->render_gen[(size_t)chunk] = 0;
+        s->cat_current[(size_t)chunk] = 0;
     }
     return ILM_OK;
 }
@@ -1611,7 +1623,7 @@
     (void)hipSetDevice(c->device);
     (void)hipStreamSynchronize(c->main());
     for (float* p : s->chunks) release_chunk(s->engine, p);
-    for (DeviceScratch* b : { &s->d_table, &s->d_slots, &s->d_slot_count }) release(*b);
+    for (DeviceScratch* b : { &s->d_table, &s->d_cat, &s->d_slots, &s->d_slot_count }) release(*b);
     for (DeviceScratch& b : s->spawn_positions) release(b);
     if (s->d_counts) (void)hipFree(s->d_counts);
     if (s->ramp) (void)hipFree(s->ramp);
@@ -1637,6 +1649,7 @@
     s->used.push_back(0);
     s->render_gen.push_back(0);
     s->ptr_out.push_back(0);
+    s->cat_current.push_back(0);
     s->table_dirty = true;
     if (out_index) *out_index = (int32_t)s->chunks.size() - 1;
     return ILM_OK;
@@ -1655,6 +1668,7 @@
     s->used.erase(s->used.begin() + index);
     s->render_gen.erase(s->render_gen.begin() + index);
     s->ptr_out.erase(s->ptr_out.begin() + index);
+    s->cat_current.assign(s->chunks.size(), 0);
     s->table_dirty = true;
     return ILM_OK;
 }
@@ -1691,6 +1705,7 @@
     HIP_TRY(hipMemcpyAsync(c->staging.p, src, bytes, hipMemcpyHostToDevice, c->main()));
     s->used[(size_t)chunk] = std::max(s->used[(size_t)chunk], first_slot + count);
     s->render_gen[(size_t)chunk] = 0;
+    s->cat_current[(size_t)chunk] = 0;
     HIP_TRY(launch_aos_to_soa(c->staging.as<const float4>(), s->chunks[(size_t)chunk] + (int64_t)plane * 4 * e->stride,
                               e->stride, first_slot, count, c->main()));
     HIP_TRY(hipStreamSynchronize(c->main()));
@@ -1724,6 +1739,7 @@
     if (out_ptr) *out_ptr = s->chunks[(size_t)chunk] + (int64_t)component * s->engine->stride;
     s->used[(size_t)chunk] = s->engine->slots;
     s->render_gen[(size_t)chunk] = 0;
+    s->cat_current[(size_t)chunk] = 0;
     s->ptr_out[(size_t)chunk] = 1;
     if (out_stride) *out_stride = s->engine->stride;
     return ILM_OK;
@@ -2295,6 +2311,35 @@
     HIP_TRY(step_regular_wave_counter(enable, value));
     if (out_regular) *out_regular = (uint64_t)value[0];
     if (out_selected) *out_selected = (uint64_t)value[1];
+    return ILM_OK;
+}
+
+int32_t ilm_debug_step_category_waves(IlmHandle hctx, int32_t enable, uint64_t* out_skipped, uint64_t* out_late, uint64_t* out_upfront) {
+    Ctx* c = from_handle<Ctx>(hctx, kMagicCtx);
+    if (!c) return fail(ILM_ERR_INVALID_HANDLE, "not a context handle");
+    HIP_TRY(hipSetDevice(c->device));
+    HIP_TRY(hipStreamSynchronize(c->main()));
+    unsigned long long value[3] = { 0, 0, 0 };
+    HIP_TRY(step_category_wave_counter(enable, value));
+    if (out_skipped) *out_skipped = (uint64_t)value[0];
+    if (out_late) *out_late = (uint64_t)value[1];
+    if (out_upfront) *out_upfront = (uint64_t)value[2];
+    return ILM_OK;
+}
+
+int32_t ilm_debug_chunk_category_bounds(IlmHandle hsystem, int32_t chunk, float* out_lo, float* out_hi, int32_t* out_current) {
+    System* s = from_handle<System>(hsystem, kMagicSystem);
+    if (!s) return fail(ILM_ERR_INVALID_HANDLE, "not a system handle");
+    if (chunk < 0 || chunk >= (int)s->chunks.size()) return fail(ILM_ERR_OUT_OF_RANGE, "chunk %d outside [0, %d)", chunk, (int)s->chunks.size());
+    Ctx* c = s->engine->ctx;
+    HIP_TRY(hipSetDevice(c->device));
+    HIP_TRY(hipStreamSynchronize(c->main()));
+    float bounds[2] = { 0.0f, 0.0f };
+    const bool held = sizeof(float) * kCategoryRecordStride * (size_t)(chunk + 1) <= s->d_cat.bytes;
+    if (held) HIP_TRY(hipMemcpy(bounds, s->d_cat.as<float>() + (size_t)chunk * kCategoryRecordStride, sizeof(bounds), hipMemcpyDeviceToHost));
+    if (out_lo) *out_lo = bounds[0];
+    if (out_hi) *out_hi = bounds[1];
+    if (out_current) *out_current = (held && s->cat_current[(size_t)chunk] && !s->render_captured && !s->ptr_out[(size_t)chunk]) ? 1 : 0;
     return ILM_OK;
 }
 
diff --git a/illuminant_amd/csrc/internal.hpp b/illuminant_amd/csrc/internal.hpp
--- a/illuminant_amd/csrc/internal.hpp
+++ b/illuminant_amd/csrc/internal.hpp
@@ -85,11 +85,14 @@
 constexpr uint32_t kElideDerived = 1u;
 constexpr uint32_t kElideColor = 2u;
 constexpr uint32_t kElideRotation = 4u;
-hipError_t launch_step(StepLaunch& a, hipStream_t stream, uint32_t render_elide = 0u, bool* refreshed = nullptr);
+constexpr int kCategoryRecordStride = 16;
+struct CategoryRecords { float* table; uint8_t* current; const int32_t* used; };
+hipError_t launch_step(StepLaunch& a, hipStream_t stream, uint32_t render_elide = 0u, bool* refreshed = nullptr, CategoryRecords* cat = nullptr);
 int step_batch_layout(StepLaunch& a, int* blocks);
 hipError_t launch_step_batch(int variant, const StepBatchItem* table, const int32_t* item_of_block, int blocks, hipStream_t stream);
 hipError_t step_sdf_sample_counter(int enable, unsigned long long* out);
 hipError_t step_regular_wave_counter(int enable, unsigned long long out[2]);
+hipError_t step_category_wave_counter(int enable, unsigned long long out[3]);
 bool step_wants_slice0_cells(const IlmStepDesc& d, int format);
 hipError_t launch_build_slice0_cells(const uint2* texels, int width, int height, void* cells, hipStream_t stream);
 int set_step_interpreter(int on);
diff --git a/illuminant_amd/csrc/particles.hip b/illuminant_amd/csrc/particles.hip
--- a/illuminant_amd/csrc/particles.hip
+++ b/illuminant_amd/csrc/particles.hip
@@ -641,6 +641,7 @@
 __device__ int g_step_count_sdf_samples;
 __device__ unsigned long long g_step_regular_waves[2];
 __device__ int g_step_count_regular_waves;
+__device__ unsigned long long g_step_category_waves[3];
 
 template <int FMT>
 ILM_DEV void df_long(float4& pos, float4& vel, float x, float y, float initial_distance, float step_distance0, bool first_done,
@@ -1102,14 +1103,15 @@
     int32_t partial_count, op_count, spawn_count; uint32_t elide;
     int32_t op_type[ILM_MAX_OPS];
     int32_t spawn_chunk[ILM_MAX_SPAWNS], spawn_unit_lo[ILM_MAX_SPAWNS], spawn_unit_hi[ILM_MAX_SPAWNS];
-    int32_t _pad1[2];
+    int32_t cat_stride, _pad1;
     float dt_s; uint32_t bezier_codes, update_bits; int32_t noise_op;
     IlmParticleSystemUniforms sys;
     IlmUpdateParams update;
     StepDerived::Op dop[ILM_MAX_OPS];
     LeanOp op[ILM_MAX_OPS];
     StepDerived::NoiseFast noise;
-    const float4* rnd; int32_t rw, rh; float inv_rw, inv_rh; int32_t _pad2[2];
+    const float4* rnd; int32_t rw, rh; float inv_rw, inv_rh;
+    const float* cat_bounds;
     union {
         IlmSpawnRecord spawns[ILM_MAX_SPAWNS];
         IlmFloat4 noise_big[2 * kNoiseBigClasses * kNoiseBigClasses];
@@ -1269,6 +1271,24 @@
     return lane_mask(cur.life > 0.0f) & lane_mask(cur.life < __builtin_inff()) & lane_mask(cur.ct >= a.regular_cat_lo) & lane_mask(cur.ct <= a.regular_cat_hi) &
            lane_mask(!__builtin_isunordered(cur.vx, cur.vy));
 }
+ILM_DEV uint64_t regular_lanes_loaded_proven(const SlotIn& cur) {
+    return lane_mask(cur.life > 0.0f) & lane_mask(cur.life < __builtin_inff()) & lane_mask(!__builtin_isunordered(cur.vx, cur.vy));
+}
+typedef const uint64_t __attribute__((address_space(4))) CUint64;
+__device__ __attribute__((aligned(8))) float g_no_category_record[2] = { __builtin_nanf(""), __builtin_nanf("") };
+ILM_DEV bool category_proven(const LeanStep& a, int chunk) {
+    const uint64_t record = *(CUint64*)((const char*)a.cat_bounds + chunk * a.cat_stride);
+    const float lo = __builtin_bit_cast(float, (uint32_t)record), hi = __builtin_bit_cast(float, (uint32_t)(record >> 32));
+    return ((lo >= a.regular_cat_lo) & (hi <= a.regular_cat_hi)) != 0;
+}
+ILM_DEV SlotIn load_slot_uncategorised(const UnitPlanes& u, unsigned lane4) {
+    SlotIn s;
+    s.life = ld_plane<true>(u, 3, lane4);
+    s.px = ld_plane<true>(u, 0, lane4); s.py = ld_plane<true>(u, 1, lane4); s.pz = ld_plane<true>(u, 2, lane4);
+    s.vx = ld_plane<true>(u, 4, lane4); s.vy = ld_plane<true>(u, 5, lane4); s.vz = ld_plane<true>(u, 6, lane4); s.ct = 0.0f;
+    s.ar = s.ag = s.ab = s.aa = 0.0f;
+    return s;
+}
 ILM_DEV uint64_t regular_lanes_updated(float new_life, float vx, float vy) {
     return lane_mask(new_life > 0.0f) & lane_mask(new_life < __builtin_inff()) & lane_mask(!__builtin_isunordered(vx, vy));
 }
@@ -1340,9 +1360,14 @@
         }
         if (!untouched) {
             const unsigned lane4 = lane * 4u;
+            bool ct_pending = false;
+            if constexpr (CURVES == kCurvesClamp) ct_pending = category_proven(a, chunk);
             const UnitPlanes up = unit_planes(((CBase*)a.chunk_bases)[chunk], a.stride, seg * 64);
             const bool elide = STREAM && ((CURVES == kCurvesClamp) || (a.elide & kElideDerived) != 0u);
-            SlotIn cur = load_slot<false, STREAM>(up, lane4);
+            SlotIn cur;
+            if (CURVES == kCurvesClamp && ct_pending) cur = load_slot_uncategorised(up, lane4);
+            else cur = load_slot<false, STREAM>(up, lane4);
+            const bool ct_proven = ct_pending;
             if (!elide) {
                 const float4 stored = load_attributes<STREAM>(up, lane4);
                 cur.ar = stored.x; cur.ag = stored.y; cur.ab = stored.z; cur.aa = stored.w;
@@ -1376,7 +1401,7 @@
             float4 rc = zero, rd = zero;
             if constexpr (CURVES == kCurvesClamp) {
                 int body = kBodySelecting;
-                if (regular_lanes_loaded(a, cur) == kAllLanes) {
+                if ((ct_proven ? regular_lanes_loaded_proven(cur) : regular_lanes_loaded(a, cur)) == kAllLanes) {
                     body = kBodyRegular;
 #pragma unroll
                     for (int o = 0; o < ILM_MAX_OPS; o++) {
@@ -1397,8 +1422,11 @@
                 if (body == kBodyRegular) {
                     update_positions_unselected(pos, vel, a.sys, a.dt_s);
                     const bool stays = regular_lanes_updated(pos.w, vel.x, vel.y) == kAllLanes;
-                    if (__builtin_amdgcn_readfirstlane(*(CInt32*)&g_step_count_regular_waves) != 0 && lane == 0u)
-                        atomicAdd(&g_step_regular_waves[stays ? 0 : 1], 1ull);
+                    const int counting = __builtin_amdgcn_readfirstlane(*(CInt32*)&g_step_count_regular_waves);
+                    if (counting != 0 && lane == 0u) {
+                        if (counting & 1) atomicAdd(&g_step_regular_waves[stays ? 0 : 1], 1ull);
+                        if (counting & 2) atomicAdd(&g_step_category_waves[ct_proven ? (stays ? 0 : 1) : 2], 1ull);
+                    }
                     if (stays) {
                         const uint64_t vx_changed = lane_mask(!same_bits(vel.x, cur.vx)), vy_changed = lane_mask(!same_bits(vel.y, cur.vy)), vz_changed = lane_mask(!same_bits(vel.z, cur.vz));
                         if (lane_mask(!same_bits(pos.x, cur.px)) != 0ull) st_plane<true>(up, 0, lane4, pos.x);
@@ -1412,11 +1440,24 @@
                         n_live = 64u;
                         goto unit_stored;
                     }
+                    if (ct_pending) {
+                        cur.ct = ld_plane<true>(up, 7, lane4);
+                        vel.w = cur.ct;
+                        ct_pending = false;
+                    }
                     const bool keep = !(pos.w <= 0.0f);
                     pos = mk4(keep ? pos.x : 0.0f, keep ? pos.y : 0.0f, keep ? pos.z : 0.0f, keep ? pos.w : 0.0f);
                     vel = mk4(keep ? vel.x : 0.0f, keep ? vel.y : 0.0f, keep ? vel.z : 0.0f, keep ? vel.w : 0.0f);
                 }
                 if (body == kBodySelecting) {
+                    if (ct_pending) {
+                        cur.ct = ld_plane<true>(up, 7, lane4);
+                        ct_pending = false;
+                    }
+                    {
+                        const int counting = __builtin_amdgcn_readfirstlane(*(CInt32*)&g_step_count_regular_waves);
+                        if ((counting & 2) != 0 && lane == 0u) atomicAdd(&g_step_category_waves[ct_proven ? 1 : 2], 1ull);
+                    }
                     pos = mk4(cur.px, cur.py, cur.pz, cur.life);
                     vel = mk4(cur.vx, cur.vy, cur.vz, cur.ct);
                     if (__ballot(process) != 0ull) {
@@ -1820,6 +1861,91 @@
     return streaming && !spawning && (f.elide & kElideDerived) != 0u && (f.bezier_codes & ~kClampCodes) == 0u && f.update_bits == 2u;
 }
 
+constexpr int kCategoryScanSlots = 65536;
+ILM_DEV uint32_t float_order_key(float v) {
+    const uint32_t b = __builtin_bit_cast(uint32_t, v);
+    return (b & 0x80000000u) ? ~b : (b | 0x80000000u);
+}
+ILM_DEV float float_of_order_key(uint32_t k) { return __builtin_bit_cast(float, (k & 0x80000000u) ? (k & 0x7FFFFFFFu) : ~k); }
+__global__ __launch_bounds__(256) void category_bounds_kernel(float* const* __restrict__ bases, int64_t stride, int first_chunk, int used, float* __restrict__ records) {
+    __shared__ float wave_lo[4], wave_hi[4];
+    __shared__ uint32_t wave_nan[4];
+    const int chunk = first_chunk + (int)blockIdx.y;
+    const float* cat = bases[chunk] + 7 * stride;
+    float lo = __builtin_inff(), hi = -__builtin_inff();
+    bool nan = false;
+#pragma unroll 4
+    for (int k = 0; k < kCategoryScanSlots / 1024; k++) {
+        const int i0 = (int)blockIdx.x * kCategoryScanSlots + k * 1024 + (int)threadIdx.x * 4;
+        if (i0 < used) {
+            const float4 c = *reinterpret_cast<const float4*>(cat + i0);
+            const float v[4] = { c.x, c.y, c.z, c.w };
+#pragma unroll
+            for (int j = 0; j < 4; j++) {
+                if (i0 + j < used) {
+                    lo = fminf(lo, v[j]); hi = fmaxf(hi, v[j]);
+                    nan = nan || (v[j] != v[j]);
+                }
+            }
+        }
+    }
+    for (int d = 32; d >= 1; d >>= 1) {
+        lo = fminf(lo, __shfl_xor(lo, d));
+        hi = fmaxf(hi, __shfl_xor(hi, d));
+    }
+    const bool wave_has_nan = __ballot(nan) != 0ull;
+    if ((threadIdx.x & 63) == 0) { wave_lo[threadIdx.x >> 6] = lo; wave_hi[threadIdx.x >> 6] = hi; wave_nan[threadIdx.x >> 6] = wave_has_nan ? 1u : 0u; }
+    __syncthreads();
+    if (threadIdx.x == 0) {
+        lo = fminf(fminf(wave_lo[0], wave_lo[1]), fminf(wave_lo[2], wave_lo[3]));
+        hi = fmaxf(fmaxf(wave_hi[0], wave_hi[1]), fmaxf(wave_hi[2], wave_hi[3]));
+        float* rec = records + (size_t)chunk * kCategoryRecordStride;
+        uint32_t* work = reinterpret_cast<uint32_t*>(rec) + 4;
+        atomicMax(&work[0], ~float_order_key(lo));
+        atomicMax(&work[1], float_order_key(hi));
+        if ((wave_nan[0] | wave_nan[1] | wave_nan[2] | wave_nan[3]) != 0u) atomicOr(&work[2], 1u);
+        __threadfence();
+        if (atomicAdd(&work[3], 1u) == gridDim.x - 1u) {
+            __threadfence();
+            const uint32_t k_lo = ~atomicOr(&work[0], 0u), k_hi = atomicOr(&work[1], 0u), any_nan = atomicOr(&work[2], 0u);
+            rec[0] = any_nan ? __builtin_nanf("") : float_of_order_key(k_lo);
+            rec[1] = float_of_order_key(k_hi);
+            work[0] = 0u; work[1] = 0u; work[2] = 0u; work[3] = 0u;
+        }
+    }
+}
+static hipError_t launch_category_bounds(float* const* chunk_bases, int64_t stride, int first_chunk, int chunk_count, int used, float* records, hipStream_t stream) {
+    const unsigned blocks = (unsigned)std::max(1, (used + kCategoryScanSlots - 1) / kCategoryScanSlots);
+    hipLaunchKernelGGL(category_bounds_kernel, dim3(blocks, (unsigned)chunk_count), dim3(256), 0, stream, chunk_bases, stride, first_chunk, used, records);
+    return hipGetLastError();
+}
+static const float* no_category_record() {
+    constexpr int kDevices = 64;
+    static std::atomic<const float*> found[kDevices];
+    int device = 0;
+    if (hipGetDevice(&device) != hipSuccess || device < 0 || device >= kDevices) { (void)hipGetLastError(); return nullptr; }
+    const float* p = found[device];
+    if (p == nullptr) {
+        void* address = nullptr;
+        if (hipGetSymbolAddress(&address, HIP_SYMBOL(g_no_category_record)) != hipSuccess) { (void)hipGetLastError(); return nullptr; }
+        found[device] = p = static_cast<const float*>(address);
+    }
+    return p;
+}
+static hipError_t scan_category_records(const StepLaunch& a, CategoryRecords& cat, hipStream_t stream) {
+    const int end = a.first_chunk + a.chunk_count;
+    for (int ci = a.first_chunk; ci < end;) {
+        if (cat.current[ci]) { ci++; continue; }
+        int run = 1;
+        while (ci + run < end && !cat.current[ci + run] && cat.used[ci + run] == cat.used[ci]) run++;
+        const hipError_t e = launch_category_bounds(a.chunk_bases, a.stride, ci, run, std::min(cat.used[ci], a.slots), cat.table, stream);
+        if (e != hipSuccess) return e;
+        for (int k = 0; k < run; k++) cat.current[ci + k] = 1;
+        ci += run;
+    }
+    return hipSuccess;
+}
+
 static hipError_t launch_lean_step(const LeanStep& f, bool spawning, bool streaming, hipStream_t stream) {
     const int units_per_block = kStepThreads / 64;
     const dim3 grid((unsigned)((f.total_units + units_per_block - 1) / units_per_block), 1, 1), block(kStepThreads, 1, 1);
@@ -1989,9 +2115,13 @@
     a.total_padded = l.total_padded; a.unit_rotate = l.unit_rotate; a.count_buckets = l.count_buckets;
     return spawning;
 }
-hipError_t launch_step(StepLaunch& a, hipStream_t stream, uint32_t render_elide, bool* refreshed) {
+static void clear_category_records(const StepLaunch& a, CategoryRecords* cat) {
+    for (int ci = a.first_chunk; cat && ci < a.first_chunk + a.chunk_count; ci++) cat->current[ci] = 0;
+}
+hipError_t launch_step(StepLaunch& a, hipStream_t stream, uint32_t render_elide, bool* refreshed, CategoryRecords* cat) {
     if (refreshed) *refreshed = false;
     const bool spawning = layout_step(a);
+    if (spawning || (a.op_mask & (1u << ILM_OP_FMA)) != 0u) { clear_category_records(a, cat); cat = nullptr; }
     if (!step_interpreter_forced() && a.unit_end > a.unit_begin) {
         if (a.desc.UpdateMode == ILM_UPDATE_WITH_DISTANCE_FIELD) {
             const char* lean_env = getenv("ILM_DF_LEAN");
@@ -2000,6 +2130,7 @@
             if (lean_df && build_lean_step(a, f.base)) {
                 f.df = a.desc.DistanceField;
                 f.sdf = a.sdf;
+                clear_category_records(a, cat);
                 g_last_step_kernel = ILM_STEP_KERNEL_LEAN_DF;
                 return launch_lean_df_step(f, a, spawning, stream);
             }
@@ -2007,12 +2138,23 @@
             LeanStep f;
             if (build_lean_step(a, f)) {
                 f.elide = ((render_elide & kElideDerived) && a.streaming) ? (kElideDerived | (color_curves_bounded(a.desc.Update) ? kElideColor : 0u) | (f.elide & kElideRotation)) : 0u;
+                if (curves_clamp(f, spawning, a.streaming != 0)) {
+                    if (cat) {
+                        const hipError_t scanned = scan_category_records(a, *cat, stream);
+                        if (scanned != hipSuccess) { clear_category_records(a, cat); return scanned; }
+                        f.cat_bounds = cat->table; f.cat_stride = kCategoryRecordStride * (int32_t)sizeof(float);
+                    } else {
+                        f.cat_bounds = no_category_record(); f.cat_stride = 0;
+                        if (f.cat_bounds == nullptr) return hipErrorInvalidSymbol;
+                    }
+                }
                 const hipError_t e = launch_lean_step(f, spawning, a.streaming != 0, stream);
                 if (refreshed) *refreshed = (e == hipSuccess);
                 return e;
             }
         }
     }
+    clear_category_records(a, cat);
     g_last_step_kernel = ILM_STEP_KERNEL_INTERPRETER;
     return spawning ? launch_step_variant<true>(a, stream) : launch_step_variant<false>(a, stream);
 }
@@ -2239,16 +2381,31 @@
     return e;
 }
 
+static std::atomic<int> g_step_wave_counting{0};
+static hipError_t set_step_wave_counting(int bit, int enable) {
+    const int flag = enable ? (g_step_wave_counting |= bit) : (g_step_wave_counting &= ~bit);
+    return hipMemcpyToSymbol(HIP_SYMBOL(g_step_count_regular_waves), &flag, sizeof(flag));
+}
 hipError_t step_regular_wave_counter(int enable, unsigned long long out[2]) {
     unsigned long long value[2] = { 0, 0 }, zero[2] = { 0, 0 };
     hipError_t e = hipMemcpyFromSymbol(value, HIP_SYMBOL(g_step_regular_waves), sizeof(value));
     if (e != hipSuccess) return e;
     e = hipMemcpyToSymbol(HIP_SYMBOL(g_step_regular_waves), zero, sizeof(zero));
     if (e != hipSuccess) return e;
-    const int flag = enable ? 1 : 0;
-    e = hipMemcpyToSymbol(HIP_SYMBOL(g_step_count_regular_waves), &flag, sizeof(flag));
+    e = set_step_wave_counting(1, enable);
     if (out) { out[0] = value[0]; out[1] = value[1]; }
     return e;
 }
 
-}
+hipError_t step_category_wave_counter(int enable, unsigned long long out[3]) {
+    unsigned long long value[3] = { 0, 0, 0 }, zero[3] = { 0, 0, 0 };
+    hipError_t e = hipMemcpyFromSymbol(value, HIP_SYMBOL(g_step_category_waves), sizeof(value));
+    if (e != hipSuccess) return e;
+    e = hipMemcpyToSymbol(HIP_SYMBOL(g_step_category_waves), zero, sizeof(zero));
+    if (e != hipSuccess) return e;
+    e = set_step_wave_counting(2, enable);
+    if (out) { out[0] = value[0]; out[1] = value[1]; out[2] = value[2]; }
+    return e;
+}
+
+}
diff --git a/illuminant_amd/native.py b/illuminant_amd/native.py
--- a/illuminant_amd/native.py
+++ b/illuminant_amd/native.py
@@ -76,6 +76,8 @@
     "ilm_debug_step_streams": (_I, [_I]),
     "ilm_debug_step_sdf_samples": (_I, [_H, _I, C.POINTER(C.c_uint64)]),
     "ilm_debug_step_regular_waves": (_I, [_H, _I, C.POINTER(C.c_uint64), C.POINTER(C.c_uint64)]),
+    "ilm_debug_chunk_category_bounds": (_I, [_H, _I, C.POINTER(C.c_float), C.POINTER(C.c_float), C.POINTER(C.c_int32)]),
+    "ilm_debug_step_category_waves": (_I, [_H, _I, C.POINTER(C.c_uint64), C.POINTER(C.c_uint64), C.POINTER(C.c_uint64)]),
     "ilm_debug_last_light_launch": (_I, [_H, C.POINTER(C.c_int32), C.POINTER(C.c_int32), C.POINTER(C.c_int32)]),
     "ilm_debug_divide_by_constants": (_I, [_H, _P, _P, _I, C.POINTER(_I)]),
     "ilm_sdf_destroy": (_I, [_H]),
diff --git a/include/illuminant_hip.h b/include/illuminant_hip.h
--- a/include/illuminant_hip.h
+++ b/include/illuminant_hip.h
@@ -340,6 +340,8 @@
 int32_t ilm_debug_step_streams(int32_t streams);
 int32_t ilm_debug_step_sdf_samples(IlmHandle ctx, int32_t enable, uint64_t* out_samples);
 int32_t ilm_debug_step_regular_waves(IlmHandle ctx, int32_t enable, uint64_t* out_regular, uint64_t* out_selected);
+int32_t ilm_debug_chunk_category_bounds(IlmHandle system, int32_t chunk, float* out_lo, float* out_hi, int32_t* out_current);
+int32_t ilm_debug_step_category_waves(IlmHandle ctx, int32_t enable, uint64_t* out_skipped, uint64_t* out_late, uint64_t* out_upfront);
 int32_t ilm_debug_last_light_launch(IlmHandle ctx, int32_t* out_workgroups, int32_t* out_split, int32_t* out_tile_macro);
 int32_t ilm_sdf_destroy(IlmHandle sdf);
 int32_t ilm_sdf_download(IlmHandle sdf, uint16_t* texels);
```

Result: faster. 93610 (median of 6 runs) (+2.3%).
